# bbc/vc2-reference

Hardware: AMD Instinct MI355X
Metric: Mpixels/s encode+decode, UHD-1 10-bit HQ_ConstQ (higher is better)
Workload: dtype int32; 1 GPU; BASELINE cfg2: UHD-1 3840x2160 4:2:2 10-bit HQ_ConstQ DD97 depth 4, -u 1 -a 2 -q 16 -S 2; streams=1, parallelism=frame-parallel x1, no collective

## Files before the change

include/vc2hip.h:

```cpp
#ifndef VC2HIP_H
#define VC2HIP_H

#include <stddef.h>
#include <stdint.h>

#ifdef __cplusplus
extern "C" {
#endif
#if defined(__GNUC__)
#pragma GCC visibility push(default)
#endif

typedef struct vc2hip_ctx vc2hip_ctx;

enum { VC2HIP_DD97 = 0, VC2HIP_LEGALL = 1, VC2HIP_DD137 = 2, VC2HIP_HAAR0 = 3,
       VC2HIP_HAAR1 = 4, VC2HIP_FIDELITY = 5, VC2HIP_DAUB97 = 6 };
enum { VC2HIP_CF444 = 0, VC2HIP_CF422 = 1, VC2HIP_CF420 = 2 };
enum { VC2HIP_HQ_CONSTQ = 0, VC2HIP_HQ_CBR = 1, VC2HIP_LD = 2 };

enum {
  VC2HIP_OK = 0,
  VC2HIP_EINVAL = -1,
  VC2HIP_EQINDEX = -2,
  VC2HIP_ESCALAR = -3,
  VC2HIP_ECBR_TOOBIG = -4,
  VC2HIP_ECBR_LEN = -5,
  VC2HIP_ECBR_WRONG = -6,
  VC2HIP_EBOUNDED = -7,
  VC2HIP_ELD_TOOBIG = -8,
  VC2HIP_ECAP = -9,
  VC2HIP_ESTREAM = -10,
  VC2HIP_ECODE32 = -11,
  VC2HIP_ESYNTAX = -12,
  VC2HIP_EHIP = -100
};

int vc2hip_create(int device, vc2hip_ctx **out);
#define VC2HIP_FLAG_STORE32         0x001u
#define VC2HIP_FLAG_NO_STREAM       0x002u
#define VC2HIP_FLAG_NO_PAIR         0x004u
#define VC2HIP_FLAG_NO_BANDPLANES   0x008u
#define VC2HIP_FLAG_NO_HEADS        0x010u
#define VC2HIP_FLAG_NO_CBR_INDEX    0x020u
#define VC2HIP_FLAG_GENERIC_DWT     0x040u
#define VC2HIP_FLAG_SINGLE_PASS_VBR 0x080u
#define VC2HIP_FLAG_CBR_GENERAL     0x100u
#define VC2HIP_FLAG_LD_DIAGONALS    0x200u
#define VC2HIP_FLAG_PLANES8_ALWAYS  0x400u
#define VC2HIP_FLAG_PLANES8_NEVER   0x800u
#define VC2HIP_FLAG_TWO_PASS_VBR    0x1000u
int vc2hip_create_with_flags(int device, unsigned flags, vc2hip_ctx **out);
int vc2hip_create_on_stream(int device, void *hip_stream, vc2hip_ctx **out);
void vc2hip_destroy(vc2hip_ctx *ctx);
const char *vc2hip_last_error(const vc2hip_ctx *ctx);
const char *vc2hip_error_string(int code);
int vc2hip_sync(vc2hip_ctx *ctx);

int vc2hip_padded_size(int size, int depth);
int vc2hip_slice_size_is_valid(int depth, int len_luma, int len_chroma, int n_size);
int vc2hip_quant_matrix(int kernel, int depth, int32_t *out);
int vc2hip_slice_bytes(int y_slices, int x_slices, int total_bytes, int scalar, int32_t *out);

int vc2hip_dwt_forward(vc2hip_ctx *ctx, const int32_t *in, int h, int w, int kernel, int depth,
                       int32_t *out);
int vc2hip_dwt_inverse(vc2hip_ctx *ctx, const int32_t *in, int ph, int pw, int kernel, int depth,
                       int32_t *out, int h, int w);
int vc2hip_quantise_np(vc2hip_ctx *ctx, const int32_t *coef, int ph, int pw, int depth,
                       const int32_t *qidx, int ys, int xs, const int32_t *qmatrix, int32_t *out);
int vc2hip_dequantise_np(vc2hip_ctx *ctx, const int32_t *q, int ph, int pw, int depth,
                         const int32_t *qidx, int ys, int xs, const int32_t *qmatrix, int32_t *out);
int vc2hip_dequantise_ld(vc2hip_ctx *ctx, const int32_t *q, int ph, int pw, int depth,
                         const int32_t *qidx, int ys, int xs, const int32_t *qmatrix, int32_t *out);

int vc2hip_quantise_ld(vc2hip_ctx *ctx, const int32_t *coef, int ph, int pw, int depth,
                       const int32_t *qidx, int ys, int xs, const int32_t *qmatrix, int32_t *out);

typedef struct {
  int luma_h, luma_w;
  int chroma_h, chroma_w;
  int depth;
  int y_slices, x_slices;
} vc2hip_geom;

int vc2hip_hq_pack(vc2hip_ctx *ctx, const int32_t *y, const int32_t *u, const int32_t *v,
                   const vc2hip_geom *g, const int32_t *qidx, int prefix, int scalar,
                   const int32_t *cbr_slice_bytes, uint8_t *out, size_t cap, size_t *out_len);
int vc2hip_hq_unpack(vc2hip_ctx *ctx, const uint8_t *in, size_t len, const vc2hip_geom *g,
                     int prefix, int scalar, int32_t *y, int32_t *u, int32_t *v, int32_t *qidx,
                     size_t *consumed);
int vc2hip_ld_unpack(vc2hip_ctx *ctx, const uint8_t *in, size_t len, const vc2hip_geom *g,
                     const int32_t *slice_bytes, int32_t *y, int32_t *u, int32_t *v,
                     int32_t *qidx, size_t *consumed);
int vc2hip_ld_pack(vc2hip_ctx *ctx, const int32_t *y, const int32_t *u, const int32_t *v,
                   const vc2hip_geom *g, const int32_t *qidx, const int32_t *slice_bytes,
                   uint8_t *out, size_t cap, size_t *out_len);
int vc2hip_ld_qindices(vc2hip_ctx *ctx, const int32_t *y, const int32_t *u, const int32_t *v,
                       const vc2hip_geom *g, const int32_t *qmatrix, const int32_t *slice_bytes,
                       int32_t *qidx);
int vc2hip_cbr_qindices(vc2hip_ctx *ctx, const int32_t *y, const int32_t *u, const int32_t *v,
                        const vc2hip_geom *g, const int32_t *qmatrix, const int32_t *slice_bytes,
                        int scalar, int32_t *qidx);

typedef struct {
  int width, height;
  int chroma_format;
  int bit_depth;
  int word_bytes;
  int chroma_bit_depth;
} vc2hip_picture_format;

typedef struct {
  int kernel, depth;
  int y_slices, x_slices;
  int mode;
  int q_index;
  int compressed_bytes;
  int prefix, scalar;
} vc2hip_coding_params;

size_t vc2hip_raw_picture_bytes(const vc2hip_picture_format *fmt);
size_t vc2hip_max_payload_bytes(const vc2hip_picture_format *fmt, const vc2hip_coding_params *cp);

int vc2hip_encode_picture_hq(vc2hip_ctx *ctx, const void *raw, const vc2hip_picture_format *fmt,
                             const vc2hip_coding_params *cp, uint8_t *payload, size_t cap,
                             size_t *len, int32_t *qidx_out);
int vc2hip_encode_picture_ld(vc2hip_ctx *ctx, const void *raw, const vc2hip_picture_format *fmt,
                             const vc2hip_coding_params *cp, uint8_t *payload, size_t cap,
                             size_t *len, int32_t *qidx_out);
int vc2hip_decode_picture_hq(vc2hip_ctx *ctx, const uint8_t *payload, size_t len,
                             const vc2hip_picture_format *fmt, const vc2hip_coding_params *cp,
                             void *raw_out);
int vc2hip_decode_picture_ld(vc2hip_ctx *ctx, const uint8_t *payload, size_t len,
                             const vc2hip_picture_format *fmt, const vc2hip_coding_params *cp,
                             void *raw_out);

#define VC2HIP_MAX_INFLIGHT 2
void *vc2hip_host_alloc(size_t bytes);
void vc2hip_host_free(void *p);
int vc2hip_encode_picture_begin(vc2hip_ctx *ctx, const void *raw, const vc2hip_picture_format *fmt,
                                const vc2hip_coding_params *cp, uint8_t *payload, size_t cap, int32_t *qidx_out, int *ticket);
int vc2hip_encode_picture_end(vc2hip_ctx *ctx, int ticket, size_t *len);
int vc2hip_decode_picture_begin(vc2hip_ctx *ctx, const uint8_t *payload, size_t len, const vc2hip_picture_format *fmt,
                                const vc2hip_coding_params *cp, void *raw_out, int *ticket);
int vc2hip_decode_picture_end(vc2hip_ctx *ctx, int ticket);

int vc2hip_set_streams(vc2hip_ctx *ctx, int k);
int vc2hip_encode_batch_dev(vc2hip_ctx *ctx, const void *d_raw, int n,
                            const vc2hip_picture_format *fmt, const vc2hip_coding_params *cp,
                            void *d_payload, size_t payload_stride, uint64_t *d_lens);
int vc2hip_decode_batch_dev(vc2hip_ctx *ctx, const void *d_payload, size_t payload_stride,
                            const uint64_t *d_lens, int n, const vc2hip_picture_format *fmt,
                            const vc2hip_coding_params *cp, void *d_raw_out);

typedef struct {
  int major_version;
  uint32_t first_picture_number;
  uint32_t prev_parse_offset;
  int end_of_sequence;
} vc2hip_stream_params;

int vc2hip_picture_header(const vc2hip_coding_params *cp, int major_version, uint32_t picture_number,
                          uint8_t *out, size_t cap, size_t *len);
int vc2hip_stream_write_dev(vc2hip_ctx *ctx, const void *d_payload, size_t payload_stride, const uint64_t *d_lens, int n,
                            const vc2hip_coding_params *cp, const vc2hip_stream_params *sp,
                            uint8_t *d_stream, size_t cap, uint64_t *d_stream_len);
int vc2hip_stream_read_dev(vc2hip_ctx *ctx, const uint8_t *d_stream, size_t len, int n,
                           const vc2hip_coding_params *cp, const vc2hip_stream_params *sp,
                           void *d_payload, size_t payload_stride, uint64_t *d_lens,
                           uint32_t *d_picture_numbers, uint64_t *d_consumed);

int vc2hip_band_plane_bits(const vc2hip_ctx *ctx);

#define VC2HIP_DWT_TILE   0
#define VC2HIP_DWT_FAST   1
#define VC2HIP_DWT_STREAM 2
#define VC2HIP_DWT_PAIR   3
#define VC2HIP_DWT_PLANE  4
typedef struct {
  int inverse;
  int level;
  int levels;
  int family;
  int edge;
  int store_bits;
  int segments;
  int tail;
  int small_gather;
  int pictures;
  int band_planes;
} vc2hip_dwt_launch;
int vc2hip_dwt_launches(const vc2hip_ctx *ctx, vc2hip_dwt_launch *out, int cap);

int vc2hip_profile_enable(vc2hip_ctx *ctx, int on);
int vc2hip_profile_only(vc2hip_ctx *ctx, const char *name);
int vc2hip_profile_count(vc2hip_ctx *ctx);
int vc2hip_profile_get(vc2hip_ctx *ctx, int i, const char **name, int *launches, double *total_ms);
int vc2hip_profile_reset(vc2hip_ctx *ctx);

#if defined(__GNUC__)
#pragma GCC visibility pop
#endif
#ifdef __cplusplus
}
#endif
#endif
```

vc2-reference_amd/csrc/vc2hip_api.hip:

```cpp
#include <math.h>
#include <stdio.h>
#include <stdlib.h>
#include <string.h>

#include <algorithm>
#include <string>
#include <map>
#include <mutex>
#include <utility>
#include <vector>

#include "vc2hip_internal.h"

void vc2_upload_tables_slices(const QuantTables &t, hipStream_t s);
int vc2_halo_x(int kernel);
int vc2_halo_y(int kernel);
void vc2_upload_vlc_lut(hipStream_t s);
void vc2_upload_unpack_lut(hipStream_t s);
bool vc2_slice_index_supported(int prefix, int scalar);
size_t vc2_pack_lds_bytes(int prefix, int scalar);
int vc2_pack_image_mode(int prefix, int scalar);
void vc2_upload_tables_fast(const QuantTables &t, hipStream_t s);
bool vc2_fast_level_applicable(LevelParams &p);
int vc2_launch_forward_fast(Launcher &L, int kernel, bool first, const LevelParams &p, int n, bool store16, hipStream_t s);
int vc2_launch_inverse_fast(Launcher &L, int kernel, bool final_level, const LevelParams &p, int n, bool store16, hipStream_t s);
bool vc2_fast_small_gather(const LevelParams &p);
void vc2_upload_tables_stream(const QuantTables &t, hipStream_t s);
size_t vc2_stream_level_applicable(LevelParams &p, int kernel, bool edge, bool inverse, bool store16, int n_pictures);
int vc2_launch_forward_stream(Launcher &L, int kernel, bool first, const LevelParams &p, int n, bool store16, size_t lds, hipStream_t s);
int vc2_launch_inverse_stream(Launcher &L, int kernel, bool final_level, const LevelParams &p, int n, bool store16, size_t lds, hipStream_t s);
size_t vc2_pair_applicable(PairParams &pp, int kernel, bool edge, bool inverse, bool store16, int n_pictures);
int vc2_launch_forward_pair(Launcher &L, int kernel, bool first, const PairParams &pp, int n, bool store16, size_t lds, hipStream_t s);
int vc2_launch_inverse_pair(Launcher &L, int kernel, bool final_level, const PairParams &pp, int n, bool store16, size_t lds, hipStream_t s);
void vc2_upload_tables_pair(const QuantTables &t, hipStream_t s);
int vc2_launch_plane_transform(Launcher &L, int kernel, int32_t *plane, long long plane_stride, int ph, int pw, int depth, bool inverse,
                               int n, hipStream_t s);
void vc2_launch_plane_ingest(Launcher &L, const void *raw, long long raw_stride, int pic_h, int pic_w, int word_bytes, int bit_depth,
                             int32_t *plane, long long plane_stride, int ph, int pw, int n, hipStream_t s);
void vc2_launch_plane_emit(Launcher &L, const int32_t *plane, long long plane_stride, int pw, void *raw, long long raw_stride, int pic_h,
                           int pic_w, int word_bytes, int bit_depth, int n, hipStream_t s);
void vc2_launch_ll_into_plane(Launcher &L, const int32_t *ll, long long ll_stride, int llh, int llw, int32_t *plane, long long plane_stride,
                              int pw, int depth, int n, hipStream_t s);
void vc2_launch_fill_i32(Launcher &L, int32_t *p, int32_t v, size_t n, hipStream_t s);
void vc2_launch_fill_u64(Launcher &L, unsigned long long *p, unsigned long long v, size_t n, hipStream_t s);

struct ProfEntry {
  std::string name;
  int launches = 0;
  double ms = 0;
};
struct Launcher {
  bool on = false;
  std::string only;
  const char *last_name = nullptr;
  std::string launch_error;
  std::vector<ProfEntry> entries;
  struct Pending { int entry; hipEvent_t a, b; };
  std::vector<Pending> pending;
  std::vector<hipEvent_t> pool;
  int cur_entry = -1;
  hipEvent_t get() {
    hipEvent_t e;
    if (!pool.empty()) { e = pool.back(); pool.pop_back(); }
    else (void)hipEventCreate(&e);
    return e;
  }
  void collect() {
    for (auto &p : pending) {
      float ms = 0;
      if (hipEventElapsedTime(&ms, p.a, p.b) == hipSuccess) { entries[p.entry].ms += ms; entries[p.entry].launches++; }
      pool.push_back(p.a);
      pool.push_back(p.b);
    }
    pending.clear();
  }
};
void vc2_prof_begin(Launcher &L, const char *name, hipStream_t s) {
  (void)s;
  L.last_name = name;
  if (!L.on) return;
  if (!L.only.empty() && ("," + L.only + ",").find(std::string(",") + name + ",") == std::string::npos) return;
  int idx = -1;
  for (size_t i = 0; i < L.entries.size(); ++i) if (L.entries[i].name == name) { idx = (int)i; break; }
  if (idx < 0) { L.entries.push_back(ProfEntry{name, 0, 0}); idx = (int)L.entries.size() - 1; }
  L.cur_entry = idx;
}
void vc2_prof_pair(Launcher &L, hipEvent_t *a, hipEvent_t *b) {
  *a = *b = nullptr;
  if (!L.on || L.cur_entry < 0) return;
  *a = L.get();
  *b = L.get();
  L.pending.push_back(Launcher::Pending{L.cur_entry, *a, *b});
}
void vc2_prof_end(Launcher &L, hipStream_t s) {
  (void)s;
  const hipError_t le = hipGetLastError();
  if (le != hipSuccess && L.launch_error.empty())
    L.launch_error = std::string("kernel launch failed (") + (L.last_name ? L.last_name : "?") + "): " + hipGetErrorString(le);
  L.cur_entry = -1;
#ifdef VC2HIP_ABLATE
  {
    static const bool dbg_sync = getenv("VC2HIP_DEBUG_SYNC") != nullptr;
    if (dbg_sync) {
      fprintf(stderr, "vc2hip stage %s ...", L.last_name ? L.last_name : "?");
      fflush(stderr);
      const hipError_t e = hipStreamSynchronize(s);
      fprintf(stderr, " %s\n", e == hipSuccess ? "done" : hipGetErrorString(e));
      fflush(stderr);
    }
  }
#endif
}
void vc2_prof_break(Launcher &L) { (void)L; }

struct Buf {
  void *p = nullptr;
  size_t cap = 0;
};
enum { B_RAW, B_STORE, B_STOREW, B_LL0, B_LLW, B_QIDX, B_SLOTS, B_SIZES, B_OFFS, B_LENS, B_PAYLOAD,
       B_INDEX, B_PLANE, B_PLANE2, B_CBRB, B_CBRO, B_QM, B_UNITS, B_SEGS, B_COUNT };

struct vc2hip_ctx {
  int device = 0;
  hipStream_t stream = nullptr;
  bool own_stream = false;
  unsigned *d_err = nullptr;
  unsigned *h_err = nullptr;
  Buf buf[B_COUNT];
  Launcher L;
  std::string err;
  int cbr_key[5] = {-1, -1, -1, -1, -1};
  uint64_t cbr_total = 0;
  int debug_skip = 0;
  bool two_pass_vbr = true;
  bool force_two_pass_vbr = false;
#ifndef VC2_ONE_PASS_MIN_PICTURES
#define VC2_ONE_PASS_MIN_PICTURES 112
#endif
  bool force_generic = false;
  bool allow_store16 = true;
  bool allow_planes = true;
  int planes8_mode = 0;
  bool planes8_on = false;
  unsigned long long *d_stat = nullptr;
  unsigned long long *h_stat = nullptr;
  hipEvent_t stat_ev = nullptr;
  bool stat_pending = false, stat_was8 = false, stat_seen = false;
  int stat_n = 0;
  int stat_n_total = 0;
  int last_plane_bits = 0;
  std::vector<vc2hip_dwt_launch> dwt_rec;
  bool dwt_rec_stale = true;
  double stat_samples = 0;
  int ld_batch = 1;
  bool allow_heads = true;
  bool allow_cbr_index = true;
  bool allow_stream = true;
  bool allow_pair = true;
  bool cbr_general = false;
  bool ld_diagonals = false;
  unsigned flags = 0;
  std::vector<vc2hip_ctx *> lanes;
  bool in_split = false;
  hipEvent_t fork_ev = nullptr;
  std::vector<hipEvent_t> join_ev;
  bool lanes_pending = false;
  struct Range { const uint8_t *lo, *hi; };
  struct LaneUse { Range r[2], w[2]; bool valid = false; };
  std::vector<LaneUse> lane_use;
  std::vector<ProfEntry> merged;
  struct Flight {
    vc2hip_ctx *lane = nullptr;
    bool open = false, encode = false;
    uint8_t *payload = nullptr;
    size_t cap = 0;
    unsigned long long *h_len = nullptr;
  };
  Flight flight[VC2HIP_MAX_INFLIGHT];
  int flight_next = 0;
};

static const char *code_text(int code) {
  switch (code) {
    case VC2HIP_OK: return "ok";
    case VC2HIP_EINVAL: return "invalid argument";
    case VC2HIP_EQINDEX: return "quantization index exceeds maximum implemented value.";
    case VC2HIP_ESCALAR: return "Slice scalar is too small, consider using a larger slice scalar.";
    case VC2HIP_ECBR_TOOBIG: return "SliceIO, HQ CBR mode: Too many bytes for the slice";
    case VC2HIP_ECBR_LEN: return "Slice component length exceeds 1 byte when divided by slice size scalar. See above for suggestions to prevent this.";
    case VC2HIP_ECBR_WRONG: return "SliceIO, HQ CBR mode: Wrong number of bytes for a slice";
    case VC2HIP_EBOUNDED: return "Attempt to write beyond end of bounded write";
    case VC2HIP_ELD_TOOBIG: return "SliceIO, LD mode: Too many bytes for the U and V slices";
    case VC2HIP_ECAP: return "output buffer too small";
    case VC2HIP_ESTREAM: return "truncated or malformed slice data";
    case VC2HIP_ECODE32: return "quantised coefficient magnitude exceeds 65534 (outside the 32-bit exp-Golomb code domain)";
    case VC2HIP_ESYNTAX: return "VC-2 stream syntax error";
    case VC2HIP_EHIP: return "HIP runtime error";
  }
  return "unknown error";
}
extern "C" const char *vc2hip_error_string(int code) { return code_text(code); }

static int set_err(vc2hip_ctx *c, int code, const char *msg = nullptr) {
  if (c) c->err = msg ? msg : code_text(code);
  return code;
}
static int hip_fail(vc2hip_ctx *c, hipError_t e, const char *what) {
  char b[256];
  snprintf(b, sizeof b, "HIP error in %s: %s", what, hipGetErrorString(e));
  return set_err(c, VC2HIP_EHIP, b);
}
#define HIPCHK(ctx, call)                                       \
  do {                                                          \
    hipError_t e_ = (call);                                     \
    if (e_ != hipSuccess) return hip_fail(ctx, e_, #call);      \
  } while (0)

extern "C" const char *vc2hip_last_error(const vc2hip_ctx *ctx) { return ctx ? ctx->err.c_str() : "null context"; }

extern "C" int vc2hip_padded_size(int size, int depth) {
  const int cell = 1 << depth;
  return cell * ((size + cell - 1) / cell);
}
extern "C" int vc2hip_slice_size_is_valid(int depth, int len_luma, int len_chroma, int n_size) {
  if (depth <= 0 || depth > 31) return 0;
  const int unit = 1 << depth;
  const int max_slices = (len_luma < len_chroma ? len_luma : len_chroma) / unit;
  if (n_size <= 0 || n_size > max_slices) return 0;
  const int ts = n_size * unit;
  const int pl = vc2hip_padded_size(len_luma, depth), pc = vc2hip_padded_size(len_chroma, depth);
  const int n = (pl + ts - 1) / ts;
  if (pl % n == 0 && (pl / n) % unit == 0 && pc % n == 0 && (pc / n) % unit == 0) return n;
  return 0;
}
extern "C" int vc2hip_quant_matrix(int kernel, int depth, int32_t *out) {
  static const float A[7] = {1.280868846f, 1.224744871f, 1.280868846f, 1.414213562f, 1.414213562f, 0.682408629f, 1.139917028f};
  static const float B[7] = {0.820572875f, 0.847791248f, 0.809253958f, 0.707106871f, 0.707106871f, 1.367856979f, 0.887168005f};
  static const int S[7] = {1, 1, 1, 0, 1, 0, 1};
  if (kernel < 0 || kernel > 6 || depth < 0 || depth > 30) return VC2HIP_EINVAL;
  if (depth == 0) { out[0] = 0; return 0; }
  const float a2 = A[kernel] * A[kernel], ab = A[kernel] * B[kernel], b2 = B[kernel] * B[kernel];
  std::vector<float> gl(depth + 1), gh(depth + 1), gd(depth + 1);
  float mn = 3.402823466e+38f;
  for (int lv = depth; lv > 0; --lv) {
    const float sc = (float)(pow((double)a2, depth - lv) / pow(2.0, S[kernel] * (depth - lv + 1)));
    gl[lv] = sc * a2; gh[lv] = sc * ab; gd[lv] = sc * b2;
    mn = fminf(fminf(fminf(gl[lv], gh[lv]), gd[lv]), mn);
  }
  auto qv = [&](float g) { return (int)floorf(4.0f * logf(g / mn) / logf(2.0f) + 0.5f); };
  int i = 0;
  out[i++] = qv(gl[1]);
  for (int lv = 1; lv <= depth; ++lv) { out[i++] = qv(gh[lv]); out[i++] = qv(gh[lv]); out[i++] = qv(gd[lv]); }
  return 0;
}
void vc2_allow_lds(const void *kernel, size_t bytes) {
  static std::mutex mu;
  static std::map<std::pair<const void *, int>, size_t> done;
  int dev = 0;
  (void)hipGetDevice(&dev);
  std::lock_guard<std::mutex> lock(mu);
  size_t &have = done[std::make_pair(kernel, dev)];
  if (bytes > have) {
    (void)hipFuncSetAttribute(kernel, hipFuncAttributeMaxDynamicSharedMemorySize, (int)bytes);
    have = bytes;
  }
}

static int gcd_i(int a, int b) { a = abs(a); b = abs(b); while (b) { int t = a % b; a = b; b = t; } return a; }
extern "C" int vc2hip_slice_bytes(int ys, int xs, int total_bytes, int scalar, int32_t *out) {
  if (ys < 1 || xs < 1 || scalar < 1) return VC2HIP_EINVAL;
  const int n = ys * xs;
  int num = total_bytes / scalar - 4 * n, den = n;
  const int g = gcd_i(num, den);
  if (g) { num /= g; den /= g; }
  const int ratio = num / den, rem = num - ratio * den;
  int residue = 0;
  for (int i = 0; i < n; ++i) {
    residue += rem;
    if (residue < den) out[i] = ratio * scalar + 4;
    else { out[i] = (ratio + 1) * scalar + 4; residue -= den; }
  }
  return 0;
}
static void make_tables(QuantTables &t) {
  for (int q = 0; q < 120; ++q) {
    const uint64_t base = 1ull << (q / 4);
    uint64_t f;
    switch (q % 4) {
      case 0: f = 4 * base; break;
      case 1: f = (503829 * base + 52958) / 105917; break;
      case 2: f = (665857 * base + 58854) / 117708; break;
      default: f = (440253 * base + 32722) / 65444; break;
    }
    t.qf[q] = (int32_t)(uint32_t)f;
    t.off[q] = q == 0 ? 1 : (q == 1 ? 2 : (int32_t)(((uint32_t)t.qf[q] + 1u)) / 2);
    t.magic[q] = 0;
    t.shift[q] = 0;
    if (t.qf[q] > 1) {
      const uint64_t d = (uint64_t)t.qf[q];
      int l = 0;
      while ((1ull << l) < d) ++l;
      t.magic[q] = (uint32_t)((((1ull << l) - d) << 32) / d + 1);
      t.shift[q] = l - 1;
    }
    const double r = 4.0 / (double)(uint32_t)t.qf[q];
    float up = (float)r;
    if ((double)up < r) up = nextafterf(up, INFINITY);
    t.inv4[q] = up;
  }
}

static int create_common(int device, hipStream_t stream, bool own, vc2hip_ctx **out, unsigned flags = 0) {
  if (!out) return VC2HIP_EINVAL;
  *out = nullptr;
  int n = 0;
  if (hipGetDeviceCount(&n) != hipSuccess || device < 0 || device >= n) return VC2HIP_EHIP;
  vc2hip_ctx *c = new vc2hip_ctx;
  c->device = device;
#ifdef VC2HIP_ABLATE
  {
    static const struct { const char *name; unsigned flag; } env[] = {
      {"VC2HIP_STORE32", VC2HIP_FLAG_STORE32}, {"VC2HIP_NO_STREAM", VC2HIP_FLAG_NO_STREAM}, {"VC2HIP_NO_PAIR", VC2HIP_FLAG_NO_PAIR},
      {"VC2HIP_NO_BANDPLANES", VC2HIP_FLAG_NO_BANDPLANES}, {"VC2HIP_NO_HEADS", VC2HIP_FLAG_NO_HEADS},
      {"VC2HIP_NO_CBR_INDEX", VC2HIP_FLAG_NO_CBR_INDEX}, {"VC2HIP_GENERIC_DWT", VC2HIP_FLAG_GENERIC_DWT},
      {"VC2HIP_SINGLE_PASS_VBR", VC2HIP_FLAG_SINGLE_PASS_VBR}, {"VC2HIP_TWO_PASS_VBR", VC2HIP_FLAG_TWO_PASS_VBR}, {"VC2HIP_CBR_GENERAL", VC2HIP_FLAG_CBR_GENERAL},
      {"VC2HIP_PLANES8_ALWAYS", VC2HIP_FLAG_PLANES8_ALWAYS}, {"VC2HIP_PLANES8_NEVER", VC2HIP_FLAG_PLANES8_NEVER}};
    for (const auto &e : env) { const char *v = getenv(e.name); if (v && v[0] == '1') flags |= e.flag; }
    { const char *v = getenv("VC2HIP_LD_ROWS"); if (v && v[0] == '0') flags |= VC2HIP_FLAG_LD_DIAGONALS; }
    { const char *e = getenv("VC2HIP_DEBUG_SKIP"); c->debug_skip = e ? atoi(e) : 0; }
  }
#endif
  c->force_generic = (flags & VC2HIP_FLAG_GENERIC_DWT) != 0;
  c->allow_store16 = !(flags & VC2HIP_FLAG_STORE32);
  c->allow_stream = !(flags & VC2HIP_FLAG_NO_STREAM);
  c->allow_pair = !(flags & VC2HIP_FLAG_NO_PAIR);
  c->allow_planes = !(flags & VC2HIP_FLAG_NO_BANDPLANES);
  c->planes8_mode = (flags & VC2HIP_FLAG_PLANES8_NEVER) ? 2 : (flags & VC2HIP_FLAG_PLANES8_ALWAYS) ? 1 : 0;
  c->allow_heads = !(flags & VC2HIP_FLAG_NO_HEADS);
  c->allow_cbr_index = !(flags & VC2HIP_FLAG_NO_CBR_INDEX);
  c->two_pass_vbr = !(flags & VC2HIP_FLAG_SINGLE_PASS_VBR);
  c->force_two_pass_vbr = (flags & VC2HIP_FLAG_TWO_PASS_VBR) != 0;
  c->cbr_general = (flags & VC2HIP_FLAG_CBR_GENERAL) != 0;
  c->ld_diagonals = (flags & VC2HIP_FLAG_LD_DIAGONALS) != 0;
  c->flags = flags;
  if (hipSetDevice(device) != hipSuccess) { delete c; return VC2HIP_EHIP; }
  if (own) { if (hipStreamCreateWithFlags(&stream, hipStreamNonBlocking) != hipSuccess) { delete c; return VC2HIP_EHIP; } }
  c->stream = stream;
  c->own_stream = own;
  if (hipMalloc((void **)&c->d_err, 256 + 4096) != hipSuccess ||
     
      hipHostMalloc((void **)&c->h_err, VC2_ERRBLK_COPY) != hipSuccess ||
      hipMalloc((void **)&c->d_stat, 64) != hipSuccess || hipHostMalloc((void **)&c->h_stat, 64 * 8) != hipSuccess ||
      hipEventCreateWithFlags(&c->stat_ev, hipEventDisableTiming) != hipSuccess) { delete c; return VC2HIP_EHIP; }
  (void)hipMemsetAsync(c->d_stat, 0, 64, c->stream);
  (void)hipMemsetAsync(c->d_err, 0, sizeof(unsigned), c->stream);
  QuantTables t;
  make_tables(t);
  vc2_upload_tables(t, c->stream);
  vc2_upload_tables_slices(t, c->stream);
  vc2_upload_tables_fast(t, c->stream);
  vc2_upload_tables_pair(t, c->stream);
  vc2_upload_tables_stream(t, c->stream);
  vc2_upload_vlc_lut(c->stream);
  vc2_upload_unpack_lut(c->stream);
  if (hipStreamSynchronize(c->stream) != hipSuccess) { delete c; return VC2HIP_EHIP; }
  *out = c;
  return VC2HIP_OK;
}
extern "C" int vc2hip_create(int device, vc2hip_ctx **out) { return create_common(device, nullptr, true, out); }
extern "C" int vc2hip_create_with_flags(int device, unsigned flags, vc2hip_ctx **out) { return create_common(device, nullptr, true, out, flags); }
extern "C" int vc2hip_create_on_stream(int device, void *s, vc2hip_ctx **out) { return create_common(device, (hipStream_t)s, false, out); }
extern "C" void vc2hip_destroy(vc2hip_ctx *c) {
  if (!c) return;
  (void)hipSetDevice(c->device);
  (void)hipStreamSynchronize(c->stream);
  for (vc2hip_ctx *l : c->lanes) if (l != c) vc2hip_destroy(l);
  for (auto &f : c->flight) { if (f.lane) vc2hip_destroy(f.lane); if (f.h_len) (void)hipHostFree(f.h_len); }
  for (hipEvent_t e : c->join_ev) (void)hipEventDestroy(e);
  if (c->fork_ev) (void)hipEventDestroy(c->fork_ev);
  c->L.collect();
  for (auto e : c->L.pool) (void)hipEventDestroy(e);
  for (auto &b : c->buf) if (b.p) (void)hipFree(b.p);
  if (c->d_err) (void)hipFree(c->d_err);
  if (c->h_err) (void)hipHostFree(c->h_err);
  if (c->h_stat) (void)hipHostFree(c->h_stat);
  if (c->d_stat) (void)hipFree(c->d_stat);
  if (c->stat_ev) (void)hipEventDestroy(c->stat_ev);
  if (c->own_stream) (void)hipStreamDestroy(c->stream);
  delete c;
}

void vc2_ld_disable_rows();
static int err_from_flags(vc2hip_ctx *c, unsigned f) {
  if (!f) return VC2HIP_OK;
  if (f & VC2_DEVERR_HANDOFF) {
    vc2_ld_disable_rows();
    return set_err(c, VC2HIP_EHIP, "LD index search: a hand-over between workgroups timed out; nothing was written for the batch. "
                                   "The library now searches with one launch per slice diagonal: submit the batch again.");
  }
  if (f & VC2_DEVERR_SYNTAX) {
    static const char *why[VC2_SYN_COUNT] = {"?", "parse info prefix is not BBCD", "unknown parse code",
                                             "data unit runs past the end of the stream", "next_parse_offset is 0",
                                             "end of sequence before the pictures asked for",
                                             "picture parameters differ from the coding parameters",
                                             "custom quantisation matrix flag set", "asymmetric transform",
                                             "picture before any sequence header and no major version given",
                                             "fragment out of order"};
    const unsigned w = *(const unsigned *)((const char *)c->h_err + VC2_ERRBLK_SYNTAX_WHY);
    char b[256];
    snprintf(b, sizeof b, "VC-2 stream syntax error at byte %llu: %s",
             *(const unsigned long long *)((const char *)c->h_err + VC2_ERRBLK_SYNTAX_AT), why[w < VC2_SYN_COUNT ? w : 0]);
    return set_err(c, VC2HIP_ESYNTAX, b);
  }
  if (f & VC2_DEVERR_QINDEX) return set_err(c, VC2HIP_EQINDEX);
  if (f & VC2_DEVERR_SCALAR) return set_err(c, VC2HIP_ESCALAR);
  if (f & VC2_DEVERR_CBR_TOOBIG) return set_err(c, VC2HIP_ECBR_TOOBIG);
  if (f & VC2_DEVERR_CBR_LEN) return set_err(c, VC2HIP_ECBR_LEN);
  if (f & VC2_DEVERR_CODE32) return set_err(c, VC2HIP_ECODE32);
  if (f & VC2_DEVERR_LD_TOOBIG) return set_err(c, VC2HIP_ELD_TOOBIG);
  if (f & VC2_DEVERR_CAP) return set_err(c, VC2HIP_ECAP);
  return set_err(c, VC2HIP_ESTREAM);
}
static int join_lanes(vc2hip_ctx *c) {
  if (!c->lanes_pending || c->in_split) return VC2HIP_OK;
  for (size_t i = 1; i < c->lanes.size(); ++i)
    if (c->lane_use[i].valid) HIPCHK(c, hipStreamWaitEvent(c->stream, c->join_ev[i], 0));
  c->lanes_pending = false;
  return VC2HIP_OK;
}
static int enter(vc2hip_ctx *c) {
  HIPCHK(c, hipSetDevice(c->device));
  if (!c->in_split) vc2_prof_break(c->L);
  c->dwt_rec_stale = true;
  return join_lanes(c);
}
#define ENTER(ctx) do { int rc_ = enter(ctx); if (rc_) return rc_; } while (0)

extern "C" int vc2hip_set_streams(vc2hip_ctx *c, int k) {
  if (!c || k < 1 || k > 16) return set_err(c, VC2HIP_EINVAL);
  ENTER(c);
  HIPCHK(c, hipStreamSynchronize(c->stream));
  for (vc2hip_ctx *l : c->lanes) if (l != c) vc2hip_destroy(l);
  c->lanes.clear();
  c->lane_use.clear();
  for (hipEvent_t e : c->join_ev) (void)hipEventDestroy(e);
  c->join_ev.clear();
  if (k == 1) return VC2HIP_OK;
  if (!c->fork_ev) HIPCHK(c, hipEventCreateWithFlags(&c->fork_ev, hipEventDisableTiming));
  for (int i = 0; i < k; ++i) {
    vc2hip_ctx *l = c;
    if (i > 0) {
      const int rc = vc2hip_create_with_flags(c->device, c->flags, &l);
      if (rc) return set_err(c, rc);
      l->L.on = c->L.on;
    }
    c->lanes.push_back(l);
    hipEvent_t e;
    HIPCHK(c, hipEventCreateWithFlags(&e, hipEventDisableTiming));
    c->join_ev.push_back(e);
  }
  c->lane_use.assign((size_t)k, vc2hip_ctx::LaneUse());
  return VC2HIP_OK;
}

template <class U, class F> static int split_batch(vc2hip_ctx *c, int n, U use, F fn) {
  const int k = std::min<int>((int)c->lanes.size(), n);
  HIPCHK(c, hipSetDevice(c->device));
  HIPCHK(c, hipEventRecord(c->fork_ev, c->stream));
  std::vector<vc2hip_ctx::LaneUse> cur((size_t)c->lanes.size());
  std::vector<int> first((size_t)k), count((size_t)k);
  auto overlap = [](const vc2hip_ctx::Range &a, const vc2hip_ctx::Range &b) { return a.lo && b.lo && a.lo < b.hi && b.lo < a.hi; };
  for (int i = 0, f0 = 0; i < k; ++i) {
    count[i] = n / k + (i < n % k ? 1 : 0);
    first[i] = f0;
    f0 += count[i];
    use(first[i], count[i], cur[i]);
    cur[i].valid = true;
  }
  for (int i = 0; i < k; ++i) {
    vc2hip_ctx *l = c->lanes[i];
    if (i > 0) HIPCHK(c, hipStreamWaitEvent(l->stream, c->fork_ev, 0));
    for (size_t j = 0; j < c->lanes.size(); ++j) {
      const vc2hip_ctx::LaneUse &p = c->lane_use[j];
      if ((int)j == i || !p.valid) continue;
      bool dep = false;
      for (int a = 0; a < 2; ++a)
        for (int b = 0; b < 2; ++b)
          dep |= overlap(cur[i].r[a], p.w[b]) || overlap(cur[i].w[a], p.w[b]) || overlap(cur[i].w[a], p.r[b]);
// ... 34 lines not shown
    return set_err(c, VC2HIP_EHIP, m.c_str());
  }
  const int rc = err_from_flags(c, *c->h_err);
  return rc ? rc : lane_rc;
}

static int need(vc2hip_ctx *c, int which, size_t bytes, void **out) {
  Buf &b = c->buf[which];
  if (b.cap < bytes) {
    HIPCHK(c, hipStreamSynchronize(c->stream));
    if (b.p) HIPCHK(c, hipFree(b.p));
    b.p = nullptr;
    b.cap = 0;
    size_t cap = bytes >= (1u << 21) ? (bytes + (1u << 21) - 1) & ~(size_t)((1u << 21) - 1) : (bytes + 4095) & ~(size_t)4095;
    { static const size_t unit = (size_t)vc2_tune_int("VC2HIP_ALLOC_ROUND_MB", 0) << 20;
      if (unit && bytes >= (1u << 21)) cap = (bytes + unit - 1) / unit * unit; }
    HIPCHK(c, hipMalloc(&b.p, cap));
    b.cap = cap;
#ifdef VC2HIP_ABLATE
    if (getenv("VC2HIP_DEBUG_ALLOC")) fprintf(stderr, "vc2hip alloc: buffer %d at %p, %zu bytes\n", which, b.p, cap);
#endif
  }
  *out = b.p;
  return VC2HIP_OK;
}
#define NEED(ctx, which, bytes, ptr)                                   \
  do {                                                                 \
    void *p_;                                                          \
    int rc_ = need(ctx, which, bytes, &p_);                            \
    if (rc_) return rc_;                                               \
    ptr = (decltype(ptr))p_;                                           \
  } while (0)

extern "C" int vc2hip_profile_enable(vc2hip_ctx *c, int on) {
  if (!c) return VC2HIP_EINVAL;
  c->L.on = on != 0;
  for (vc2hip_ctx *l : c->lanes) l->L.on = on != 0;
  return 0;
}
extern "C" int vc2hip_profile_only(vc2hip_ctx *c, const char *name) {
  if (!c) return VC2HIP_EINVAL;
  c->L.only = name ? name : "";
  for (vc2hip_ctx *l : c->lanes) l->L.only = c->L.only;
  return 0;
}
extern "C" int vc2hip_profile_count(vc2hip_ctx *c) {
  if (!c) return 0;
  c->merged = c->L.entries;
  for (vc2hip_ctx *l : c->lanes)
    if (l != c) for (const ProfEntry &e : l->L.entries) {
      bool found = false;
      for (ProfEntry &m : c->merged) if (m.name == e.name) { m.launches += e.launches; m.ms += e.ms; found = true; break; }
      if (!found) c->merged.push_back(e);
    }
  return (int)c->merged.size();
}
extern "C" int vc2hip_profile_get(vc2hip_ctx *c, int i, const char **name, int *launches, double *total_ms) {
  if (!c || i < 0 || i >= (int)c->merged.size()) return VC2HIP_EINVAL;
  if (name) *name = c->merged[i].name.c_str();
  if (launches) *launches = c->merged[i].launches;
  if (total_ms) *total_ms = c->merged[i].ms;
  return 0;
}
extern "C" int vc2hip_profile_reset(vc2hip_ctx *c) {
  if (!c) return VC2HIP_EINVAL;
  c->L.collect(); c->L.entries.clear(); c->merged.clear();
  for (vc2hip_ctx *l : c->lanes) if (l != c) { l->L.collect(); l->L.entries.clear(); }
  return 0;
}

static int make_geom(Geom &g, const int ph[3], const int pw[3], const int h[3], const int w[3], int depth,
                     int ys, int xs) {
  if (depth < 1 || depth > VC2_MAX_DEPTH || ys < 1 || xs < 1) return VC2HIP_EINVAL;
  g.depth = depth; g.ys = ys; g.xs = xs;
  int off = 0;
  for (int c = 0; c < 3; ++c) {
    CompGeom &cg = g.c[c];
    cg.h = h[c]; cg.w = w[c]; cg.ph = ph[c]; cg.pw = pw[c];
    if (ph[c] == 0 || pw[c] == 0) { cg.sh = cg.sw = cg.n0 = 0; cg.coef_off = off; continue; }
    if (ph[c] % ys || pw[c] % xs) return VC2HIP_EINVAL;
    cg.sh = ph[c] / ys; cg.sw = pw[c] / xs;
    if (cg.sh % (1 << depth) || cg.sw % (1 << depth)) return VC2HIP_EINVAL;
    cg.n0 = (cg.sh >> depth) * (cg.sw >> depth);
    cg.coef_off = off;
    off += cg.sh * cg.sw;
  }
  g.slice_coefs = off;
  return VC2HIP_OK;
}

static void chroma_dims(int h, int w, int cf, int *ch, int *cw) {
  *ch = cf == VC2HIP_CF420 ? h / 2 : h;
  *cw = cf == VC2HIP_CF444 ? w : w / 2;
}

static int picture_geom(Geom &g, const vc2hip_picture_format *f, const vc2hip_coding_params *cp, bool decoder) {
  if (!f || !cp || f->width < 1 || f->height < 1 || f->word_bytes < 1 || f->word_bytes > 4 ||
      f->bit_depth < 1 || f->bit_depth > 8 * f->word_bytes || f->chroma_format < 0 || f->chroma_format > 2 ||
      f->chroma_bit_depth < 0 || f->chroma_bit_depth > 8 * f->word_bytes)
    return VC2HIP_EINVAL;
  int ch, cw;
  chroma_dims(f->height, f->width, f->chroma_format, &ch, &cw);
  int h[3] = {f->height, ch, ch}, w[3] = {f->width, cw, cw}, ph[3], pw[3];
  ph[0] = vc2hip_padded_size(f->height, cp->depth);
  pw[0] = vc2hip_padded_size(f->width, cp->depth);
  if (decoder) chroma_dims(ph[0], pw[0], f->chroma_format, &ph[1], &pw[1]);
  else { ph[1] = vc2hip_padded_size(ch, cp->depth); pw[1] = vc2hip_padded_size(cw, cp->depth); }
  ph[2] = ph[1]; pw[2] = pw[1];
  return make_geom(g, ph, pw, h, w, cp->depth, cp->y_slices, cp->x_slices);
}

extern "C" size_t vc2hip_raw_picture_bytes(const vc2hip_picture_format *f) {
  int ch, cw;
  chroma_dims(f->height, f->width, f->chroma_format, &ch, &cw);
  return ((size_t)f->height * f->width + 2 * (size_t)ch * cw) * f->word_bytes;
}
static size_t max_slice_bytes(int prefix, int scalar) { return (size_t)prefix + 4 + 3 * 255 * (size_t)scalar; }
extern "C" size_t vc2hip_max_payload_bytes(const vc2hip_picture_format *f, const vc2hip_coding_params *cp) {
  (void)f;
  const size_t n = (size_t)cp->y_slices * cp->x_slices;
  if (cp->mode == VC2HIP_HQ_CONSTQ) return n * max_slice_bytes(cp->prefix, cp->scalar);
  if (cp->mode == VC2HIP_HQ_CBR) return (size_t)cp->compressed_bytes + n * (cp->prefix + (size_t)cp->scalar + 4);
  return (size_t)cp->compressed_bytes + n;
}

struct LLPlanes {
  void *p[VC2_MAX_DEPTH + 1][3];
  int32_t *w[VC2_MAX_DEPTH + 1][3];
  long long stride[VC2_MAX_DEPTH + 1][3];
};

static size_t ll_elems(const Geom &g, int n) {
  size_t e = 0;
  for (int l = 1; l <= g.depth; ++l)
    for (int c = 0; c < 3; ++c) e += (((size_t)(g.c[c].ph >> l) * (g.c[c].pw >> l) * n + 7) & ~(size_t)7);
  return e;
}
static size_t ll_bytes(const Geom &g, int n) { return ll_elems(g, n) * sizeof(int32_t); }
static void ll_layout(const Geom &g, int n, void *base, int elem_bytes, int32_t *wide, LLPlanes &ll) {
  size_t off = 0;
  memset(&ll, 0, sizeof ll);
  for (int l = 1; l <= g.depth; ++l)
    for (int c = 0; c < 3; ++c) {
      const size_t e = (size_t)(g.c[c].ph >> l) * (g.c[c].pw >> l);
      ll.p[l][c] = (char *)base + off * elem_bytes;
      ll.w[l][c] = wide ? wide + off : nullptr;
      ll.stride[l][c] = (long long)e;
      off += (e * n + 7) & ~(size_t)7;
    }
}
static void ll_layout(const Geom &g, int n, int32_t *base, LLPlanes &ll) { ll_layout(g, n, base, 4, nullptr, ll); }

static void record_dwt(vc2hip_ctx *c, bool inverse, int level, int levels, int family, bool edge, bool s16, int segments, int tail,
                       bool small_gather, int n, int band_planes = 0) {
  if (c->dwt_rec_stale) { c->dwt_rec.clear(); c->dwt_rec_stale = false; }
  vc2hip_dwt_launch r;
  r.inverse = inverse; r.level = level; r.levels = levels; r.family = family; r.edge = edge; r.store_bits = s16 ? 16 : 32;
  r.segments = segments; r.tail = tail; r.small_gather = small_gather; r.pictures = n; r.band_planes = band_planes;
  c->dwt_rec.push_back(r);
}

static int band_plane_bits(const LevelParams &p) {
  for (int k = 0; k < 3; ++k) if (p.bp_base[k] >= 0) return p.bp8 ? 8 : 16;
  return 0;
}

static void fill_level(LevelParams &p, const Geom &g, int level, int kernel, const int32_t *qm) {
  const int D = g.depth, Lv = D - level;
  p.band = 3 * (Lv - 1) + 1;
  p.ys = g.ys; p.xs = g.xs; p.slice_coefs = g.slice_coefs;
  const int hx = vc2_halo_x(kernel), hy = vc2_halo_y(kernel);
  for (int c = 0; c < 3; ++c) {
    const CompGeom &cg = g.c[c];
    p.in_h[c] = cg.ph >> level; p.in_w[c] = cg.pw >> level;
    p.pic_h[c] = cg.h; p.pic_w[c] = cg.w;
    p.coef_off[c] = cg.coef_off;
    p.rec_stride[c] = g.slice_coefs;
    if (cg.ph == 0) { p.tiles_x[c] = p.tiles_y[c] = 0; p.fh[c] = p.fw[c] = 2; p.tsy[c] = p.tsx[c] = 1; continue; }
    p.fh[c] = cg.sh >> level; p.fw[c] = cg.sw >> level;
    int tsy = 1, tsx = 1;
    while (tsy * 2 * p.fh[c] <= 64 && tsy * 2 <= g.ys) tsy *= 2;
    while (tsx * 2 * p.fw[c] <= 128 && tsx * 2 <= g.xs) tsx *= 2;
    while ((size_t)(tsy * p.fh[c] + 2 * hy) * (tsx * p.fw[c] + 2 * hx) * 4 > 150 * 1024) {
      if (tsx > 1) tsx /= 2; else if (tsy > 1) tsy /= 2; else break;
    }
    p.tsy[c] = tsy; p.tsx[c] = tsx;
    p.tiles_y[c] = (g.ys + tsy - 1) / tsy;
    p.tiles_x[c] = (g.xs + tsx - 1) / tsx;
    p.band_n[c] = (p.fh[c] / 2) * (p.fw[c] / 2);
    p.band_off[c] = p.band_n[c];
  }
  for (int b = 0; b < 3 * D + 1; ++b) p.qmatrix[b] = qm ? qm[b] : 0;
}

static int run_forward(vc2hip_ctx *c, const Geom &g, int kernel, int n, const void *const src[3],
                       const long long src_stride[3], bool src_raw, const vc2hip_picture_format *f,
                       void *store, const LLPlanes &ll, bool s16 = false, int32_t *store_wide = nullptr) {
  auto level_params = [&](LevelParams &p, int level) {
    memset(&p, 0, sizeof p);
    fill_level(p, g, level, kernel, nullptr);
    p.store = store; p.store_stride = (long long)g.ys * g.xs * g.slice_coefs;
    p.store_wide = store_wide;
    p.err = c->d_err;
    p.ll_to_store = (level == g.depth - 1);
    const bool first = (level == 0) && src_raw;
    for (int k = 0; k < 3; ++k) {
      if (level == 0) { p.plane[k] = (void *)src[k]; p.plane_stride[k] = src_stride[k]; }
      else { p.plane[k] = ll.p[level][k]; p.plane_wide[k] = ll.w[level][k]; p.plane_stride[k] = ll.stride[level][k]; }
      p.ll[k] = ll.p[level + 1][k]; p.ll_wide[k] = ll.w[level + 1][k]; p.ll_stride[k] = ll.stride[level + 1][k];
    }
    if (first) {
      p.word_bytes = f->word_bytes;
      p.sample_shift = 8 * f->word_bytes - f->bit_depth;
      p.sample_offset = 1 << (f->bit_depth - 1);
      const int cd = f->chroma_bit_depth ? f->chroma_bit_depth : f->bit_depth;
      p.sample_shift_c = 8 * f->word_bytes - cd;
      p.sample_offset_c = 1 << (cd - 1);
    }
  };
  for (int level = 0; level < g.depth; ++level) {
    LevelParams p;
    level_params(p, level);
    const bool first = (level == 0) && src_raw;
    if (!c->force_generic && c->allow_stream && c->allow_pair && level + 1 < g.depth) {
      PairParams pp;
      memset(&pp, 0, sizeof pp);
      pp.a = p;
      pp.a.debug_skip = c->debug_skip;
      level_params(pp.b, level + 1);
      const size_t lds = vc2_pair_applicable(pp, kernel, first, false, s16, n);
      if (lds) {
        int rc = vc2_launch_forward_pair(c->L, kernel, first, pp, n, s16, lds, c->stream);
        if (rc) return set_err(c, rc, "invalid wavelet kernel");
        record_dwt(c, false, level, 2, VC2HIP_DWT_PAIR, first, s16, pp.a.st_segmax, 0, false, n);
        ++level;
        continue;
      }
    }
    LevelParams pf = p;
    pf.debug_skip = c->debug_skip;
    if (!c->force_generic && c->allow_stream) {
      LevelParams ps = p;
      const size_t lds = vc2_stream_level_applicable(ps, kernel, first, false, s16, n);
      if (lds) {
        int rc = vc2_launch_forward_stream(c->L, kernel, first, ps, n, s16, lds, c->stream);
        if (rc) return set_err(c, rc, "invalid wavelet kernel");
        record_dwt(c, false, level, 1, VC2HIP_DWT_STREAM, first, s16, ps.st_segmax, ps.st_tail, false, n);
        continue;
      }
    }
    if (!c->force_generic && vc2_fast_level_applicable(pf)) {
      int rc = vc2_launch_forward_fast(c->L, kernel, first, pf, n, s16, c->stream);
      if (rc) return set_err(c, rc, "invalid wavelet kernel");
      record_dwt(c, false, level, 1, VC2HIP_DWT_FAST, first, s16, 0, 0, false, n);
      continue;
    }
    if (s16) return set_err(c, VC2HIP_EINVAL, "internal: 16-bit store without the fast level kernels");
    if (vc2_level_lds_bytes(kernel, p) > 160 * 1024) return set_err(c, VC2HIP_EINVAL, "slice too large for one LDS tile");
    int rc = vc2_launch_forward_level(c->L, kernel, first, p, n, c->stream);
    if (rc) return set_err(c, rc, "invalid wavelet kernel");
    record_dwt(c, false, level, 1, VC2HIP_DWT_TILE, first, false, 0, 0, false, n);
  }
  return VC2HIP_OK;
}

static int run_inverse(vc2hip_ctx *c, const Geom &g, int kernel, int n, void *store, const int32_t *qidx,
                       const int32_t *qm, bool dequant, bool ll_ready, const LLPlanes &ll, void *const dst[3],
                       const long long dst_stride[3], bool dst_raw, const vc2hip_picture_format *f,
                       bool s16 = false, int32_t *store_wide = nullptr, const BandPlanes *bp = nullptr,
                       long long store_stride = 0, unsigned *stream_mask = nullptr, const HeadSplit *hs = nullptr, int head_level = 1 << 30,
                       unsigned *fast_mask = nullptr, unsigned *tail_mask = nullptr) {
  if (tail_mask) *tail_mask = 0;
  if (stream_mask) *stream_mask = 0;
  if (fast_mask) *fast_mask = 0;
  auto level_params = [&](LevelParams &p, int level) {
    memset(&p, 0, sizeof p);
    fill_level(p, g, level, kernel, qm);
    if (hs && level >= head_level)
      for (int k = 0; k < 3; ++k) if (g.c[k].ph) { p.rec_stride[k] = hs->n[k]; p.coef_off[k] = (int)hs->base[k]; }
    p.store = store; p.store_stride = store_stride ? store_stride : (long long)g.ys * g.xs * g.slice_coefs;
    for (int k = 0; k < 3; ++k) p.bp_base[k] = (bp && level < bp->levels && g.c[k].ph) ? bp->base[k][level] : -1;
    p.bp8 = bp && level < bp->levels && bp->bytes8;
    p.store_wide = store_wide;
    p.qidx = qidx; p.err = c->d_err; p.dequant = dequant;
    p.ll_from_store = (level == g.depth - 1) && !ll_ready;
    const bool fin = (level == 0) && dst_raw;
    for (int k = 0; k < 3; ++k) {
      if (level == 0) { p.plane[k] = dst ? dst[k] : nullptr; p.plane_stride[k] = dst_stride ? dst_stride[k] : 0; }
      else { p.plane[k] = ll.p[level][k]; p.plane_wide[k] = ll.w[level][k]; p.plane_stride[k] = ll.stride[level][k]; }
      p.ll[k] = ll.p[level + 1][k]; p.ll_wide[k] = ll.w[level + 1][k]; p.ll_stride[k] = ll.stride[level + 1][k];
    }
    if (fin) {
      p.word_bytes = f->word_bytes;
      p.sample_shift = 8 * f->word_bytes - f->bit_depth;
      p.sample_offset = 1 << (f->bit_depth - 1);
      p.clip_lo = -(1 << (f->bit_depth - 1));
      p.clip_hi = (1 << (f->bit_depth - 1)) - 1;
    }
  };
  for (int level = g.depth - 1; level >= 0; --level) {
    LevelParams p;
    level_params(p, level);
    const bool fin = (level == 0) && dst_raw;
    if (!stream_mask && !c->force_generic && c->allow_stream && c->allow_pair && level >= 1) {
      PairParams pp;
      memset(&pp, 0, sizeof pp);
      level_params(pp.a, level - 1);
      pp.b = p;
      pp.a.debug_skip = c->debug_skip;
      const bool fin_a = (level - 1 == 0) && dst_raw;
      static const int inv_final = vc2_tune_int("VC2HIP_PAIR_INV_FINAL", 0);
      const size_t lds = (fin_a && !inv_final) ? 0 : vc2_pair_applicable(pp, kernel, fin_a, true, s16, n);
      if (lds) {
        int rc = vc2_launch_inverse_pair(c->L, kernel, fin_a, pp, n, s16, lds, c->stream);
        if (rc) return set_err(c, rc, "invalid wavelet kernel");
        record_dwt(c, true, level - 1, 2, VC2HIP_DWT_PAIR, fin_a, s16, pp.a.st_segmax, 0, false, n,
                   std::max(band_plane_bits(pp.a), band_plane_bits(pp.b)));
        --level;
        continue;
      }
    }
    LevelParams pf = p;
    pf.debug_skip = c->debug_skip;
    if (!c->force_generic && c->allow_stream) {
      LevelParams ps = p;
      const size_t lds = vc2_stream_level_applicable(ps, kernel, fin, true, s16, n);
      if (lds) {
        if (stream_mask) { *stream_mask |= 1u << level; if (tail_mask && ps.st_tail) *tail_mask |= 1u << level; continue; }
        int rc = vc2_launch_inverse_stream(c->L, kernel, fin, ps, n, s16, lds, c->stream);
        if (rc) return set_err(c, rc, "invalid wavelet kernel");
        record_dwt(c, true, level, 1, VC2HIP_DWT_STREAM, fin, s16, ps.st_segmax, ps.st_tail, false, n, band_plane_bits(ps));
        continue;
      }
    }
    if (stream_mask) { if (fast_mask && !c->force_generic && vc2_fast_level_applicable(pf)) *fast_mask |= 1u << level; continue; }
    if (bp && level < bp->levels) return set_err(c, VC2HIP_EINVAL, "internal: band planes without the streaming kernel");
    if (!c->force_generic && vc2_fast_level_applicable(pf)) {
      int rc = vc2_launch_inverse_fast(c->L, kernel, fin, pf, n, s16, c->stream);
      if (rc) return set_err(c, rc, "invalid wavelet kernel");
      record_dwt(c, true, level, 1, VC2HIP_DWT_FAST, fin, s16, 0, 0, vc2_fast_small_gather(pf), n, band_plane_bits(pf));
      continue;
    }
    if (s16) return set_err(c, VC2HIP_EINVAL, "internal: 16-bit store without the fast level kernels");
    if (vc2_level_lds_bytes(kernel, p) > 160 * 1024) return set_err(c, VC2HIP_EINVAL, "slice too large for one LDS tile");
    int rc = vc2_launch_inverse_level(c->L, kernel, fin, p, n, c->stream);
    if (rc) return set_err(c, rc, "invalid wavelet kernel");
    record_dwt(c, true, level, 1, VC2HIP_DWT_TILE, fin, false, 0, 0, false, n, band_plane_bits(p));
  }
  return VC2HIP_OK;
}

static bool use_store16(const vc2hip_ctx *c, const Geom &g, int kernel) {
  if (!c->allow_store16 || c->force_generic) return false;
  for (int k = 0; k < 3; ++k) {
    if (!g.c[k].ph) continue;
    if ((g.c[k].sh * g.c[k].sw) % 8 || g.c[k].coef_off % 8) return false;
  }
  if (g.slice_coefs % 8) return false;
  for (int level = 0; level < g.depth; ++level) {
    LevelParams p;
    memset(&p, 0, sizeof p);
    fill_level(p, g, level, kernel, nullptr);
    if (!vc2_fast_level_applicable(p)) return false;
  }
  return true;
}

static bool needs_plane_path(const vc2hip_ctx *c, const Geom &g, int kernel) {
  for (int level = 0; level < g.depth; ++level) {
    LevelParams p;
    memset(&p, 0, sizeof p);
    fill_level(p, g, level, kernel, nullptr);
    LevelParams pf = p;
    if (!c->force_generic && vc2_fast_level_applicable(pf)) continue;
    if (vc2_level_lds_bytes(kernel, p) > 160 * 1024) return true;
  }
  return false;
}
static size_t plane_elems(const Geom &g) {
  size_t e = 0;
  for (int k = 0; k < 3; ++k) e += (size_t)g.c[k].ph * g.c[k].pw;
  return e;
}
static int plane_forward(vc2hip_ctx *c, const Geom &g, int kernel, int n, const void *const src[3], const long long ss[3],
                         const vc2hip_picture_format *f, int32_t *d_store) {
  int32_t *d_plane;
  NEED(c, B_PLANE, plane_elems(g) * n * 4, d_plane);
// ... 724 lines not shown
        for (int k = 0; k < c->stat_n; ++k) bytes += (double)c->h_stat[1 + k];
        const double bits = c->stat_n ? 8.0 * bytes / (c->stat_n * c->stat_samples) : 99.0;
        const double esc = (double)c->h_stat[0] * 8.0 / (std::max(1, c->stat_n_total) * c->stat_samples);
#ifdef VC2HIP_ABLATE
        if (getenv("VC2HIP_PLANES8_DEBUG")) fprintf(stderr, "planes8: previous batch %d pictures, %.2f payload bits per sample, %s planes, escape pieces %.4f%%\n", c->stat_n, bits, c->stat_was8 ? "byte" : "16-bit", 100 * esc);
#endif
        if (c->stat_was8 && esc > 0.005) c->planes8_on = false;
        else if (!c->stat_was8 || esc < 0.002) c->planes8_on = bits < (c->planes8_on ? 6.5 : 6.0);
      }
      bool b8 = c->planes8_mode == 1 || (c->planes8_mode == 0 && c->planes8_on);
      for (int l = 0; l < bp.levels; ++l) if (tails >> l & 1) b8 = false;
      bp.bytes8 = b8;
    }
  }
  HeadSplit hs;
  memset(&hs, 0, sizeof hs);
  int head_level = 1 << 30;
  if (s16 && !plane_path && c->allow_heads) {
    unsigned smask = 0, fmask = 0;
    LLPlanes none;
    memset(&none, 0, sizeof none);
    (void)run_inverse(c, g, cp->kernel, n, nullptr, nullptr, qm, true, ld, none, dst, ds, true, f, s16, nullptr, nullptr, 0, &smask, nullptr, 1 << 30, &fmask);
    int ls = g.depth;
    while (ls > 0 && !(smask >> (ls - 1) & 1) && (fmask >> (ls - 1) & 1)) --ls;
    bool ok = ls >= 1 && ls < g.depth && ls >= bp.levels;
    for (int k = 0; k < 3 && ok; ++k) {
      if (!g.c[k].ph) continue;
      const int hn = (g.c[k].sh >> ls) * (g.c[k].sw >> ls);
      ok = hn >= 8 && hn % 8 == 0 && hn <= bp.from[k];
    }
    if (ok) {
      long long at = sstride;
      for (int k = 0; k < 3; ++k) {
        if (!g.c[k].ph) continue;
        hs.n[k] = (g.c[k].sh >> ls) * (g.c[k].sw >> ls);
        hs.base[k] = at;
        at += ((long long)ns * hs.n[k] + 7) & ~7ll;
      }
      if (at < (1ll << 31)) { sstride = at; head_level = ls; } else memset(&hs, 0, sizeof hs);
    }
  }
  int32_t *d_store, *d_ll, *d_q, *d_storew = nullptr, *d_llw = nullptr;
  {
    static const int pad = vc2_tune_int("VC2HIP_DEC_STORE_PAD", 0);
    if (s16 && pad > 0 && sstride + pad < (1ll << 31)) sstride += pad & ~7;
  }
  NEED(c, B_STORE, std::max((size_t)n * ns * g.slice_coefs * 4, (size_t)n * (size_t)sstride * 2), d_store);
  NEED(c, B_LL0, ll_bytes(g, n) + 16, d_ll);
  if (s16) {
    NEED(c, B_STOREW, (size_t)n * sstride * 4, d_storew);
    NEED(c, B_LLW, ll_bytes(g, n) + 16, d_llw);
  }
  NEED(c, B_QIDX, (size_t)n * ns * 4, d_q);
  LLPlanes ll;
  ll_layout(g, n, d_ll, s16 ? 2 : 4, d_llw, ll);
  if (!ld) {
    if (!d_lens || cp->scalar < 1 || cp->prefix < 0) return set_err(c, VC2HIP_EINVAL);
    uint32_t *d_offs;
    const int32_t *d_cb = nullptr; const uint32_t *d_co = nullptr; uint64_t cbr_total = 0;
    if (cp->mode == VC2HIP_HQ_CBR && cp->compressed_bytes > 0 && c->allow_cbr_index) {
      const int key[5] = {g.ys, g.xs, cp->compressed_bytes, cp->scalar, cp->prefix};
      if (memcmp(key, c->cbr_key, sizeof key) || !c->buf[B_CBRB].p) {
        std::vector<int32_t> sb(ns);
        int32_t *db; uint32_t *dof; uint64_t total;
        if (vc2hip_slice_bytes(g.ys, g.xs, cp->compressed_bytes, cp->scalar, sb.data()) == VC2HIP_OK &&
            cbr_offsets_upload(c, sb.data(), ns, cp->prefix, &db, &dof, &total) == VC2HIP_OK) {
          memcpy(c->cbr_key, key, sizeof key);
          c->cbr_total = total;
        }
      }
      if (!memcmp(key, c->cbr_key, sizeof key)) { d_cb = (const int32_t *)c->buf[B_CBRB].p; d_co = (const uint32_t *)c->buf[B_CBRO].p; cbr_total = c->cbr_total; }
    }
    if ((rc = build_index(c, (const uint8_t *)d_payload, (long long)payload_stride, (const unsigned long long *)d_lens, n, ns,
                          cp->prefix, cp->scalar, &d_offs, d_cb, d_co, cbr_total))) return rc;
    UnpackParams p;
    memset(&p, 0, sizeof p);
    p.payload = (const uint8_t *)d_payload; p.payload_stride = (long long)payload_stride;
    p.lens = (const unsigned long long *)d_lens; p.offsets = d_offs;
    p.store = d_store; p.store_stride = sstride; p.qidx = d_q;
    p.store16 = s16; p.store_wide = d_storew;
    p.n_slices = ns; p.slice_coefs = g.slice_coefs;
    int n0[3];
    fill_comp_arrays(g, p.comp_n, p.comp_off, n0);
    p.prefix = cp->prefix; p.scalar = cp->scalar; p.err = c->d_err;
    p.bp = bp; p.hs = hs; p.xs = g.xs;
    c->last_plane_bits = bp.levels ? (bp.bytes8 ? 8 : 16) : 0;
    p.stats = c->d_stat;
    bool capturing = false;
    if (!c->own_stream) {
      hipStreamCaptureStatus cs = hipStreamCaptureStatusNone;
      capturing = hipStreamIsCapturing(c->stream, &cs) != hipSuccess || cs != hipStreamCaptureStatusNone;
    }
    const bool track = bp.levels && c->planes8_mode == 0 && !c->stat_pending && !capturing;
    if (track) HIPCHK(c, hipMemsetAsync(c->d_stat, 0, 8, c->stream));
    vc2_launch_unpack(c->L, p, n, c->stream);
    if (track) {
      c->stat_n = std::min(n, 60);
      c->stat_n_total = n;
      c->stat_samples = 0;
      for (int k = 0; k < 3; ++k) c->stat_samples += (double)g.c[k].h * g.c[k].w;
      c->stat_was8 = bp.bytes8 != 0;
      HIPCHK(c, hipMemcpyAsync(c->h_stat, c->d_stat, 8, hipMemcpyDeviceToHost, c->stream));
      HIPCHK(c, hipMemcpyAsync(c->h_stat + 1, d_lens, (size_t)c->stat_n * 8, hipMemcpyDeviceToHost, c->stream));
      HIPCHK(c, hipEventRecord(c->stat_ev, c->stream));
      c->stat_pending = true;
    }
  } else {
    int32_t *d_sb; uint32_t *d_so; uint64_t total;
    const int key[5] = {g.ys, g.xs, cp->compressed_bytes, 1, -7};
    if (memcmp(key, c->cbr_key, sizeof key) || !c->buf[B_CBRB].p) {
      std::vector<int32_t> sb(ns);
      vc2hip_slice_bytes(g.ys, g.xs, cp->compressed_bytes, 1, sb.data());
      if ((rc = ld_offsets_upload(c, sb.data(), ns, &d_sb, &d_so, &total))) return rc;
      memcpy(c->cbr_key, key, sizeof key);
      c->cbr_total = total;
    }
    d_sb = (int32_t *)c->buf[B_CBRB].p; d_so = (uint32_t *)c->buf[B_CBRO].p; total = c->cbr_total;
    if (total > payload_stride) return set_err(c, VC2HIP_ESTREAM);
    LdUnpackParams p;
    fill_ld_unpack(p, g, (const uint8_t *)d_payload, (long long)payload_stride, d_sb, d_so, d_store, d_q, c->d_err);
    unsigned *d_shifted; uint32_t *d_starts;
    NEED(c, B_SIZES, (size_t)n * 4, d_shifted);
    NEED(c, B_OFFS, (size_t)n * ns * 4, d_starts);
    int flag_fill = 0;
#ifdef VC2HIP_ABLATE
    if (getenv("VC2HIP_DEBUG_LD_REDO")) flag_fill = 1;
#endif
    HIPCHK(c, hipMemsetAsync(d_shifted, flag_fill, (size_t)n * 4, c->stream));
    vc2_prof_break(c->L);
    p.lens = (const unsigned long long *)d_lens; p.shifted = d_shifted; p.starts = d_starts;
    vc2_launch_ld_unpack(c->L, p, n, c->stream);
    vc2_launch_ld_walk(c->L, p, n, c->stream);
    p.redo = 1;
    vc2_launch_ld_unpack(c->L, p, n, c->stream);
    LdLl3Params lp;
    lp.store = d_store; lp.store_stride = (long long)ns * g.slice_coefs; lp.slice_coefs = g.slice_coefs;
    lp.ys = g.ys; lp.xs = g.xs; lp.qidx = d_q; lp.qm0 = qm[0]; lp.err = c->d_err;
    for (int k = 0; k < 3; ++k) {
      lp.coef_off[k] = g.c[k].coef_off; lp.llh[k] = g.c[k].ph >> g.depth; lp.llw[k] = g.c[k].pw >> g.depth;
      lp.ll_plane[k] = (int32_t *)ll.p[g.depth][k]; lp.ll_stride[k] = ll.stride[g.depth][k];
    }
    if (!vc2_launch_ld_ll3(c->L, lp, n, c->stream))
    for (int k = 0; k < 3; ++k)
      vc2_launch_ld_ll(c->L, d_store, (long long)ns * g.slice_coefs, g.slice_coefs, g.c[k].coef_off, g.c[k].n0,
                       g.c[k].ph >> g.depth, g.c[k].pw >> g.depth, g.ys, g.xs, d_q, qm[0], (int32_t *)ll.p[g.depth][k],
                       ll.stride[g.depth][k], n, c->d_err, c->stream);
  }
  if (plane_path) return plane_inverse(c, g, cp->kernel, n, d_store, d_q, qm, dst, ds, f, ld ? &ll : nullptr);
  return run_inverse(c, g, cp->kernel, n, d_store, d_q, qm, true, ld, ll, dst, ds, true, f, s16, d_storew, &bp, sstride, nullptr,
                     hs.n[0] ? &hs : nullptr, head_level);
}

extern "C" int vc2hip_band_plane_bits(const vc2hip_ctx *c) { return c ? c->last_plane_bits : 0; }

namespace {
struct HeaderBits {
  uint8_t *out;
  size_t cap, pos = 0;
  unsigned cache = 0;
  int cached = 0;
  void bit(unsigned b) {
    cache = (cache << 1) | (b & 1);
    if (++cached == 8) { if (pos < cap) out[pos] = (uint8_t)cache; ++pos; cache = 0; cached = 0; }
  }
  void uvlc(uint32_t v) {
    const unsigned long long x = (unsigned long long)v + 1;
    int top = 63;
    while (!(x >> top & 1)) --top;
    for (int i = top - 1; i >= 0; --i) { bit(0); bit((unsigned)(x >> i) & 1); }
    bit(1);
  }
  void align() { while (cached) bit(0); }
};
bool stream_cp_ok(const vc2hip_coding_params *cp) {
  if (!cp || cp->kernel < 0 || cp->kernel > 6 || cp->depth < 0 || cp->y_slices < 1 || cp->x_slices < 1) return false;
  if (cp->mode == VC2HIP_LD) return cp->compressed_bytes > 0;
  return (cp->mode == VC2HIP_HQ_CONSTQ || cp->mode == VC2HIP_HQ_CBR) && cp->prefix >= 0 && cp->scalar >= 1;
}
void stream_ab(const vc2hip_coding_params *cp, uint32_t *a, uint32_t *b) {
  if (cp->mode != VC2HIP_LD) { *a = (uint32_t)cp->prefix; *b = (uint32_t)cp->scalar; return; }
  const int ns = cp->y_slices * cp->x_slices, g = gcd_i(cp->compressed_bytes, ns);
  *a = (uint32_t)(cp->compressed_bytes / g);
  *b = (uint32_t)(ns / g);
}
}

extern "C" int vc2hip_picture_header(const vc2hip_coding_params *cp, int major_version, uint32_t picture_number, uint8_t *out,
                                     size_t cap, size_t *len) {
  if (!stream_cp_ok(cp) || major_version < 1 || !len || (cap && !out)) return VC2HIP_EINVAL;
  uint32_t a, b;
  stream_ab(cp, &a, &b);
  HeaderBits w{out, cap};
  for (int i = 24; i >= 0; i -= 8) for (int k = 7; k >= 0; --k) w.bit(picture_number >> (i + k));
  w.uvlc((uint32_t)cp->kernel);
  w.uvlc((uint32_t)cp->depth);
  if (major_version >= 3) { w.bit(0); w.bit(0); }
  w.uvlc((uint32_t)cp->x_slices);
  w.uvlc((uint32_t)cp->y_slices);
  w.uvlc(a);
  w.uvlc(b);
  w.bit(0);
  w.align();
  *len = w.pos;
  return w.pos > cap ? VC2HIP_ECAP : VC2HIP_OK;
}

extern "C" int vc2hip_stream_write_dev(vc2hip_ctx *c, const void *d_payload, size_t payload_stride, const uint64_t *d_lens, int n,
                                       const vc2hip_coding_params *cp, const vc2hip_stream_params *sp, uint8_t *d_stream,
                                       size_t cap, uint64_t *d_stream_len) {
  if (!c || !d_payload || !d_lens || n < 1 || !cp || !sp || !d_stream || !d_stream_len) return set_err(c, VC2HIP_EINVAL);
  if (((size_t)d_payload | payload_stride | (size_t)d_stream) & 15 || ((size_t)d_lens | (size_t)d_stream_len) & 7)
    return set_err(c, VC2HIP_EINVAL, "device buffers and the payload stride must be 16-byte aligned");
  if (sp->major_version < 1) return set_err(c, VC2HIP_EINVAL, "major_version must be at least 1");
  StreamWriteParams p;
  memset(&p, 0, sizeof p);
  size_t hl = 0;
  if (vc2hip_picture_header(cp, sp->major_version, sp->first_picture_number, p.hdr, sizeof p.hdr, &hl))
    return set_err(c, VC2HIP_EINVAL);
  ENTER(c);
  NEED(c, B_UNITS, (size_t)n * 8, p.unit_off);
  p.payload = (const uint8_t *)d_payload; p.payload_stride = (long long)payload_stride;
  p.lens = (const unsigned long long *)d_lens;
  p.stream = d_stream; p.cap = cap; p.stream_len = (unsigned long long *)d_stream_len;
  p.err = c->d_err;
  p.n = n; p.hdr_len = (int)hl; p.code = cp->mode == VC2HIP_LD ? 0xC8 : 0xE8; p.eos = sp->end_of_sequence != 0;
  p.first_picture_number = sp->first_picture_number; p.prev_parse_offset = sp->prev_parse_offset;
  vc2_launch_stream_layout(c->L, p, c->stream);
  vc2_launch_stream_copy(c->L, p, c->stream);
  return VC2HIP_OK;
}

extern "C" int vc2hip_stream_read_dev(vc2hip_ctx *c, const uint8_t *d_stream, size_t len, int n, const vc2hip_coding_params *cp,
                                      const vc2hip_stream_params *sp, void *d_payload, size_t payload_stride, uint64_t *d_lens,
                                      uint32_t *d_picture_numbers, uint64_t *d_consumed) {
  if (!c || !d_stream || n < 1 || !cp || !sp || !d_payload || !d_lens) return set_err(c, VC2HIP_EINVAL);
  if (((size_t)d_payload | payload_stride) & 15 || ((size_t)d_lens | (size_t)d_consumed) & 7 || (size_t)d_picture_numbers & 3)
    return set_err(c, VC2HIP_EINVAL, "device buffers and the payload stride must be 16-byte aligned");
  if (!stream_cp_ok(cp) || sp->major_version < 0 || payload_stride >= (1ull << 32)) return set_err(c, VC2HIP_EINVAL);
  ENTER(c);
  StreamReadParams p;
  memset(&p, 0, sizeof p);
  p.seg_cap = cp->y_slices * cp->x_slices + 1;
  NEED(c, B_SEGS, (size_t)n * p.seg_cap * sizeof(StreamSeg), p.segs);
  NEED(c, B_UNITS, (size_t)n * sizeof(uint2), p.meta);
  p.stream = d_stream; p.len = len; p.n = n; p.major_version = sp->major_version;
  p.kernel = cp->kernel; p.depth = cp->depth; p.ys = cp->y_slices; p.xs = cp->x_slices; p.ld = cp->mode == VC2HIP_LD;
  stream_ab(cp, &p.a, &p.b);
  p.payload = (uint8_t *)d_payload; p.payload_stride = (long long)payload_stride;
  p.lens = (unsigned long long *)d_lens; p.picture_numbers = d_picture_numbers; p.consumed = (unsigned long long *)d_consumed;
  p.err = c->d_err;
  vc2_launch_stream_walk(c->L, p, c->stream);
  vc2_launch_stream_gather(c->L, p, c->stream);
  return VC2HIP_OK;
}

extern "C" int vc2hip_dwt_launches(const vc2hip_ctx *c, vc2hip_dwt_launch *out, int cap) {
  if (!c || cap < 0 || (cap && !out)) return VC2HIP_EINVAL;
  const int n = (int)c->dwt_rec.size();
  for (int i = 0; i < n && i < cap; ++i) out[i] = c->dwt_rec[i];
  return n;
}

extern "C" int vc2hip_decode_batch_dev(vc2hip_ctx *c, const void *d_payload, size_t payload_stride, const uint64_t *d_lens,
                                       int n, const vc2hip_picture_format *f, const vc2hip_coding_params *cp, void *d_raw_out) {
  if (c && c->lanes.size() > 1 && n > 1 && !c->in_split && d_payload && f && cp && d_raw_out) {
    const size_t rb = vc2hip_raw_picture_bytes(f);
    const uint8_t *out8 = (const uint8_t *)d_raw_out, *pay8 = (const uint8_t *)d_payload, *len8 = (const uint8_t *)d_lens;
    return split_batch(c, n,
      [&](int first, int count, vc2hip_ctx::LaneUse &u) {
        u.r[0] = {pay8 + (size_t)first * payload_stride, pay8 + (size_t)(first + count) * payload_stride};
        u.r[1] = {len8 ? len8 + (size_t)first * 8 : nullptr, len8 ? len8 + (size_t)(first + count) * 8 : nullptr};
        u.w[0] = {out8 + (size_t)first * rb, out8 + (size_t)(first + count) * rb}; u.w[1] = {nullptr, nullptr};
      },
      [&](vc2hip_ctx *l, int first, int count) {
        return vc2hip_decode_batch_dev(l, pay8 + (size_t)first * payload_stride, payload_stride,
                                       d_lens ? d_lens + first : nullptr, count, f, cp, (uint8_t *)d_raw_out + (size_t)first * rb);
      });
  }
  return decode_batch_common(c, d_payload, payload_stride, d_lens, n, f, cp, d_raw_out, cp && cp->mode == VC2HIP_LD);
}

extern "C" int vc2hip_encode_picture_hq(vc2hip_ctx *c, const void *raw, const vc2hip_picture_format *f,
                                        const vc2hip_coding_params *cp, uint8_t *payload, size_t cap, size_t *len,
                                        int32_t *qidx_out) {
  if (!c || !raw || !f || !cp || !payload || !len) return set_err(c, VC2HIP_EINVAL);
  ENTER(c);
  const size_t rb = vc2hip_raw_picture_bytes(f), pcap = (vc2hip_max_payload_bytes(f, cp) + 15) & ~(size_t)15;
  uint8_t *d_raw, *d_pay; unsigned long long *d_len;
  NEED(c, B_RAW, rb + 64, d_raw);
  NEED(c, B_PAYLOAD, pcap + 64, d_pay);
  NEED(c, B_LENS, 64, d_len);
  HIPCHK(c, hipMemcpyAsync(d_raw, raw, rb, hipMemcpyHostToDevice, c->stream));
  int rc = vc2hip_encode_batch_dev(c, d_raw, 1, f, cp, d_pay, pcap, (uint64_t *)d_len);
  if (rc) return rc;
  unsigned long long l = 0;
  HIPCHK(c, hipMemcpyAsync(&l, d_len, 8, hipMemcpyDeviceToHost, c->stream));
  if (qidx_out)
    HIPCHK(c, hipMemcpyAsync(qidx_out, c->buf[B_QIDX].p, (size_t)cp->y_slices * cp->x_slices * 4, hipMemcpyDeviceToHost, c->stream));
  if ((rc = vc2hip_sync(c))) return rc;
  if (l > cap) return set_err(c, VC2HIP_ECAP);
  HIPCHK(c, hipMemcpy(payload, d_pay, l, hipMemcpyDeviceToHost));
  *len = (size_t)l;
  return VC2HIP_OK;
}

extern "C" int vc2hip_encode_picture_ld(vc2hip_ctx *c, const void *raw, const vc2hip_picture_format *f,
// ... 126 lines not shown
```

vc2-reference_amd/csrc/vc2hip_dwt_pair.hip:

```cpp
#include <stdio.h>
#include <stdlib.h>

#include <algorithm>
#include <map>
#include <mutex>
#include <tuple>
#include <type_traits>
#include <vector>

#include "vc2hip_internal.h"
#include "vc2hip_store.h"
#include "vc2hip_wavelets.h"

void vc2_prof_begin(Launcher &L, const char *name, hipStream_t s);
void vc2_prof_end(Launcher &L, hipStream_t s);

__constant__ QuantTables c_qsp;
void vc2_upload_tables_pair(const QuantTables &t, hipStream_t s) {
  (void)hipMemcpyToSymbolAsync(HIP_SYMBOL(c_qsp), &t, sizeof t, 0, hipMemcpyHostToDevice, s);
}

namespace {

#ifndef VC2_PAIR_NT
#define VC2_PAIR_NT 1
#endif
#include "vc2hip_stream_eng.h"

__device__ __forceinline__ void pair_prio(int mode, int prio0, int block) {
  if (mode == 1) { prio_turn(prio0 + block); return; }
  const int t = mode == 2 ? block : block >> (mode - 2);
  if ((prio0 + t) & 1) __builtin_amdgcn_s_setprio(3);
  else __builtin_amdgcn_s_setprio(0);
}

template <int V> using IC = std::integral_constant<int, V>;
template <bool V> using BC = std::integral_constant<bool, V>;

template <int K> constexpr bool pair_kernel() {
  if constexpr (K == VC2HIP_FIDELITY || K == VC2HIP_DAUB97) return false;
  else return reach_fits<K, 2>() && reach_fits<K, 4>() && WT<K>::nsteps == 2;
}
template <int K> constexpr int pair_halo() { return halo_lanes<K, 4>() + halo_lanes<K, 2>(); }
constexpr int fdiv2(int v) { return v >= 0 ? v / 2 : -((-v + 1) / 2); }

#ifndef VC2_PAIR_WPE
#define VC2_PAIR_WPE 2
#endif
template <int K> constexpr int pair_wpe() { return K == VC2HIP_DD137 ? 2 : VC2_PAIR_WPE; }
#ifndef VC2_PAIR_PF
#define VC2_PAIR_PF 2
#endif
constexpr int PFP = VC2_PAIR_PF;
template <int K, bool FIRST, class ST>
__global__ __launch_bounds__(64, (pair_wpe<K>())) void k_fwd_pair(const PairParams pp) {
  using S_ = St<ST>;
  using EA = VEng<K, false, 4>;
  using EB = VEng<K, false, 2>;
  using T = VT<K, false>;
  constexpr int OFFL = T::OFFL, SD = T::sum_dmin();
  constexpr int ACC = WT<K>::accuracy;
  extern __shared__ __attribute__((aligned(16))) unsigned char smem[];
#define p pp.a
#define pb pp.b
  const int lane = threadIdx.x & 63;
  int comp, pic;
  Strip sp;
  if (!strip_of_block_h<pair_halo<K>()>(p, comp, pic, sp)) return;
  const int spl = pp.spl[comp];
  sp.nsl *= spl;
  sp.sx0 *= spl;
  ST *imgA = (ST *)smem, *imgB = (ST *)(smem + pp.img_b);
  unsigned *ring_ll = (unsigned *)(smem + pp.ring_ll);
  const int szA = pp.sz_a, szB = pp.sz_b, grpA = pp.grp_a, nll = pp.n_ll;
  const int xs = p.xs, slice_coefs = p.slice_coefs, st_prio = p.st_prio;
#ifdef VC2HIP_ABLATE
  const int dskip = p.debug_skip;
#else
  constexpr int dskip = 0;
#endif
  const int pieceA = pp.piece_a[comp], pieceB = pp.piece_b[comp];
  const int sshift = FIRST ? (comp ? p.sample_shift_c : p.sample_shift) : 0;
  const int bias = FIRST ? -((comp ? p.sample_offset_c : p.sample_offset) << ACC) : 0;
  const int in_h = p.in_h[comp], in_w = p.in_w[comp], npA = in_h >> 1, npB = npA >> 1;
  const int chunk = min(sp.c0 + lane, (in_w >> 3) - 1);
  const bool own = lane >= sp.lo && lane < sp.hi;
  const bool redge = sp.c0 + lane == (in_w >> 3) - 1 && lane != 63;

  const uint8_t *raw = nullptr;
  const ST *lvl = nullptr;
  const int32_t *lvl_w = nullptr;
  if constexpr (FIRST) raw = (const uint8_t *)p.plane[comp] + (size_t)pic * p.plane_stride[comp] + (size_t)chunk * 16;
  else {
    lvl = (const ST *)p.plane[comp] + (size_t)pic * p.plane_stride[comp] + (size_t)chunk * 8;
    if constexpr (S_::narrow) lvl_w = p.plane_wide[comp] + (size_t)pic * p.plane_stride[comp] + (size_t)chunk * 8;
  }
  const int pic_h = FIRST ? p.pic_h[comp] : in_h;
  constexpr int NQ = (FIRST || S_::narrow) ? 1 : 2;
  uint4 pf[PFP][2][NQ];
  auto fetch = [&](int m, int slot) __attribute__((always_inline)) {
#pragma unroll
    for (int h = 0; h < 2; ++h) {
      const int y = min(2 * m + h, pic_h - 1);
      if constexpr (FIRST) pf[slot][h][0] = *(const uint4 *)(raw + mul24z(y, in_w) * 2);
      else {
        const ST *q = lvl + mul24z(y, in_w);
        pf[slot][h][0] = *(const uint4 *)q;
        if constexpr (NQ == 2) pf[slot][h][1] = *(const uint4 *)(q + 4);
      }
    }
  };
  auto convert = [&](int m, int slot, int h, RowT<4> &r) __attribute__((always_inline)) {
    if constexpr (FIRST) {
      const unsigned w[4] = {pf[slot][h][0].x, pf[slot][h][0].y, pf[slot][h][0].z, pf[slot][h][0].w};
#pragma unroll
      for (int k = 0; k < 4; ++k) {
        const unsigned b = __builtin_amdgcn_perm(w[k], w[k], 0x02030001u);
        r[k] = (int)(((b & 0xFFFFu) >> sshift) << ACC) + bias;
        r[4 + k] = (int)((b >> (16 + sshift)) << ACC) + bias;
      }
    } else {
      int s[8];
      if constexpr (S_::narrow) S_::unpack8(pf[slot][h][0], lvl_w + mul24z(2 * m + h, in_w), s);
      else {
        s[0] = (int)pf[slot][h][0].x; s[1] = (int)pf[slot][h][0].y; s[2] = (int)pf[slot][h][0].z; s[3] = (int)pf[slot][h][0].w;
        s[4] = (int)pf[slot][h][NQ - 1].x; s[5] = (int)pf[slot][h][NQ - 1].y; s[6] = (int)pf[slot][h][NQ - 1].z; s[7] = (int)pf[slot][h][NQ - 1].w;
      }
#pragma unroll
      for (int k = 0; k < 4; ++k) { r[k] = (int)((unsigned)s[2 * k] << ACC); r[4 + k] = (int)((unsigned)s[2 * k + 1] << ACC); }
    }
  };

  const int bshA = p.fh[comp] >> 1, bswA = p.fw[comp] >> 1, lbshA = ilog2d(bshA), bnA = bshA * bswA;
  const int bshB = bshA >> 1, bswB = bswA >> 1, lbshB = lbshA - 1, bnB = bshB * bswB;
  const int b_last = pb.ll_to_store;
  const int run0A = p.coef_off[comp] + bnA, run0B = pb.coef_off[comp] + (b_last ? 0 : bnB);
  const int ssA = pp.ss_a[comp], ssB = pp.ss_b[comp];
  const int llps = p.st_llps[comp];
  const int si = spl == 1 ? (lane - sp.lo) >> llps : (lane - sp.lo) * spl;
  const int cl = spl == 1 ? (lane - sp.lo) & ((1 << llps) - 1) : 0;
  ST *store = (ST *)p.store + (size_t)pic * p.store_stride;
  int32_t *wide = S_::narrow ? p.store_wide + (size_t)pic * p.store_stride : nullptr;
  ST *llp = nullptr;
  int32_t *llp_w = nullptr;
  const int owB = in_w >> 2;
  if (!b_last) {
    llp = (ST *)pb.ll[comp] + (size_t)pic * pb.ll_stride[comp] + (size_t)chunk * 2;
    if constexpr (S_::narrow) llp_w = pb.ll_wide[comp] + (size_t)pic * pb.ll_stride[comp] + (size_t)chunk * 2;
  }
  const int baseA = si * ssA + cl * 4, baseB = si * ssB + cl * 2;
  auto escapes = [&](int *v, auto NBc, auto NVc, int sv, int run0, int bn, int off_r, int clv) __attribute__((always_inline)) {
    constexpr int NB = decltype(NBc)::value, NV = decltype(NVc)::value, H = NV / 2;
    if constexpr (S_::narrow) {
      int32_t *w0 = wide + mul24z(sv * xs + sp.sx0 + si, slice_coefs) + run0 + off_r + (spl == 1 ? clv : 0);
      int32_t *w1 = spl == 1 ? w0 + H : w0 + slice_coefs;
#pragma unroll
      for (int b = 0; b < NB; ++b, w0 += bn, w1 += bn)
#pragma unroll
        for (int j = 0; j < NV; ++j)
          if (!S_::fits(v[b * NV + j])) { (j < H ? w0 : w1)[j % H] = v[b * NV + j]; v[b * NV + j] = VC2_ST_SENTINEL; }
    }
  };
  auto stageA = [&](ST *img, int r, int sv, const RowT<4> &oe, const RowT<4> &oo) __attribute__((always_inline)) {
    int v[12] = {oe[4], oe[5], oe[6], oe[7], oo[0], oo[1], oo[2], oo[3], oo[4], oo[5], oo[6], oo[7]};
    if constexpr (S_::narrow) {
      int mx = v[0], mn = v[0];
#pragma unroll
      for (int j = 1; j < 12; ++j) { mx = max(mx, v[j]); mn = min(mn, v[j]); }
      if (__builtin_expect(mx > 32767 || mn < -32767, 0)) escapes(v, IC<3>(), IC<4>(), sv, run0A, bnA, r * bswA, cl * 4);
    }
    ST *d = img + baseA + r * bswA;
#pragma unroll
    for (int b = 0; b < 3; ++b, d += bnA) {
      if constexpr (S_::narrow) {
        const unsigned w0 = vc2_pack16(v[4 * b], v[4 * b + 1]), w1 = vc2_pack16(v[4 * b + 2], v[4 * b + 3]);
        if (spl == 1) *(uint2 *)d = make_uint2(w0, w1);
        else { *(unsigned *)d = w0; *(unsigned *)(d + ssA) = w1; }
      } else {
        if (spl == 1) *(int4 *)d = make_int4(v[4 * b], v[4 * b + 1], v[4 * b + 2], v[4 * b + 3]);
        else { *(int2 *)d = make_int2(v[4 * b], v[4 * b + 1]); *(int2 *)(d + ssA) = make_int2(v[4 * b + 2], v[4 * b + 3]); }
      }
    }
  };
  auto stageB = [&](ST *img, int r, int sv, const RowT<2> &oe, const RowT<2> &oo) __attribute__((always_inline)) {
    int v[8] = {oe[0], oe[1], oe[2], oe[3], oo[0], oo[1], oo[2], oo[3]};
    if constexpr (S_::narrow) {
      int mx = v[2], mn = v[2];
#pragma unroll
      for (int j = 3; j < 8; ++j) { mx = max(mx, v[j]); mn = min(mn, v[j]); }
      if (b_last) { mx = max(mx, max(v[0], v[1])); mn = min(mn, min(v[0], v[1])); }
      if (__builtin_expect(mx > 32767 || mn < -32767, 0)) {
        if (b_last) escapes(v, IC<4>(), IC<2>(), sv, run0B, bnB, r * bswB, cl * 2);
        else escapes(v + 2, IC<3>(), IC<2>(), sv, run0B, bnB, r * bswB, cl * 2);
      }
    }
    ST *d = img + baseB + r * bswB;
#pragma unroll
    for (int b = 0; b < 4; ++b) {
      if (b == 0 && !b_last) continue;
      if constexpr (S_::narrow) {
        if (spl == 1) *(unsigned *)d = vc2_pack16(v[2 * b], v[2 * b + 1]);
        else { *d = (ST)v[2 * b]; *(d + ssB) = (ST)v[2 * b + 1]; }
      } else {
        if (spl == 1) *(int2 *)d = make_int2(v[2 * b], v[2 * b + 1]);
        else { *d = (ST)v[2 * b]; *(d + ssB) = (ST)v[2 * b + 1]; }
      }
      d += bnB;
    }
  };
  auto flush = [&](const ST *img, int ss, int run0, int run_n, int piece, int sv) __attribute__((always_inline)) {
    const int epp = piece / (int)sizeof(ST), ppr = run_n / epp;
    ST *rec0 = store + mul24z(sv * xs + sp.sx0, slice_coefs) + run0;
    const bool nt = FIRST && VC2_PAIR_NT && piece == 16 && (((run0 | run_n | slice_coefs) * (int)sizeof(ST)) & 127) == 0;
    if (ppr <= 64) {
      const int spt = 64 / ppr;
      int ls = (int)((float)lane * (1.0f / (float)ppr));
      ls -= ls * ppr > lane ? 1 : 0;
      ls += (ls + 1) * ppr <= lane ? 1 : 0;
      const int e = (lane - ls * ppr) * epp;
      const ST *src = img + ls * ss + e;
      ST *dst = rec0 + mul24z(ls, slice_coefs) + e;
      const int dsrc = spt * ss;
      const size_t ddst = mul24z(spt, slice_coefs);
#pragma unroll 1
      for (int s2 = ls; s2 < sp.nsl; s2 += spt, src += dsrc, dst += ddst) {
        if (ls < spt) {
          if (piece == 16) { if (nt) st_nt(dst, *(const uint4 *)src); else *(uint4 *)dst = *(const uint4 *)src; }
          else if (piece == 8) *(uint2 *)dst = *(const uint2 *)src;
          else *(unsigned *)dst = *(const unsigned *)src;
        }
      }
    } else {
#pragma unroll 1
      for (int s2 = 0; s2 < sp.nsl; ++s2) {
        const ST *src = img + s2 * ss;
        ST *dst = rec0 + mul24z(s2, slice_coefs);
#pragma unroll 1
        for (int q = lane; q < ppr; q += 64) {
          if (piece == 16) { if (nt) st_nt(dst + q * epp, *(const uint4 *)(src + q * epp)); else *(uint4 *)(dst + q * epp) = *(const uint4 *)(src + q * epp); }
          else if (piece == 8) *(uint2 *)(dst + q * epp) = *(const uint2 *)(src + q * epp);
          else *(unsigned *)(dst + q * epp) = *(const unsigned *)(src + q * epp);
        }
      }
    }
  };

  EA engA;
  EB engB;
  engA.clear();
  engB.clear();
  const int kA = sp.kA, kB = sp.kB, kA1 = kA >> 1, kB1 = kB >> 1;
  const int want = (kA + 3 * SD) & ~1;
  const bool top = want <= 0;
  const bool bottom = kB >= npA;
  const int m0 = top ? 0 : bottom ? npA - ((npA - want + 7) & ~7) : want;
  const int mend = bottom ? npA : kB + 3 * OFFL;
  const int mload = npA - 1;
#pragma unroll
  for (int u = 0; u < PFP; ++u) fetch(min(m0 + u, mload), u);
  static_assert(8 % PFP == 0, "the prefetch ring shares the unrolled walk");
  const int sv0 = kA >> lbshA, sv1 = kB >> lbshA;
  int stA = sv0, dnA = sv0, stB = sv0, dnB = sv0, stL = kA1, dnL = kA1;
  int slotBs = 0, slotBf = 0;
  bool due = false;
  int llE[4] = {0, 0, 0, 0};
  int mb = m0;

  auto burst = [&]() __attribute__((always_inline)) {
    wave_sync();
#pragma unroll 1
    for (; stA < dnA; ++stA) if (!(dskip & 256)) flush(imgA + ((stA - sv0) & (grpA - 1)) * szA, ssA, run0A, 3 * bnA, pieceA, stA);
#pragma unroll 1
    for (; stB < dnB; ++stB) {
      if (!(dskip & 64)) flush(imgB + slotBf * szB, ssB, run0B, (b_last ? 4 : 3) * bnB, pieceB, stB);
      slotBf = slotBf == grpA ? 0 : slotBf + 1;
    }
    if (!b_last) {
#pragma unroll 1
      for (; stL < dnL; ++stL) {
        if (own && !(dskip & 128)) {
          ST *d = llp + mul24z(stL, owB);
          if constexpr (S_::narrow) *(unsigned *)d = ring_ll[(stL & (nll - 1)) * 64 + lane];
          else *(uint2 *)d = *(const uint2 *)(ring_ll + ((stL & (nll - 1)) * 64 + lane) * 2);
        }
      }
    }
    wave_sync();
    due = false;
  };
  auto deferred = [&]() __attribute__((always_inline)) { if (__builtin_expect(due, 0)) burst(); };
  auto emitB = [&](auto UBc, int k1) __attribute__((always_inline)) {
    constexpr int UB = decltype(UBc)::value;
    if (k1 >= kA1 && k1 < kB1) {
      const RowT<2> &oe = engB.template out<UB>(false), &oo = engB.template out<UB>(true);
      const int r = k1 & (bshB - 1), sv = k1 >> lbshB;
      if (!(dskip & 16)) {
        if (!b_last) {
          int a0 = oe[0], a1 = oe[1];
          if constexpr (S_::narrow) {
            if (__builtin_expect(own && (!S_::fits(a0) || !S_::fits(a1)), 0)) {
              int32_t *w = llp_w + mul24z(k1, owB);
              if (!S_::fits(a0)) { w[0] = a0; a0 = VC2_ST_SENTINEL; }
              if (!S_::fits(a1)) { w[1] = a1; a1 = VC2_ST_SENTINEL; }
            }
#if !(defined(VC2_PAIR_X) && (VC2_PAIR_X & 2))
            ring_ll[(k1 & (nll - 1)) * 64 + lane] = vc2_pack16(a0, a1);
#endif
          } else *(uint2 *)(ring_ll + ((k1 & (nll - 1)) * 64 + lane) * 2) = make_uint2((unsigned)a0, (unsigned)a1);
          dnL = k1 + 1;
        }
#if !(defined(VC2_PAIR_X) && (VC2_PAIR_X & 1))
        if (own) stageB(imgB + slotBs * szB, r, sv, oe, oo);
#endif
#if !(defined(VC2_PAIR_X) && (VC2_PAIR_X & 4))
        if (r == bshB - 1) {
          dnB = sv + 1;
          slotBs = slotBs == grpA ? 0 : slotBs + 1;
          if (sv + 1 == sv1) due = true;
        }
#endif
      }
    }
  };
  auto iter = [&](auto U0c, auto BMc, auto DRc) __attribute__((always_inline)) {
    constexpr int U0 = decltype(U0c)::value, BM = decltype(BMc)::value;
    constexpr bool DRAIN = decltype(DRc)::value;
    if constexpr (!DRAIN || U0 < OFFL) {
      constexpr int UA = U0 & 3;
      constexpr int MODEA = DRAIN ? 2 : (BM == 1 && U0 < 4) ? 1 : 0;
      const int m = DRAIN ? npA + U0 : mb + U0;
      RowT<4> re, ro;
      if constexpr (!DRAIN) {
        convert(min(m, mload), U0 % PFP, 0, re);
        convert(min(m, mload), U0 % PFP, 1, ro);
      }
      deferred();
      if constexpr (!DRAIN) {
        fetch(min(m + PFP, mload), U0 % PFP);
        h_lift<K, false, 4>(re, redge);
        h_lift<K, false, 4>(ro, redge);
      }
      engA.template step<UA, MODEA, (DRAIN ? U0 : UA)>(m, npA, re, ro);
      const int k = m - OFFL;
      const RowT<4> &oe = engA.template out<UA>(false), &oo = engA.template out<UA>(true);
      if (k >= kA && k < kB) {
        const int r = k & (bshA - 1), sv = k >> lbshA;
        if (!(dskip & 32)) {
          if (own) stageA(imgA + ((sv - sv0) & (grpA - 1)) * szA, r, sv, oe, oo);
          if (r == bshA - 1) {
            dnA = sv + 1;
            if (((sv + 1 - sv0) & (grpA - 1)) == 0 || sv + 1 == sv1) due = true;
          }
        }
      }
      constexpr bool KODD = ((U0 - OFFL) & 1) != 0;
      if constexpr (!KODD) {
#pragma unroll
        for (int j = 0; j < 4; ++j) llE[j] = oe[j];
      } else {
        constexpr int J = fdiv2(U0 - OFFL - 1);
        constexpr int UB = ((J % 4) + 4) % 4;
        constexpr bool SKIP = BM == 1 && J < 0;
        constexpr int MODEB = (BM == 1 && J >= 0 && J < 4) || (BM == 2 && J < 0) ? 1 : 0;
        if (!SKIP && !(dskip & 8)) {
          const int m1 = ((DRAIN ? npA : mb) >> 1) + J;
          RowT<2> re1, ro1;
          re1[0] = (int)((unsigned)llE[0] << ACC); re1[1] = (int)((unsigned)llE[2] << ACC);
          re1[2] = (int)((unsigned)llE[1] << ACC); re1[3] = (int)((unsigned)llE[3] << ACC);
          ro1[0] = (int)((unsigned)oe[0] << ACC); ro1[1] = (int)((unsigned)oe[2] << ACC);
          ro1[2] = (int)((unsigned)oe[1] << ACC); ro1[3] = (int)((unsigned)oe[3] << ACC);
          h_lift<K, false, 2>(re1, redge);
          h_lift<K, false, 2>(ro1, redge);
          engB.template step<UB, MODEB>(m1, npB, re1, ro1);
          emitB(IC<UB>(), m1 - OFFL);
        }
      }
    }
  };
  auto block = [&](auto BMc, auto DRc) __attribute__((always_inline)) {
    iter(IC<0>(), BMc, DRc); iter(IC<1>(), BMc, DRc); iter(IC<2>(), BMc, DRc); iter(IC<3>(), BMc, DRc);
    iter(IC<4>(), BMc, DRc); iter(IC<5>(), BMc, DRc); iter(IC<6>(), BMc, DRc); iter(IC<7>(), BMc, DRc);
  };
  if (top) {
    block(IC<1>(), BC<false>());
    mb += 8;
    block(IC<2>(), BC<false>());
    mb += 8;
  }
  const int prio0 = (int)(blockIdx.x >> 10);
  for (; mb < mend; mb += 8) {
    if (st_prio) pair_prio(st_prio, prio0, mb >> 3);
    block(IC<0>(), BC<false>());
  }
  if (bottom) {
    block(IC<0>(), BC<true>());
    auto drainB = [&](auto Dc) __attribute__((always_inline)) {
      constexpr int D = decltype(Dc)::value;
      if constexpr (D < OFFL) {
        deferred();
        RowT<2> none;
#pragma unroll
        for (int j = 0; j < 4; ++j) none[j] = 0;
        engB.template step<D, 2, D>(npB + D, npB, none, none);
        emitB(IC<D>(), npB + D - OFFL);
      }
    };
    drainB(IC<0>()); drainB(IC<1>()); drainB(IC<2>()); drainB(IC<3>());
  }
  burst();
#undef p
#undef pb
}

__device__ __forceinline__ int dequant_fullp(int v, int qf, int off) {
  if (v == 0) return 0;
  const unsigned mag = v < 0 ? 0u - (unsigned)v : (unsigned)v;
  int a = (int)(mag * (unsigned)qf);
  if (a > 0) a = (int)((unsigned)a + (unsigned)off);
  a = (int)((unsigned)a + 2u);
  a /= 4;
  return v < 0 ? (int)(0u - (unsigned)a) : a;
}

#ifndef VC2_PAIR_WPE_INV
#define VC2_PAIR_WPE_INV 2
#endif
#ifndef VC2_PAIR_PFI
#define VC2_PAIR_PFI 2
#endif
constexpr int PFQ = VC2_PAIR_PFI;
template <int K, bool FINAL, class ST, bool SPL2>
__global__ __launch_bounds__(64, (K == VC2HIP_DD137 || SPL2 ? 2 : VC2_PAIR_WPE_INV)) void k_inv_pair(const PairParams pp) {
  using S_ = St<ST>;
  using EA = VEng<K, true, 4>;
  using EB = VEng<K, true, 2>;
  using T = VT<K, true>;
  constexpr int OFFL = T::OFFL, SD = T::sum_dmin();
  constexpr int ACC = WT<K>::accuracy;
  __shared__ int qtab[360];
  __shared__ int rare[12 * 64];
  constexpr bool PARK = !SPL2 && VC2_PAIR_WPE_INV >= 3;
  __shared__ __attribute__((aligned(16))) int parked[PARK ? VEng<K, true, 2>::park_rows() * 64 * 4 : 4];
#define p pp.a
#define pb pp.b
  const int lane = threadIdx.x & 63;
  int comp, pic;
  Strip sp;
  if (!strip_of_block_h<pair_halo<K>()>(p, comp, pic, sp)) return;
  for (int i = lane; i < 120; i += 64) {
    const int qf = c_qsp.qf[i], off = c_qsp.off[i];
    qtab[i] = qf; qtab[120 + i] = off;
    qtab[240 + i] = (qf > 0 && qf < (1 << 24)) ? (int)min(((1u << 25) - (unsigned)off - 8u) / (unsigned)qf, 0x7FFFFFu) : -1;
  }
  wave_sync();
  const int spl = SPL2 ? pp.spl[comp] : 1;
  const int xs = p.xs, st_prio = p.st_prio, dequant = p.dequant;
#ifdef VC2HIP_ABLATE
  const int dskip = p.debug_skip;
#else
  constexpr int dskip = 0;
#endif
  const int out_h = p.in_h[comp], out_w = p.in_w[comp], npA = out_h >> 1, npB = npA >> 1, owA = out_w >> 1, owB = out_w >> 2;
  const int chunk = min(sp.c0 + lane, (out_w >> 3) - 1);
  const bool own = lane >= sp.lo && lane < sp.hi;
  const bool redge = sp.c0 + lane == (out_w >> 3) - 1 && lane != 63;
  const int bshA = p.fh[comp] >> 1, bswA = p.fw[comp] >> 1, lbshA = ilog2d(bshA), bnA = bshA * bswA;
  const int bshB = bshA >> 1, bswB = bswA >> 1, lbshB = lbshA - 1, bnB = bshB * bswB;
  const int llps = p.st_llps[comp];
  const int sx = spl == 1 ? chunk >> llps : chunk * 2;
  const int cl = spl == 1 ? chunk & ((1 << llps) - 1) : 0;
  const int b_last = pb.ll_from_store;
  const int rsA = p.rec_stride[comp], rsB = pb.rec_stride[comp];
  const int run0A = p.coef_off[comp] + bnA + cl * 4, run0B = pb.coef_off[comp] + (b_last ? 0 : bnB) + cl * 2;
  const long long bpA = p.bp_base[comp], bpB = pb.bp_base[comp];
  const ST *store = (const ST *)p.store + (size_t)pic * p.store_stride;
  const int32_t *wide = S_::narrow ? p.store_wide + (size_t)pic * p.store_stride : nullptr;
  const int32_t *qidx = p.qidx ? p.qidx + (size_t)pic * p.ys * xs : nullptr;
  const ST *llp = nullptr;
  const int32_t *llp_w = nullptr;
  if (!b_last) {
    llp = (const ST *)pb.ll[comp] + (size_t)pic * pb.ll_stride[comp];
    if constexpr (S_::narrow) llp_w = pb.ll_wide[comp] + (size_t)pic * pb.ll_stride[comp];
  }
  auto ldq = [&](const void *base, unsigned elem, auto tag) __attribute__((always_inline)) {
    using Q = decltype(tag);
    return *(const Q *)((const char *)base + (size_t)(elem * (unsigned)sizeof(ST)));
  };
  const int qmA = p.band, qmB = pb.band;
  const int qm0 = p.qmatrix[0];
  int qmxA[3], qmxB[3];
#pragma unroll
  for (int b = 0; b < 3; ++b) { qmxA[b] = p.qmatrix[qmA + b]; qmxB[b] = p.qmatrix[qmB + b]; }

  const unsigned bpA32 = (unsigned)bpA + (unsigned)chunk * 4, bpB32 = (unsigned)bpB + (unsigned)chunk * 2;
  auto atA = [&](int m, int b) __attribute__((always_inline)) -> unsigned {
    if (bpA >= 0) return bpA32 + __umul24((unsigned)((b - 1) * npA + m), (unsigned)owA);
    const int sv = m >> lbshA, r = m & (bshA - 1);
    return __umul24((unsigned)(sv * xs + sx), (unsigned)rsA) + (unsigned)(run0A + (b - 1) * bnA + r * bswA);
  };
  auto atB = [&](int m1, int b) __attribute__((always_inline)) -> unsigned {
    if (bpB >= 0 && b > 0) return bpB32 + __umul24((unsigned)((b - 1) * npB + m1), (unsigned)owB);
    const int sv = m1 >> lbshB, r = m1 & (bshB - 1);
    return __umul24((unsigned)(sv * xs + sx), (unsigned)rsB) + (unsigned)(run0B + (b - (b_last ? 0 : 1)) * bnB + r * bswB);
  };
  typedef typename std::conditional<S_::narrow, uint2, uint4>::type Q4;
  typedef typename std::conditional<S_::narrow, unsigned, uint2>::type Q2;
  typedef typename std::conditional<S_::narrow, unsigned short, unsigned>::type Q1;
  Q4 bqA[PFQ][3];
  Q2 bqB[4];
  const bool splitA = spl == 2 && bpA < 0, splitB = spl == 2 && bpB < 0;
  auto fetchA = [&](int m, int slot) __attribute__((always_inline)) {
#pragma unroll
    for (int b = 1; b < 4; ++b) {
      const unsigned q = atA(m, b);
      if (!splitA) bqA[slot][b - 1] = ldq(store, q, Q4());
      else {
        const Q2 lo = ldq(store, q, Q2()), hi = ldq(store, q + (unsigned)rsA, Q2());
        if constexpr (S_::narrow) bqA[slot][b - 1] = make_uint2(lo, hi);
        else bqA[slot][b - 1] = make_uint4(lo.x, lo.y, hi.x, hi.y);
      }
    }
  };
  auto fetchB = [&](int m1) __attribute__((always_inline)) {
// ... 229 lines not shown
#pragma unroll
    for (int r = 0; r < EB::park_rows(); ++r) *(int4 *)(parked + (r * 64 + lane) * 4) = make_int4(0, 0, 0, 0);
  }
  const int kA = sp.kA, kB = sp.kB;
  const int wantA = kA + SD;
  const int wantB = (wantA >> 1) + SD;
  const bool top = wantB <= 0;
  const bool bottom = kB >= npA;
  const int m0e = wantA & ~1;
  const int m0 = top ? 0 : bottom ? npA - ((npA - m0e + 7) & ~7) : m0e;
  const int mend = bottom ? npA : kB + OFFL;
  const int mloadA = npA - 1, mloadB = npB - 1;
  int pend_k = -1;
  Pend pe, po;
#pragma unroll
  for (int k = 0; k < OW; ++k) { pe.w[k] = 0; po.w[k] = 0; }
  int llO[4] = {0, 0, 0, 0};
  int mb = m0;

  auto stepB = [&](auto UBc, auto MODEc, auto Dc, int m1, bool prefetch, int (&llE)[4]) __attribute__((always_inline)) {
    constexpr int UB = decltype(UBc)::value, MODE = decltype(MODEc)::value, D = decltype(Dc)::value;
    RowT<2> re1, ro1;
    if constexpr (MODE != 2) {
      const int ml = min(max(m1, 0), mloadB), sv = ml >> lbshB;
      if (__builtin_expect(sv != svB_have, 0)) { load_qB(sv); svB_have = sv; }
      int v[8] = {0, 0, 0, 0, 0, 0, 0, 0};
      if (!(dskip & 16)) unpackB(ml, v);
      re1[0] = v[0]; re1[1] = v[1]; re1[2] = v[2]; re1[3] = v[3];
      ro1[0] = v[4]; ro1[1] = v[5]; ro1[2] = v[6]; ro1[3] = v[7];
      if (prefetch && !(dskip & 64)) fetchB(min(max(m1 + 1, 0), mloadB));
    } else {
#pragma unroll
      for (int j = 0; j < 4; ++j) { re1[j] = 0; ro1[j] = 0; }
    }
    if constexpr (PARK) engB.template unpark<((UB + 3) & 3)>(parked, lane);
    if (!(dskip & 128)) engB.template step<UB, MODE, D>(m1, npB, re1, ro1);
    RowT<2> oe = engB.template out<UB>(false), oo = engB.template out<UB>(true);
    if constexpr (PARK) engB.template park<UB>(parked, lane);
    if (!(dskip & 256)) {
      h_lift<K, true, 2>(oe, redge);
      h_lift<K, true, 2>(oo, redge);
    }
#pragma unroll
    for (int j = 0; j < 2; ++j) {
      int a = oe[j], b = oe[2 + j], c = oo[j], d = oo[2 + j];
      if (ACC) { a = (a + (1 << (ACC > 0 ? ACC - 1 : 0))) >> ACC; b = (b + (1 << (ACC > 0 ? ACC - 1 : 0))) >> ACC; c = (c + (1 << (ACC > 0 ? ACC - 1 : 0))) >> ACC; d = (d + (1 << (ACC > 0 ? ACC - 1 : 0))) >> ACC; }
      llE[2 * j] = a; llE[2 * j + 1] = b; llO[2 * j] = c; llO[2 * j + 1] = d;
    }
  };
  auto iter = [&](auto U0c, auto BMc, auto DRc) __attribute__((always_inline)) {
    constexpr int U0 = decltype(U0c)::value, BM = decltype(BMc)::value;
    constexpr bool DRAIN = decltype(DRc)::value;
    if constexpr (!DRAIN || U0 < OFFL) {
      constexpr int UA = U0 & 3;
      constexpr int MODEA = DRAIN ? 2 : (BM == 1 && U0 < 4) ? 1 : 0;
      const int m = DRAIN ? npA + U0 : mb + U0;
      int ll[4];
      if constexpr (!DRAIN && (U0 & 1) == 0) {
        constexpr int J = U0 / 2, UB = (J + OFFL) & 3;
        constexpr int DB = J + OFFL - 4;
        constexpr int MODEB = (BM == 1 && J + OFFL < 4) ? 1 : (BM == 3 && DB >= 0) ? 2 : 0;
#ifdef VC2_PAIR_NO_B
        ll[0] = ll[1] = ll[2] = ll[3] = 0;
#else
        if (!(dskip & 8)) stepB(IC<UB>(), IC<MODEB>(), IC<(MODEB == 2 ? DB : UB)>(), (mb >> 1) + J + OFFL, true, ll);
        else { ll[0] = ll[1] = ll[2] = ll[3] = 0; }
#endif
      } else {
#pragma unroll
        for (int j = 0; j < 4; ++j) ll[j] = llO[j];
      }
      RowT<4> re, ro;
      if constexpr (!DRAIN) {
        const int ml = min(m, mloadA), sv = ml >> lbshA;
        if (__builtin_expect(sv != svA_have, 0)) { load_qA(sv); svA_have = sv; }
        int v[12];
        unpackA(ml, U0 % PFQ, v);
#pragma unroll
        for (int j = 0; j < 4; ++j) { re[j] = ll[j]; re[4 + j] = v[j]; ro[j] = v[4 + j]; ro[4 + j] = v[8 + j]; }
      }
      if (pend_k >= 0) { put_out(2 * pend_k, pe); put_out(2 * pend_k + 1, po); }
      if constexpr (!DRAIN) fetchA(min(m + PFQ, mloadA), U0 % PFQ);
      engA.template step<UA, MODEA, (DRAIN ? U0 : UA)>(m, npA, re, ro);
      const int k = m - OFFL;
      if (k >= kA && k < kB) {
        RowT<4> oe = engA.template out<UA>(false), oo = engA.template out<UA>(true);
        make_out(2 * k, oe, pe);
        make_out(2 * k + 1, oo, po);
        pend_k = k;
      } else pend_k = -1;
    }
  };
  auto block = [&](auto BMc, auto DRc) __attribute__((always_inline)) {
    iter(IC<0>(), BMc, DRc); iter(IC<1>(), BMc, DRc); iter(IC<2>(), BMc, DRc); iter(IC<3>(), BMc, DRc);
    iter(IC<4>(), BMc, DRc); iter(IC<5>(), BMc, DRc); iter(IC<6>(), BMc, DRc); iter(IC<7>(), BMc, DRc);
  };
  {
    int none[4];
    auto pro = [&](auto Ic, auto TOPc) __attribute__((always_inline)) {
      constexpr int I = decltype(Ic)::value;
      constexpr bool TOP = decltype(TOPc)::value;
      constexpr int NPRO = TOP ? OFFL : OFFL - SD;
      if constexpr (I < NPRO) {
        constexpr int REL = OFFL - NPRO + I;
        constexpr int UB = ((REL % 4) + 4) % 4;
        const int m1 = (m0 >> 1) + REL;
        fetchB(min(max(m1, 0), mloadB));
        stepB(IC<UB>(), IC<(TOP ? 1 : 0)>(), IC<UB>(), m1, false, none);
      }
    };
    if (top) { pro(IC<0>(), BC<true>()); pro(IC<1>(), BC<true>()); pro(IC<2>(), BC<true>()); pro(IC<3>(), BC<true>()); }
    else {
      pro(IC<0>(), BC<false>()); pro(IC<1>(), BC<false>()); pro(IC<2>(), BC<false>()); pro(IC<3>(), BC<false>());
      pro(IC<4>(), BC<false>()); pro(IC<5>(), BC<false>()); pro(IC<6>(), BC<false>()); pro(IC<7>(), BC<false>());
    }
    fetchB(min((m0 >> 1) + OFFL, mloadB));
  }
#pragma unroll
  for (int u = 0; u < PFQ; ++u) fetchA(min(m0 + u, mloadA), u);
  static_assert(8 % PFQ == 0, "the prefetch ring shares the unrolled walk");
  if (top) {
    block(IC<1>(), BC<false>());
    mb += 8;
  }
  const int prio0 = (int)(blockIdx.x >> 10);
  const int mlast = bottom ? npA - 8 : mend;
  for (; mb < mlast; mb += 8) {
    if (st_prio) pair_prio(st_prio, prio0, mb >> 3);
    block(IC<0>(), BC<false>());
  }
  if (bottom) {
    if constexpr (OFFL > 0) block(IC<3>(), BC<false>());
    else block(IC<0>(), BC<false>());
    mb += 8;
    block(IC<0>(), BC<true>());
  }
  if (pend_k >= 0) { put_out(2 * pend_k, pe); put_out(2 * pend_k + 1, po); }
#undef p
#undef pb
}

#ifdef VC2HIP_ABLATE
#define VC2_PAIR_INV_EDGE true
#else
#define VC2_PAIR_INV_EDGE false
#endif
#ifdef VC2_PAIR_ONLY_INV
#define VC2_PAIR_HAS(INV, EDGE) ((INV) && (!(EDGE) || VC2_PAIR_INV_EDGE))
#elif defined(VC2_PAIR_ONLY_FWD)
#define VC2_PAIR_HAS(INV, EDGE) (!(INV))
#else
#define VC2_PAIR_HAS(INV, EDGE) (!(INV) || !(EDGE) || VC2_PAIR_INV_EDGE)
#endif
template <int K, bool EDGE, bool INV, class ST> const void *pair_fn(bool SPL2) {
  if constexpr (!pair_kernel<K>() || !VC2_PAIR_HAS(INV, EDGE)) return nullptr;
  else if constexpr (INV) return SPL2 ? (const void *)k_inv_pair<K, EDGE, ST, true> : (const void *)k_inv_pair<K, EDGE, ST, false>;
  else return (const void *)k_fwd_pair<K, EDGE, ST>;
}
template <int K, bool EDGE, bool INV, class ST>
int launch_pair(Launcher &L, const PairParams &pp, int n_pictures, size_t lds, hipStream_t s) {
  if constexpr (!pair_kernel<K>() || !VC2_PAIR_HAS(INV, EDGE)) return VC2HIP_EINVAL;
  else {
    const LevelParams &p = pp.a;
    const int cols = (p.st_strips[0] + p.st_strips[1] + p.st_strips[2]) * n_pictures;
    const int gx = ((cols + 7) / 8) * p.st_segmax * 8;
    dim3 grid(gx), block(64);
    if constexpr (INV) {
      vc2_prof_begin(L, EDGE ? "idwt_pair_final" : "idwt_pair", s);
      if (pp.spl[0] == 2 || pp.spl[1] == 2 || pp.spl[2] == 2) VC2_LAUNCH(L, (k_inv_pair<K, EDGE, ST, true>), grid, block, 0, s, pp);
      else VC2_LAUNCH(L, (k_inv_pair<K, EDGE, ST, false>), grid, block, 0, s, pp);
    } else {
      vc2_prof_begin(L, EDGE ? "dwt_pair_first" : "dwt_pair", s);
      vc2_allow_lds((const void *)k_fwd_pair<K, EDGE, ST>, std::max<size_t>(64 * 1024, lds));
      VC2_LAUNCH(L, (k_fwd_pair<K, EDGE, ST>), grid, block, lds, s, pp);
    }
    vc2_prof_end(L, s);
    return 0;
  }
}
template <int K, bool EDGE, bool INV, class ST> int pair_slots_of(size_t lds) {
  int nb = 0, dev = 0;
  hipDeviceProp_t prop;
  const void *fn = pair_fn<K, EDGE, INV, ST>(false);
  if (!fn) return 0;
  if (!INV) vc2_allow_lds(fn, std::max<size_t>(64 * 1024, lds));
  if (hipGetDevice(&dev) != hipSuccess || hipGetDeviceProperties(&prop, dev) != hipSuccess ||
      hipOccupancyMaxActiveBlocksPerMultiprocessor(&nb, fn, 64, INV ? 0 : lds) != hipSuccess || nb < 1)
    return 256 * 8;
  static const int whole = vc2_tune_int("VC2HIP_PAIR_WHOLE_SIMDS", 0);
  if (nb >= 4 && whole) nb &= ~3;
  return nb * prop.multiProcessorCount;
}
#ifdef VC2_PAIR_ONE
#define VC2_PAIR_CASES(X) X(VC2HIP_DD97)
#else
#define VC2_PAIR_CASES(X) X(VC2HIP_DD97) X(VC2HIP_LEGALL) X(VC2HIP_DD137) X(VC2HIP_HAAR0) X(VC2HIP_HAAR1)
#endif
template <bool INV, class ST> int pair_dispatch(Launcher &L, int kernel, bool edge, const PairParams &pp, int n, size_t lds, hipStream_t s) {
#define VC2_CASE(KK) case KK: return edge ? launch_pair<KK, true, INV, ST>(L, pp, n, lds, s) : launch_pair<KK, false, INV, ST>(L, pp, n, lds, s);
  switch (kernel) { VC2_PAIR_CASES(VC2_CASE) }
#undef VC2_CASE
  return VC2HIP_EINVAL;
}
template <bool INV, class ST> int pair_slots_dispatch(int kernel, bool edge, size_t lds) {
#define VC2_CASE(KK) case KK: return edge ? pair_slots_of<KK, true, INV, ST>(lds) : pair_slots_of<KK, false, INV, ST>(lds);
  switch (kernel) { VC2_PAIR_CASES(VC2_CASE) }
#undef VC2_CASE
  return 0;
}
int pair_slots(int kernel, bool edge, bool inverse, bool store16, size_t lds) {
  static std::mutex mu;
  static std::map<std::tuple<int, int, int, int, size_t, int>, int> cache;
  int dev = 0;
  (void)hipGetDevice(&dev);
  const auto key = std::make_tuple(kernel, (int)edge, (int)inverse, (int)store16, lds, dev);
  std::lock_guard<std::mutex> lock(mu);
  auto it = cache.find(key);
  if (it != cache.end()) return it->second;
  int v;
  if (!store16) v = 0;
  else if (inverse) v = pair_slots_dispatch<true, int16_t>(kernel, edge, lds);
  else v = pair_slots_dispatch<false, int16_t>(kernel, edge, lds);
  cache[key] = v;
  return v;
}
struct PairTaps { int halo, offl, sd; };
template <int K> constexpr PairTaps taps_of(bool inv) {
  return inv ? PairTaps{pair_halo<K>(), VT<K, true>::OFFL, VT<K, true>::sum_dmin()} : PairTaps{pair_halo<K>(), VT<K, false>::OFFL, VT<K, false>::sum_dmin()};
}
bool pair_taps(int kernel, bool inv, PairTaps &t) {
  switch (kernel) {
#define VC2_CASE(KK) case KK: t = taps_of<KK>(inv); return true;
    VC2_PAIR_CASES(VC2_CASE)
#undef VC2_CASE
  }
  return false;
}
bool pow2p(int v) { return v > 0 && (v & (v - 1)) == 0; }
int spl_of(int fw) { return fw >= 8 ? 1 : 2; }
int ilog2h(int v) { return 31 - __builtin_clz((unsigned)v); }

int image_stride(int run_elems, int elem, int lps, int spl, int vals) {
  const int base = (run_elems * elem + 15) & ~15;
  int best = base, best_cost = 1 << 30;
  for (int pad = 0; pad <= 256; pad += 16) {
    const int ss = base + pad;
    int bank[64] = {0};
    for (int l = 0; l < 64; ++l)
      for (int q = 0; q < spl; ++q) {
        const int slice = spl == 1 ? l / lps : l * spl + q;
        const int off = spl == 1 ? (l % lps) * vals * elem : 0;
        const int bytes = std::max(4, vals / spl * elem);
        for (int b = 0; b < bytes; b += 4) ++bank[((slice * ss + off + b) >> 2) & 63];
      }
    int cost = 0;
    for (int b = 0; b < 64; ++b) cost = std::max(cost, bank[b]);
    if (cost < best_cost) { best_cost = cost; best = ss; }
  }
  return best / elem;
}

}

size_t vc2_pair_applicable(PairParams &pp, int kernel, bool edge, bool inverse, bool store16, int n_pictures) {
  PairTaps t;
  if (!pair_taps(kernel, inverse, t)) return 0;
  LevelParams &p = pp.a;
  const LevelParams &pb = pp.b;
  const int elem = store16 ? 2 : 4;
  const bool b_last = inverse ? pb.ll_from_store != 0 : pb.ll_to_store != 0;
  if (inverse && (p.bp8 || pb.bp8)) return 0;
  if (!store16) return 0;
  size_t imgA = 16, imgB = 16;
  p.st_tail = 0;
  p.st_segmax = 0;
  for (int c = 0; c < 3; ++c) {
    p.st_strips[c] = p.st_segs[c] = 0;
    pp.spl[c] = 1;
    if (p.tiles_x[c] == 0 || p.tiles_y[c] == 0) continue;
    const int w = p.in_w[c], h = p.in_h[c], fw = p.fw[c], fh = p.fh[c];
    if (w < VC2_STREAM_MIN_W || (w & 7) || (h & 3) || h < 48) return 0;
    if (edge && (p.word_bytes != 2 || p.pic_w[c] != w)) return 0;
    if (!pow2p(fw) || !pow2p(fh) || fw < 4 || fh < 4 || fw > 64 * 8) return 0;
    if (pb.fw[c] * 2 != fw || pb.fh[c] * 2 != fh || pb.in_w[c] * 2 != w || pb.in_h[c] * 2 != h) return 0;
    const int spl = fw >= 8 ? 1 : 2, lps = fw >= 8 ? fw / 8 : 1;
    const int bnA = (fh / 2) * (fw / 2), bnB = (fh / 4) * (fw / 4);
    const int runA = 3 * bnA, runB = (b_last ? 4 : 3) * bnB;
    const int pieceA = std::min(16, bnA * elem), pieceB = std::min(16, (b_last ? 4 * bnB : bnB) * elem);
    if (!inverse) {
      if (pieceA < 4 || pieceB < 4) return 0;
      if ((p.coef_off[c] * elem) % 16 || (pb.coef_off[c] * elem) % 16 || (p.slice_coefs * elem) % 16) return 0;
    } else {
      if ((p.coef_off[c] | pb.coef_off[c] | p.rec_stride[c] | pb.rec_stride[c] | bnA) & 3) return 0;
      if ((bnB & 1) && !(bnB == 1 && b_last && spl_of(fw) == 2)) return 0;
    }
    pp.piece_a[c] = pieceA;
    pp.piece_b[c] = pieceB;
    pp.spl[c] = spl;
    static const int out_cap = vc2_tune_int("VC2HIP_PAIR_OUT", 64);
    const int out = (std::min(64 - 2 * t.halo, out_cap) / lps) * lps;
    if (out < lps) return 0;
    const int nch = w / 8;
    p.st_out[c] = out;
    p.st_llps[c] = ilog2h(lps);
    p.st_strips[c] = (nch + out - 1) / out;
    const int nsl = out / lps * spl;
    pp.ss_a[c] = image_stride(runA, elem, lps, spl, 4);
    pp.ss_b[c] = (runB * elem + 15) / 16 * 16 / elem;
    imgA = std::max(imgA, (size_t)nsl * pp.ss_a[c] * elem);
    imgB = std::max(imgB, (size_t)nsl * pp.ss_b[c] * elem);
  }
  if (inverse) imgA = imgB = 0;
  imgA = (imgA + 15) & ~(size_t)15;
  imgB = (imgB + 15) & ~(size_t)15;
  int bsh_min = 1 << 20, bshb_max = 1;
  for (int c = 0; c < 3; ++c) if (p.st_strips[c]) { bsh_min = std::min(bsh_min, p.fh[c] / 2); bshb_max = std::max(bshb_max, p.fh[c] / 4); }
  int grp = 1;
  auto lds_of = [&](int g) {
    int nll = 4;
    while (nll < g * bshb_max) nll *= 2;
    return (size_t)g * imgA + (size_t)(g + 1) * imgB + (b_last ? 0 : (size_t)nll * 64 * (store16 ? 4 : 8));
  };
  while (grp * 2 * bsh_min <= 8 && lds_of(grp * 2) <= 20 * 1024) grp *= 2;
  static const int force_grp = vc2_tune_int("VC2HIP_PAIR_GROUP", 0);
  if (force_grp > 0) grp = force_grp;
  int nll = 4;
  while (nll < grp * bshb_max) nll *= 2;
  pp.grp_a = grp;
  pp.sz_a = (int)(imgA / elem);
  pp.sz_b = (int)(imgB / elem);
  pp.img_b = (int)(grp * imgA);
  pp.ring_ll = (int)(grp * imgA + (grp + 1) * imgB);
  pp.n_ll = nll;
  const size_t lds = inverse ? 16 : lds_of(grp);
  if (lds > 48 * 1024) return 0;
  int cols = 0;
  for (int c = 0; c < 3; ++c) if (p.st_strips[c]) cols += p.st_strips[c] * n_pictures;
  const int slots = pair_slots(kernel, edge, inverse, store16, lds);
  if (slots <= 0) return 0;
  const int runin = -3 * t.sd + 3 * t.offl + 8;
  int nseg = 0;
  long long best = -1;
  for (int g = 1; g <= p.ys; ++g) {
    bool ok = true;
    int tallest = 0;
    for (int c = 0; c < 3 && ok; ++c) {
      if (!p.st_strips[c]) continue;
      const int bsh = p.fh[c] / 2, np = p.in_h[c] / 2;
      tallest = std::max(tallest, ((p.ys + g - 1) / g) * bsh);
      if (g == 1) { ok = np % 8 == 0; continue; }
      const int ka_bottom = (int)((long long)(g - 1) * p.ys / g) * bsh;
      if (np - ka_bottom < 3 * t.offl) ok = false;
      if (ka_bottom + 3 * t.sd - 8 < 0) ok = false;
    }
    if (!ok) continue;
    const long long rounds = ((long long)cols * g + slots - 1) / slots;
    const long long cost = rounds * ((long long)tallest + runin);
    if (best < 0 || cost <= best) { best = cost; nseg = g; }
  }
  if (!nseg) return 0;
  {
    static const int f = vc2_tune_int("VC2HIP_PAIR_NSEG", 0), fe = vc2_tune_int("VC2HIP_PAIR_NSEG_EDGE", 0);
    if (f > 0) nseg = std::min(f, p.ys);
    if (fe > 0 && edge) nseg = std::min(fe, p.ys);
  }
  for (int c = 0; c < 3; ++c) if (p.st_strips[c]) p.st_segs[c] = nseg;
  p.st_segmax = nseg;
  p.st_npic = n_pictures;
  static const int prio = vc2_tune_int("VC2HIP_PAIR_PRIO", 1);
  p.st_prio = prio;
  p.st_lds = (int)lds;
#ifdef VC2HIP_ABLATE
  if (getenv("VC2HIP_PAIR_DEBUG")) fprintf(stderr, "pair: kernel %d edge %d lds %zu (img a %zu) slots %d cols %d nseg %d runin %d\n", kernel, (int)edge, lds, imgA, slots, cols, nseg, runin);
#endif
  return lds;
}
int vc2_launch_forward_pair(Launcher &L, int kernel, bool first, const PairParams &pp, int n, bool store16, size_t lds, hipStream_t s) {
  return store16 ? pair_dispatch<false, int16_t>(L, kernel, first, pp, n, lds, s) : VC2HIP_EINVAL;
}
int vc2_launch_inverse_pair(Launcher &L, int kernel, bool final_level, const PairParams &pp, int n, bool store16, size_t lds, hipStream_t s) {
  return store16 ? pair_dispatch<true, int16_t>(L, kernel, final_level, pp, n, lds, s) : VC2HIP_EINVAL;
}
```

vc2-reference_amd/csrc/vc2hip_internal.h:

```cpp
#pragma once

#include <hip/hip_runtime.h>
#include <hip/hip_ext.h>
#include <stddef.h>
#include <stdint.h>

#include "../../include/vc2hip.h"

#define VC2_MAX_DEPTH 7
#define VC2_MAX_BANDS (3 * VC2_MAX_DEPTH + 1)

enum : unsigned {
  VC2_DEVERR_QINDEX = 1u << 0,
  VC2_DEVERR_SCALAR = 1u << 1,
  VC2_DEVERR_CBR_TOOBIG = 1u << 2,
  VC2_DEVERR_CBR_LEN = 1u << 3,
  VC2_DEVERR_CODE32 = 1u << 4,
  VC2_DEVERR_STREAM = 1u << 5,
  VC2_DEVERR_LD_TOOBIG = 1u << 6,
  VC2_DEVERR_HANDOFF = 1u << 7,
  VC2_DEVERR_CAP = 1u << 8,
  VC2_DEVERR_SYNTAX = 1u << 9,
};
#define VC2_ERRBLK_SYNTAX_AT 8
#define VC2_ERRBLK_SYNTAX_WHY 16
#define VC2_ERRBLK_COPY 32
enum {
  VC2_SYN_PREFIX = 1, VC2_SYN_CODE, VC2_SYN_PAST_END, VC2_SYN_NEXT_ZERO, VC2_SYN_FEWER, VC2_SYN_PARAMS, VC2_SYN_QUANT_MATRIX,
  VC2_SYN_ASYMMETRIC, VC2_SYN_NO_VERSION, VC2_SYN_FRAGMENT, VC2_SYN_COUNT
};

struct CompGeom {
  int h, w;
  int ph, pw;
  int sh, sw;
  int coef_off;
  int n0;
};

struct Geom {
  CompGeom c[3];
  int depth, ys, xs;
  int slice_coefs;
};

__host__ __device__ inline int band_offset(int n0, int band) {
  if (band == 0) return 0;
  const int L = (band - 1) / 3 + 1, kind = (band - 1) % 3;
  return n0 * ((1 << (2 * (L - 1))) * (1 + kind));
}
__host__ __device__ inline int band_of_index(int j, int n0) {
  const int m = j / n0;
  if (m == 0) return 0;
#if defined(__HIP_DEVICE_COMPILE__)
  const int lg = 31 - __clz(m);
#else
  const int lg = 31 - __builtin_clz((unsigned)m);
#endif
  const int L = lg / 2 + 1;
  return 3 * (L - 1) + (m >> (2 * (L - 1)));
}

struct QuantTables {
  int32_t qf[120];
  int32_t off[120];
  uint32_t magic[120];
  int32_t shift[120];
  float inv4[120];
};

struct LevelParams {
  void *plane[3];
  long long plane_stride[3];
  void *ll[3];
  long long ll_stride[3];
  void *store;
  long long store_stride;
  int32_t *store_wide;
  int32_t *plane_wide[3];
  int32_t *ll_wide[3];
  const int32_t *qidx;
  int in_h[3], in_w[3];
  int pic_h[3], pic_w[3];
  int fh[3], fw[3];
  int tsy[3], tsx[3];
  int tiles_y[3], tiles_x[3];
  int coef_off[3];
  int band_off[3];
  int band_n[3];
  int band;
  int ys, xs, slice_coefs;
  int rec_stride[3];
  int word_bytes, sample_shift, sample_offset;
  int sample_shift_c, sample_offset_c;
  int clip_lo, clip_hi;
  int ll_from_store;
  int ll_to_store;
  int dequant;
  unsigned *err;
  int debug_skip;
  int qmatrix[VC2_MAX_BANDS];
  int st_strips[3], st_segs[3];
  int st_out[3];
  int st_llps[3];
  int st_tail;
  int st_prio;
  int st_segmax, st_npic;
  int st_lds;
  long long bp_base[3];
  int bp8;
};

struct PairParams {
  LevelParams a, b;
  int spl[3];
  int img_b;
  int grp_a;
  int sz_a, sz_b;
  int ring_ll, n_ll;
  int ss_a[3], ss_b[3];
  int piece_a[3], piece_b[3];
};

#include <stdlib.h>
#ifdef VC2HIP_ABLATE
static inline int vc2_tune_int(const char *name, int def) { const char *e = getenv(name); return e ? atoi(e) : def; }
#else
static inline int vc2_tune_int(const char *, int def) { return def; }
#endif

#ifdef VC2HIP_ABLATE
#define VC2_SKIP(p, bit) (((p).debug_skip & (bit)) != 0)
#else
#define VC2_SKIP(p, bit) false
#endif

struct PackParams {
  const void *store;
  const int32_t *store_wide;
  int store16;
  long long store_stride;
  const int32_t *qidx;
  int n_slices, slice_coefs;
  int comp_n[3], comp_off[3], comp_n0[3];
  int depth;
  int prefix, scalar;
  int qmatrix[VC2_MAX_BANDS];
  uint8_t *slots;
  int slot_bytes;
  uint32_t *sizes;
  int tile_slices;
  const int32_t *cbr_bytes;
  const uint32_t *cbr_offsets;
  uint8_t *payload;
  long long payload_stride;
  unsigned *err;
  int quantise;
  int big_lut;
  float inv_scalar;
  union {
    unsigned char band_lut[768];
    unsigned lane16[200];
  };
  int debug_skip;
  unsigned long long *lookback;
  long long lookback_stride;
  unsigned long long *lens;
};

constexpr int VC2_BP_MAX = 3;
struct BandPlanes {
  int levels;
  int bytes8;
  int from[3];
  long long base[3][VC2_BP_MAX];
  int ow[3][VC2_BP_MAX], np[3][VC2_BP_MAX];
  int lbsh[3][VC2_BP_MAX], lbsw[3][VC2_BP_MAX];
};

struct HeadSplit {
  int n[3];
  long long base[3];
};

struct UnpackParams {
  const uint8_t *payload;
  long long payload_stride;
  const unsigned long long *lens;
  const uint32_t *offsets;
  void *store;
  int32_t *store_wide;
  int store16;
  long long store_stride;
  int32_t *qidx;
  int n_slices, slice_coefs;
  int comp_n[3], comp_off[3];
  int prefix, scalar;
  unsigned *err;
  BandPlanes bp;
  HeadSplit hs;
  int xs;
  unsigned long long *stats;
  int debug_skip;
};

struct CbrParams {
  const void *store;
  const int32_t *store_wide;
  int store16;
  long long store_stride;
  int32_t *qidx;
  const int32_t *slice_bytes;
  int n_slices, slice_coefs;
  int comp_n[3], comp_off[3], comp_n0[3];
  int scalar;
  int n_bands;
  int qmatrix[VC2_MAX_BANDS];
  unsigned *err;
  int only_marked;
  int general_only;
  float inv_scalar;
  int qm_min;
  union {
    unsigned char band_lut[768];
    unsigned lane8[72];
  };
};
#define VC2_CBR_MARK 0x7FFFFFFF

struct Launcher;
void vc2_prof_pair(Launcher &L, hipEvent_t *a, hipEvent_t *b);
#define VC2_LAUNCH(L, kernel, grid, block, lds, s, ...)                                        \
  do {                                                                                         \
    hipEvent_t vc2_ev_a_, vc2_ev_b_;                                                           \
    vc2_prof_pair(L, &vc2_ev_a_, &vc2_ev_b_);                                                  \
    hipExtLaunchKernelGGL(kernel, grid, block, lds, s, vc2_ev_a_, vc2_ev_b_, 0, __VA_ARGS__);  \
  } while (0)

void vc2_allow_lds(const void *kernel, size_t bytes);

void vc2_upload_tables(const QuantTables &t, hipStream_t s);
int vc2_launch_forward_level(Launcher &L, int kernel, bool first, const LevelParams &p, int n_pictures,
                             hipStream_t s);
int vc2_launch_inverse_level(Launcher &L, int kernel, bool final_level, const LevelParams &p,
                             int n_pictures, hipStream_t s);
size_t vc2_level_lds_bytes(int kernel, const LevelParams &p);

void vc2_launch_pack(Launcher &L, const PackParams &p, int n_pictures, hipStream_t s);
int vc2_pack_slices_per_tile(const PackParams &p);
bool vc2_pack_one_pass_default(const PackParams &p);
void vc2_launch_scan_sizes(Launcher &L, const uint32_t *sizes, uint32_t *offsets,
                           unsigned long long *totals, int n_slices, int n_pictures, hipStream_t s);
void vc2_launch_compact(Launcher &L, const uint8_t *slots, int slot_bytes, const uint32_t *sizes,
                        const uint32_t *offsets, uint8_t *payload, long long payload_stride,
                        int n_slices, int n_pictures, hipStream_t s);
void vc2_launch_cbr(Launcher &L, const CbrParams &p, int n_pictures, hipStream_t s);
void vc2_launch_unpack(Launcher &L, const UnpackParams &p, int n_pictures, hipStream_t s);
void vc2_launch_cbr_index(Launcher &L, const uint8_t *payload, long long stride, const unsigned long long *lens, const int32_t *budget,
                          const uint32_t *cbr_offs, unsigned long long total, uint32_t *offsets, int n_slices, int prefix, int scalar,
                          int n_pictures, unsigned *bad, hipStream_t s);
void vc2_launch_slice_index(Launcher &L, const uint8_t *payload, long long payload_stride,
                            const unsigned long long *lens, uint32_t *offsets, int n_slices,
                            int prefix, int scalar, int n_pictures, unsigned *err, hipStream_t s,
                            void *workspace, size_t workspace_bytes, const unsigned *skip = nullptr);
size_t vc2_slice_index_workspace(int n_pictures, size_t max_payload, int prefix, int scalar);

void vc2_launch_plane_to_store(Launcher &L, const int32_t *plane, int ph, int pw, int depth, int ys,
                               int xs, int32_t *store, int slice_coefs, int coef_off, hipStream_t s);
void vc2_launch_store_to_plane(Launcher &L, const int32_t *store, int slice_coefs, int coef_off,
                               int32_t *plane, int ph, int pw, int depth, int ys, int xs,
                               const int32_t *qidx, const int *qmatrix, int mode ,
                               unsigned *err, hipStream_t s);
void vc2_launch_quantise_store(Launcher &L, int32_t *store, int n_slices, int slice_coefs, int comp_n,
                               int comp_off, int n0, const int32_t *qidx, const int *qmatrix,
// ... 99 lines not shown
```

vc2-reference_amd/csrc/vc2hip_stream_eng.h:

```cpp
#pragma once

#ifndef VC2_STREAM_MIN_W
#define VC2_STREAM_MIN_W 192
#endif
#ifndef VC2_STREAM_PF
#define VC2_STREAM_PF 2
#endif
constexpr int PF = VC2_STREAM_PF;
#ifndef VC2_STREAM_PFI
#define VC2_STREAM_PFI 1
#endif
constexpr int PFI = VC2_STREAM_PFI;

template <int NP> struct RowT {
  int v[2 * NP];
  __device__ __forceinline__ int &operator[](int i) { return v[i]; }
  __device__ __forceinline__ const int &operator[](int i) const { return v[i]; }
};
using Row = RowT<4>;
template <int NP> __device__ __forceinline__ RowT<NP> operator+(const RowT<NP> &a, const RowT<NP> &b) { RowT<NP> r; _Pragma("unroll") for (int i = 0; i < 2 * NP; ++i) r.v[i] = a.v[i] + b.v[i]; return r; }
template <int NP> __device__ __forceinline__ RowT<NP> operator-(const RowT<NP> &a, const RowT<NP> &b) { RowT<NP> r; _Pragma("unroll") for (int i = 0; i < 2 * NP; ++i) r.v[i] = a.v[i] - b.v[i]; return r; }
template <int NP> __device__ __forceinline__ RowT<NP> operator-(const RowT<NP> &a) { RowT<NP> r; _Pragma("unroll") for (int i = 0; i < 2 * NP; ++i) r.v[i] = -a.v[i]; return r; }
template <int NP> __device__ __forceinline__ RowT<NP> operator+(const RowT<NP> &a, int b) { RowT<NP> r; _Pragma("unroll") for (int i = 0; i < 2 * NP; ++i) r.v[i] = a.v[i] + b; return r; }
template <int NP> __device__ __forceinline__ RowT<NP> operator*(int b, const RowT<NP> &a) { RowT<NP> r; _Pragma("unroll") for (int i = 0; i < 2 * NP; ++i) r.v[i] = b * a.v[i]; return r; }
template <int NP> __device__ __forceinline__ RowT<NP> operator>>(const RowT<NP> &a, int b) { RowT<NP> r; _Pragma("unroll") for (int i = 0; i < 2 * NP; ++i) r.v[i] = a.v[i] >> b; return r; }
template <int NP> __device__ __forceinline__ RowT<NP> vc2_times9(const RowT<NP> &a) { RowT<NP> r; _Pragma("unroll") for (int i = 0; i < 2 * NP; ++i) r.v[i] = ::vc2_times9(a.v[i]); return r; }

template <int CTRL> __device__ __forceinline__ int dppm(int old, int v) {
  return __builtin_amdgcn_update_dpp(old, v, CTRL, 0xf, 0xf, false);
}
typedef int vc2_nt4_t __attribute__((ext_vector_type(4)));
typedef int vc2_nt2_t __attribute__((ext_vector_type(2)));
__device__ __forceinline__ void st_nt(void *p, uint4 v) {
  const vc2_nt4_t x = {(int)v.x, (int)v.y, (int)v.z, (int)v.w};
  __builtin_nontemporal_store(x, (__attribute__((address_space(1))) vc2_nt4_t *)(size_t)p);
}
__device__ __forceinline__ void st_nt(void *p, uint2 v) {
  const vc2_nt2_t x = {(int)v.x, (int)v.y};
  __builtin_nontemporal_store(x, (__attribute__((address_space(1))) vc2_nt2_t *)(size_t)p);
}
__device__ __forceinline__ void st_nt(void *p, unsigned v) { __builtin_nontemporal_store((int)v, (__attribute__((address_space(1))) int *)(size_t)p); }

__device__ __forceinline__ void wave_sync() {
  __builtin_amdgcn_fence(__ATOMIC_RELEASE, "wavefront");
  __builtin_amdgcn_wave_barrier();
  __builtin_amdgcn_fence(__ATOMIC_ACQUIRE, "wavefront");
}

template <int K> constexpr int kdmin(int s) {
  return s == 0 ? step_dmin<K, 0>() : s == 1 ? step_dmin<K, 1>() : s == 2 ? step_dmin<K, 2>() : step_dmin<K, 3>();
}
template <int K> constexpr int kdmax(int s) {
  return s == 0 ? step_dmax<K, 0>() : s == 1 ? step_dmax<K, 1>() : s == 2 ? step_dmax<K, 2>() : step_dmax<K, 3>();
}
template <int K> constexpr bool kodd(int s) {
  return s == 0 ? step_targets_odd<K, 0>() : s == 1 ? step_targets_odd<K, 1>() : s == 2 ? step_targets_odd<K, 2>() : step_targets_odd<K, 3>();
}
template <int K, int NP = 4> constexpr int halo_lanes() {
  int l = 0, r = 0;
  for (int s = 0; s < WT<K>::nsteps; ++s) { l -= kdmin<K>(s); r += kdmax<K>(s); }
  return ((l > r ? l : r) + NP - 1) / NP;
}
template <int K, int NP> constexpr bool reach_fits() {
  for (int s = 0; s < WT<K>::nsteps; ++s) if (-kdmin<K>(s) > NP || kdmax<K>(s) > NP) return false;
  return true;
}

template <int K, int S, bool INV, int NP> __device__ __forceinline__ void h_step(RowT<NP> &r, bool redge) {
  constexpr bool odd = step_targets_odd<K, S>();
  constexpr int dmin = step_dmin<K, S>(), dmax = step_dmax<K, S>();
  static_assert(-dmin <= NP && dmax <= NP, "taps beyond the adjacent lane");
  constexpr int TO = odd ? NP : 0, UO = odd ? 0 : NP;
  int W[NP + dmax - dmin];
#pragma unroll
  for (int j = dmin; j <= NP - 1 + dmax; ++j) {
    if (j < 0) W[j - dmin] = dppm<0x138>(r[UO], r[UO + NP + j]);
    else if (j > NP - 1) {
      const int nb = dppm<0x130>(r[UO + NP - 1], r[UO + j - NP]);
      W[j - dmin] = redge ? r[UO + NP - 1] : nb;
    } else W[j - dmin] = r[UO + j];
  }
#pragma unroll
  for (int i = 0; i < NP; ++i) {
    const int d = lift_delta<K, S>([&](int t) -> int { return W[i + t - dmin]; });
    r[TO + i] = INV ? r[TO + i] - d : r[TO + i] + d;
  }
}
template <int K, bool INV, int NP> __device__ __forceinline__ void h_lift(RowT<NP> &r, bool redge) {
  constexpr int N = WT<K>::nsteps;
  if constexpr (!INV) {
    h_step<K, 0, false, NP>(r, redge);
    h_step<K, 1, false, NP>(r, redge);
    if constexpr (N == 4) { h_step<K, 2, false, NP>(r, redge); h_step<K, 3, false, NP>(r, redge); }
  } else {
    if constexpr (N == 4) { h_step<K, 3, true, NP>(r, redge); h_step<K, 2, true, NP>(r, redge); }
    h_step<K, 1, true, NP>(r, redge);
    h_step<K, 0, true, NP>(r, redge);
  }
}

template <int K, bool INV> struct VT {
  static constexpr int N = WT<K>::nsteps;
  static constexpr int sid(int p) { return INV ? N - 1 - p : p; }
  static constexpr int dmin(int p) { return kdmin<K>(sid(p)); }
  static constexpr int dmax(int p) { return kdmax<K>(sid(p)); }
  static constexpr bool odd(int p) { return kodd<K>(sid(p)); }
  static constexpr int off(int p) { int s = 0; for (int t = 0; t <= p; ++t) s += dmax(t); return s; }
  static constexpr int sum_dmin() { int s = 0; for (int t = 0; t < N; ++t) s += dmin(t); return s; }
  static constexpr int OFFL = off(N - 1);
  static constexpr int mx(int a, int b) { return a > b ? a : b; }
  static constexpr int len_raw(bool parity_odd) {
    if (parity_odd == odd(0)) return off(0) + 1;
    return mx(dmax(0) - dmin(0), N >= 2 ? off(1) : 0) + 1;
  }
  static constexpr int len_x(int p) {
    int d = 0;
    if (p + 1 < N) d = mx(d, dmax(p + 1) - dmin(p + 1));
    if (p + 2 < N) d = mx(d, dmax(p + 1) + dmax(p + 2));
    if (p >= N - 2) d = mx(d, off(N - 1) - off(p));
    return d + 1;
  }
};

template <int K> constexpr int RLK = K == VC2HIP_FIDELITY ? 8 : 4;
template <int K, bool INV, int NP = 4> struct VEng {
  using T = VT<K, INV>;
  using Row = RowT<NP>;
  static constexpr int RL = RLK<K>;
  static_assert(T::len_raw(false) <= RL && T::len_raw(true) <= RL && T::len_x(0) <= RL && T::len_x(1) <= RL &&
                (T::N < 3 || (T::len_x(2) <= RL && T::len_x(3) <= RL)), "row ring too short for this wavelet");
  Row rw[2][RL];
  Row x[4][RL];
  static constexpr int sl(int rel) { return ((rel % RL) + RL) % RL; }

  __device__ __forceinline__ void clear() {
#pragma unroll
    for (int j = 0; j < RL; ++j)
#pragma unroll
      for (int k = 0; k < 2 * NP; ++k) { rw[0][j].v[k] = 0; rw[1][j].v[k] = 0; x[0][j].v[k] = 0; x[1][j].v[k] = 0; x[2][j].v[k] = 0; x[3][j].v[k] = 0; }
  }
  template <int SLOT> static __device__ __forceinline__ void put(Row (&w)[RL], const Row &r, bool first) {
#pragma unroll
    for (int k = 0; k < 2 * NP; ++k) w[SLOT].v[k] = r.v[k];
    if (first) {
#pragma unroll
      for (int j = 0; j < RL; ++j)
        if (j != SLOT) {
#pragma unroll
          for (int k = 0; k < 2 * NP; ++k) w[j].v[k] = r.v[k];
        }
    }
  }
  template <int SRC, int DST> static __device__ __forceinline__ void copy(Row (&w)[RL]) {
#pragma unroll
    for (int k = 0; k < 2 * NP; ++k) w[DST].v[k] = w[SRC].v[k];
  }
  template <int U, int P, int MODE, int D> __device__ __forceinline__ void pos(int m, int np) {
    if constexpr (P < T::N) {
      constexpr int dst = sl(U - T::off(P));
      constexpr int dmin = T::dmin(P), dmax = T::dmax(P);
      if constexpr (MODE == 2 && (D + 1 > T::off(P))) copy<sl(U - T::off(P) - 1), dst>(x[P]);
      else {
        Row W[dmax - dmin + 1];
#pragma unroll
        for (int t = dmin; t <= dmax; ++t) {
          if constexpr (P == 0) W[t - dmin] = rw[T::odd(0) ? 0 : 1][sl(U - T::off(P) + t)];
          else W[t - dmin] = x[P - 1][sl(U - T::off(P) + t)];
        }
        const Row d = lift_delta<K, T::sid(P)>([&](int t) -> Row { return W[t - dmin]; });
        Row o;
        if constexpr (P < 2) o = rw[T::odd(P) ? 1 : 0][dst];
        else o = x[P - 2][dst];
        put<dst>(x[P], INV ? o - d : o + d, MODE == 1 && U == T::off(P));
      }
      pos<U, P + 1, MODE, D>(m, np);
    }
  }
  template <int U, int MODE, int D = U> __device__ __forceinline__ void step(int m, int np, const Row &re, const Row &ro) {
    if constexpr (MODE == 2) { copy<sl(U - 1), U>(rw[0]); copy<sl(U - 1), U>(rw[1]); }
    else { put<U>(rw[0], re, MODE == 1 && U == 0); put<U>(rw[1], ro, MODE == 1 && U == 0); }
    pos<U, 0, MODE, D>(m, np);
  }
  static constexpr int park_rows() { int n = T::len_raw(false) + T::len_raw(true); for (int p = 0; p < T::N; ++p) n += T::len_x(p); return n; }
  template <int U, bool STORE> __device__ __forceinline__ void park_io(int *area, int lane) {
    int r = 0;
    auto io = [&](Row &row) __attribute__((always_inline)) {
      int *q = area + (r * 64 + lane) * 2 * NP;
      ++r;
      static_assert(NP == 2 || NP == 4, "16- or 32-byte rows");
      if constexpr (STORE) {
        *(int4 *)q = make_int4(row.v[0], row.v[1], row.v[2], row.v[3]);
        if constexpr (NP == 4) *(int4 *)(q + 4) = make_int4(row.v[4], row.v[5], row.v[6], row.v[7]);
      } else {
        const int4 a = *(const int4 *)q;
        row.v[0] = a.x; row.v[1] = a.y; row.v[2] = a.z; row.v[3] = a.w;
        if constexpr (NP == 4) { const int4 b = *(const int4 *)(q + 4); row.v[4] = b.x; row.v[5] = b.y; row.v[6] = b.z; row.v[7] = b.w; }
      }
    };
#pragma unroll
    for (int par = 0; par < 2; ++par)
#pragma unroll
      for (int j = 0; j < RL; ++j) if (j < T::len_raw(par == 1)) io(rw[par][sl(U - j)]);
#pragma unroll
    for (int p = 0; p < 4; ++p)
#pragma unroll
      for (int j = 0; j < RL; ++j) if (p < T::N && j < T::len_x(p < T::N ? p : 0)) io(x[p][sl(U - T::off(p < T::N ? p : 0) - j)]);
  }
  template <int U> __device__ __forceinline__ void park(int *area, int lane) { park_io<U, true>(area, lane); }
  template <int U> __device__ __forceinline__ void unpark(int *area, int lane) { park_io<U, false>(area, lane); }
  template <int U> __device__ __forceinline__ const Row &out(bool odd_row) const {
    constexpr int N = T::N, s = sl(U - T::OFFL);
    if (T::odd(N - 1) == odd_row) return x[N - 1][s];
    return x[N - 2][s];
  }
};

struct Strip {
  int c0;
  int lo, hi;
  int nsl, sx0;
  int kA, kB;
};
#ifndef VC2_STREAM_WG_WAVES
#define VC2_STREAM_WG_WAVES 1
#endif
__device__ __forceinline__ int stream_wave() { return VC2_STREAM_WG_WAVES > 1 ? __builtin_amdgcn_readfirstlane((int)(threadIdx.x >> 6)) : 0; }
__device__ __forceinline__ int stream_item() {
  if (VC2_STREAM_WG_WAVES == 1) return (int)blockIdx.x;
  const int g = (int)blockIdx.x;
  return 8 * (VC2_STREAM_WG_WAVES * (g >> 3) + stream_wave()) + (g & 7);
}
template <int HLN> __device__ __forceinline__ bool strip_of_block_h(const LevelParams &p, int &comp, int &pic, Strip &s) {
  const int b = stream_item(), x = b & 7, t = b >> 3;
  const int seg = t % p.st_segmax, col = (t / p.st_segmax) * 8 + x;
  const int n0 = p.st_npic * p.st_strips[0], n1 = p.st_npic * p.st_strips[1], n2 = p.st_npic * p.st_strips[2];
  int within;
  if (col < n0) { comp = 0; within = col; }
  else if (col < n0 + n1) { comp = 1; within = col - n0; }
  else if (col < n0 + n1 + n2) { comp = 2; within = col - n0 - n1; }
  else return false;
  if (seg >= p.st_segs[comp]) return false;
  pic = within / p.st_strips[comp];
  const int strip = within - pic * p.st_strips[comp];
  const int nch = p.in_w[comp] >> 3, out = p.st_out[comp];
  s.c0 = max(min(max(strip * out - HLN, 0), nch - 64), 0);
  s.lo = strip * out - s.c0;
  s.hi = min((strip + 1) * out, nch) - s.c0;
  s.nsl = (s.hi - s.lo) >> p.st_llps[comp];
  s.sx0 = (strip * out) >> p.st_llps[comp];
  const int bsh = p.fh[comp] >> 1;
  s.kA = (int)(__umul24(seg, p.ys) / (unsigned)p.st_segmax) * bsh;
  s.kB = (int)(__umul24(seg + 1, p.ys) / (unsigned)p.st_segmax) * bsh;
  return true;
}

__device__ __forceinline__ void prio_turn(int v) {
  switch (v & 3) {
    case 0: __builtin_amdgcn_s_setprio(0); break;
    case 1: __builtin_amdgcn_s_setprio(1); break;
    case 2: __builtin_amdgcn_s_setprio(2); break;
    default: __builtin_amdgcn_s_setprio(3); break;
  }
}
__device__ __forceinline__ int ilog2d(int v) { return 31 - __clz(v); }
__device__ __forceinline__ size_t mul24z(int a, int b) { return (size_t)__umul24((unsigned)a, (unsigned)b); }

template <int K> __device__ __forceinline__ bool strip_of_block(const LevelParams &p, int &comp, int &pic, Strip &s) {
  return strip_of_block_h<halo_lanes<K>()>(p, comp, pic, s);
}
```

vc2-reference_amd/csrc/vc2hip_wavelets.h:

```cpp
#pragma once
#include "vc2hip_internal.h"

template <int K> struct WT;
template <> struct WT<VC2HIP_DD97>     { static constexpr int nsteps = 2, accuracy = 1, halo = 4; };
template <> struct WT<VC2HIP_LEGALL>   { static constexpr int nsteps = 2, accuracy = 1, halo = 2; };
template <> struct WT<VC2HIP_DD137>    { static constexpr int nsteps = 2, accuracy = 1, halo = 6; };
template <> struct WT<VC2HIP_HAAR0>    { static constexpr int nsteps = 2, accuracy = 0, halo = 0; };
template <> struct WT<VC2HIP_HAAR1>    { static constexpr int nsteps = 2, accuracy = 1, halo = 0; };
template <> struct WT<VC2HIP_FIDELITY> { static constexpr int nsteps = 2, accuracy = 0, halo = 14; };
template <> struct WT<VC2HIP_DAUB97>   { static constexpr int nsteps = 4, accuracy = 1, halo = 4; };

template <int K, int S> __device__ __forceinline__ constexpr bool step_targets_odd() {
  if constexpr (K == VC2HIP_FIDELITY) return S == 1;
  else return (S % 2) == 0;
}

__device__ __forceinline__ int vc2_times9(int x) { return (int)(((unsigned)x << 3) + (unsigned)x); }
template <class T> __device__ __forceinline__ T vc2_times9(const T &x) { const T d = x + x, q = d + d; return q + q + x; }

template <int K, int S, class F> __device__ __forceinline__ auto lift_delta(F at) {
  if constexpr (K == VC2HIP_DD97 || K == VC2HIP_DD137) {
    if constexpr (S == 0) return -((vc2_times9(at(0) + at(1)) - (at(-1) + at(2)) + 8) >> 4);
    else if constexpr (K == VC2HIP_DD97) return (at(-1) + at(0) + 2) >> 2;
    else return (vc2_times9(at(-1) + at(0)) - (at(-2) + at(1)) + 16) >> 5;
  } else if constexpr (K == VC2HIP_LEGALL) {
    if constexpr (S == 0) return -((at(0) + at(1) + 1) >> 1);
    else return (at(-1) + at(0) + 2) >> 2;
  } else if constexpr (K == VC2HIP_HAAR0 || K == VC2HIP_HAAR1) {
    if constexpr (S == 0) return -at(0);
    else return (at(0) + 1) >> 1;
  } else if constexpr (K == VC2HIP_FIDELITY) {
    if constexpr (S == 0)
      return (-8 * at(-4) + 21 * at(-3) - 46 * at(-2) + 161 * at(-1) + 161 * at(0) - 46 * at(1) +
              21 * at(2) - 8 * at(3) + 128) >> 8;
    else
      return -((-2 * at(-3) + 10 * at(-2) - 25 * at(-1) + 81 * at(0) + 81 * at(1) - 25 * at(2) +
                10 * at(3) - 2 * at(4) + 128) >> 8);
  } else {
    if constexpr (S == 0) return -((6497 * at(0) + 6497 * at(1) + 2048) >> 12);
    else if constexpr (S == 1) return -((217 * at(-1) + 217 * at(0) + 2048) >> 12);
    else if constexpr (S == 2) return (3616 * at(0) + 3616 * at(1) + 2048) >> 12;
    else return (1817 * at(-1) + 1817 * at(0) + 2048) >> 12;
  }
}

template <int K> __host__ __device__ constexpr int halo_y() { return WT<K>::halo; }
template <int K> __host__ __device__ constexpr int halo_x() { return (WT<K>::halo + 7) & ~7; }


template <int K, int S> __host__ __device__ constexpr int step_dmin() {
  if constexpr (K == VC2HIP_DD97) return S == 0 ? -1 : -1;
  else if constexpr (K == VC2HIP_LEGALL) return S == 0 ? 0 : -1;
  else if constexpr (K == VC2HIP_DD137) return S == 0 ? -1 : -2;
  else if constexpr (K == VC2HIP_HAAR0 || K == VC2HIP_HAAR1) return 0;
  else if constexpr (K == VC2HIP_FIDELITY) return S == 0 ? -4 : -3;
  else return (S % 2 == 0) ? 0 : -1;
}
template <int K, int S> __host__ __device__ constexpr int step_dmax() {
  if constexpr (K == VC2HIP_DD97) return S == 0 ? 2 : 0;
  else if constexpr (K == VC2HIP_LEGALL) return S == 0 ? 1 : 0;
  else if constexpr (K == VC2HIP_DD137) return S == 0 ? 2 : 1;
  else if constexpr (K == VC2HIP_HAAR0 || K == VC2HIP_HAAR1) return 0;
  else if constexpr (K == VC2HIP_FIDELITY) return S == 0 ? 3 : 4;
  else return (S % 2 == 0) ? 1 : 0;
}
```

vc2-reference_amd/vc2hip_py.py:

```python
import ctypes as C
import os

import numpy as np

HERE = os.path.dirname(os.path.abspath(__file__))
LIB_PATH = os.environ.get("VC2HIP_LIB") or os.path.join(HERE, "libvc2hip.so")

i32p = np.ctypeslib.ndpointer(dtype=np.int32, flags="C_CONTIGUOUS")
u8p = np.ctypeslib.ndpointer(dtype=np.uint8, flags="C_CONTIGUOUS")

FLAGS = {"STORE32": 0x001, "NO_STREAM": 0x002, "NO_PAIR": 0x004, "NO_BANDPLANES": 0x008, "NO_HEADS": 0x010, "NO_CBR_INDEX": 0x020,
         "GENERIC_DWT": 0x040, "SINGLE_PASS_VBR": 0x080, "CBR_GENERAL": 0x100, "LD_DIAGONALS": 0x200,
         "PLANES8_ALWAYS": 0x400, "PLANES8_NEVER": 0x800, "TWO_PASS_VBR": 0x1000}

KERNELS = {"DD97": 0, "LeGall": 1, "DD137": 2, "Haar0": 3, "Haar1": 4, "Fidelity": 5, "Daub97": 6}
CF = {"444": 0, "422": 1, "420": 2}
MODES = {"HQ_ConstQ": 0, "HQ_CBR": 1, "LD": 2}


class Geom(C.Structure):
    _fields_ = [("luma_h", C.c_int), ("luma_w", C.c_int), ("chroma_h", C.c_int),
                ("chroma_w", C.c_int), ("depth", C.c_int), ("y_slices", C.c_int),
                ("x_slices", C.c_int)]


class PictureFormat(C.Structure):
    _fields_ = [("width", C.c_int), ("height", C.c_int), ("chroma_format", C.c_int),
                ("bit_depth", C.c_int), ("word_bytes", C.c_int), ("chroma_bit_depth", C.c_int)]


class CodingParams(C.Structure):
    _fields_ = [("kernel", C.c_int), ("depth", C.c_int), ("y_slices", C.c_int),
                ("x_slices", C.c_int), ("mode", C.c_int), ("q_index", C.c_int),
                ("compressed_bytes", C.c_int), ("prefix", C.c_int), ("scalar", C.c_int)]


class DwtLaunch(C.Structure):
    _fields_ = [("inverse", C.c_int), ("level", C.c_int), ("levels", C.c_int), ("family", C.c_int), ("edge", C.c_int),
                ("store_bits", C.c_int), ("segments", C.c_int), ("tail", C.c_int), ("small_gather", C.c_int),
                ("pictures", C.c_int), ("band_planes", C.c_int)]


class StreamParams(C.Structure):
    _fields_ = [("major_version", C.c_int), ("first_picture_number", C.c_uint32), ("prev_parse_offset", C.c_uint32),
                ("end_of_sequence", C.c_int)]


DWT_FAMILIES = ("tile", "fast", "stream", "pair", "plane")


class Vc2HipError(RuntimeError):
    def __init__(self, code, msg):
        super().__init__(msg)
        self.code = code


EXPORTS = [
    "vc2hip_create", "vc2hip_create_with_flags", "vc2hip_create_on_stream", "vc2hip_destroy", "vc2hip_last_error",
    "vc2hip_error_string", "vc2hip_sync", "vc2hip_padded_size", "vc2hip_slice_size_is_valid",
    "vc2hip_quant_matrix", "vc2hip_slice_bytes", "vc2hip_dwt_forward", "vc2hip_dwt_inverse",
    "vc2hip_quantise_np", "vc2hip_dequantise_np", "vc2hip_dequantise_ld", "vc2hip_hq_pack",
    "vc2hip_hq_unpack", "vc2hip_ld_unpack", "vc2hip_cbr_qindices", "vc2hip_quantise_ld", "vc2hip_ld_pack",
    "vc2hip_ld_qindices", "vc2hip_encode_picture_ld", "vc2hip_set_streams", "vc2hip_raw_picture_bytes",
    "vc2hip_max_payload_bytes", "vc2hip_encode_picture_hq", "vc2hip_decode_picture_hq",
    "vc2hip_decode_picture_ld", "vc2hip_encode_batch_dev", "vc2hip_decode_batch_dev",
    "vc2hip_profile_enable", "vc2hip_profile_only", "vc2hip_profile_count", "vc2hip_profile_get", "vc2hip_profile_reset",
    "vc2hip_host_alloc", "vc2hip_host_free", "vc2hip_encode_picture_begin", "vc2hip_encode_picture_end",
    "vc2hip_decode_picture_begin", "vc2hip_decode_picture_end", "vc2hip_band_plane_bits", "vc2hip_dwt_launches",
    "vc2hip_picture_header", "vc2hip_stream_write_dev", "vc2hip_stream_read_dev",
]


def load_library():
    if not os.path.exists(LIB_PATH):
        raise RuntimeError(f"{LIB_PATH} is missing: run `python -c 'import __graft_entry__ as g; g.build()'` "
                           "(there is no CPU fallback)")
    if os.environ.get("VC2HIP_NO_TORCH") != "1":
        try:
            import torch
        except Exception:
            pass
    lib = C.CDLL(LIB_PATH)
    vp = C.c_void_p
    lib.vc2hip_create.argtypes = [C.c_int, C.POINTER(vp)]
    lib.vc2hip_create_with_flags.argtypes = [C.c_int, C.c_uint, C.POINTER(vp)]
    lib.vc2hip_create_on_stream.argtypes = [C.c_int, vp, C.POINTER(vp)]
    lib.vc2hip_destroy.argtypes = [vp]
    lib.vc2hip_destroy.restype = None
    lib.vc2hip_last_error.argtypes = [vp]
    lib.vc2hip_last_error.restype = C.c_char_p
    lib.vc2hip_error_string.argtypes = [C.c_int]
    lib.vc2hip_error_string.restype = C.c_char_p
    lib.vc2hip_sync.argtypes = [vp]
    lib.vc2hip_set_streams.argtypes = [vp, C.c_int]
    lib.vc2hip_quant_matrix.argtypes = [C.c_int, C.c_int, i32p]
    lib.vc2hip_slice_bytes.argtypes = [C.c_int, C.c_int, C.c_int, C.c_int, i32p]
    lib.vc2hip_dwt_forward.argtypes = [vp, i32p, C.c_int, C.c_int, C.c_int, C.c_int, i32p]
    lib.vc2hip_dwt_inverse.argtypes = [vp, i32p, C.c_int, C.c_int, C.c_int, C.c_int, i32p, C.c_int, C.c_int]
    for f in (lib.vc2hip_quantise_np, lib.vc2hip_dequantise_np, lib.vc2hip_dequantise_ld, lib.vc2hip_quantise_ld):
        f.argtypes = [vp, i32p, C.c_int, C.c_int, C.c_int, i32p, C.c_int, C.c_int, i32p, i32p]
    lib.vc2hip_hq_pack.argtypes = [vp, i32p, i32p, i32p, C.POINTER(Geom), i32p, C.c_int, C.c_int,
                                   vp, u8p, C.c_size_t, C.POINTER(C.c_size_t)]
    lib.vc2hip_hq_unpack.argtypes = [vp, u8p, C.c_size_t, C.POINTER(Geom), C.c_int, C.c_int, i32p,
                                     i32p, i32p, i32p, C.POINTER(C.c_size_t)]
    lib.vc2hip_ld_unpack.argtypes = [vp, u8p, C.c_size_t, C.POINTER(Geom), i32p, i32p, i32p, i32p,
                                     i32p, C.POINTER(C.c_size_t)]
    lib.vc2hip_cbr_qindices.argtypes = [vp, i32p, i32p, i32p, C.POINTER(Geom), i32p, i32p, C.c_int, i32p]
    lib.vc2hip_ld_qindices.argtypes = [vp, i32p, i32p, i32p, C.POINTER(Geom), i32p, i32p, i32p]
    lib.vc2hip_ld_pack.argtypes = [vp, i32p, i32p, i32p, C.POINTER(Geom), i32p, i32p, u8p, C.c_size_t,
                                   C.POINTER(C.c_size_t)]
    lib.vc2hip_raw_picture_bytes.argtypes = [C.POINTER(PictureFormat)]
    lib.vc2hip_raw_picture_bytes.restype = C.c_size_t
    lib.vc2hip_max_payload_bytes.argtypes = [C.POINTER(PictureFormat), C.POINTER(CodingParams)]
    lib.vc2hip_max_payload_bytes.restype = C.c_size_t
    for f in (lib.vc2hip_encode_picture_hq, lib.vc2hip_encode_picture_ld):
        f.argtypes = [vp, u8p, C.POINTER(PictureFormat), C.POINTER(CodingParams), u8p, C.c_size_t,
                      C.POINTER(C.c_size_t), vp]
    for f in (lib.vc2hip_decode_picture_hq, lib.vc2hip_decode_picture_ld):
        f.argtypes = [vp, u8p, C.c_size_t, C.POINTER(PictureFormat), C.POINTER(CodingParams), u8p]
    lib.vc2hip_encode_batch_dev.argtypes = [vp, vp, C.c_int, C.POINTER(PictureFormat),
                                            C.POINTER(CodingParams), vp, C.c_size_t, vp]
    lib.vc2hip_decode_batch_dev.argtypes = [vp, vp, C.c_size_t, vp, C.c_int, C.POINTER(PictureFormat),
                                            C.POINTER(CodingParams), vp]
    lib.vc2hip_picture_header.argtypes = [C.POINTER(CodingParams), C.c_int, C.c_uint32, u8p, C.c_size_t,
                                          C.POINTER(C.c_size_t)]
    lib.vc2hip_stream_write_dev.argtypes = [vp, vp, C.c_size_t, vp, C.c_int, C.POINTER(CodingParams), C.POINTER(StreamParams),
                                            vp, C.c_size_t, vp]
    lib.vc2hip_stream_read_dev.argtypes = [vp, vp, C.c_size_t, C.c_int, C.POINTER(CodingParams), C.POINTER(StreamParams),
                                           vp, C.c_size_t, vp, vp, vp]
    lib.vc2hip_profile_enable.argtypes = [vp, C.c_int]
    lib.vc2hip_profile_only.argtypes = [vp, C.c_char_p]
    lib.vc2hip_profile_count.argtypes = [vp]
    lib.vc2hip_profile_get.argtypes = [vp, C.c_int, C.POINTER(C.c_char_p), C.POINTER(C.c_int),
                                       C.POINTER(C.c_double)]
    lib.vc2hip_profile_reset.argtypes = [vp]
    lib.vc2hip_band_plane_bits.argtypes = [vp]
    lib.vc2hip_dwt_launches.argtypes = [vp, C.POINTER(DwtLaunch), C.c_int]
    lib.vc2hip_host_alloc.argtypes = [C.c_size_t]
    lib.vc2hip_host_alloc.restype = vp
    lib.vc2hip_host_free.argtypes = [vp]
    lib.vc2hip_host_free.restype = None
    lib.vc2hip_encode_picture_begin.argtypes = [vp, vp, C.POINTER(PictureFormat), C.POINTER(CodingParams), vp, C.c_size_t, vp,
                                                C.POINTER(C.c_int)]
    lib.vc2hip_encode_picture_end.argtypes = [vp, C.c_int, C.POINTER(C.c_size_t)]
    lib.vc2hip_decode_picture_begin.argtypes = [vp, vp, C.c_size_t, C.POINTER(PictureFormat), C.POINTER(CodingParams), vp,
                                                C.POINTER(C.c_int)]
    lib.vc2hip_decode_picture_end.argtypes = [vp, C.c_int]
    return lib


def picture_format(width, height, cf, bits, word_bytes=2, chroma_bits=0):
    return PictureFormat(width, height, CF[cf], bits, word_bytes, chroma_bits)


def coding_params(lib, fmt, kernel, depth, u, a, mode="HQ_ConstQ", q=0, s=0, prefix=0, scalar=1):
    ch = fmt.height // 2 if fmt.chroma_format == 2 else fmt.height
    cw = fmt.width if fmt.chroma_format == 0 else fmt.width // 2
    ys = lib.vc2hip_slice_size_is_valid(depth, fmt.height, ch, u)
    xs = lib.vc2hip_slice_size_is_valid(depth, fmt.width, cw, a)
    if not ys or not xs:
        raise ValueError("The given waveletDepth, hSlice, and vSlice parameters cannot encode this input.")
    return CodingParams(KERNELS[kernel], depth, ys, xs, MODES[mode], q, s, prefix, scalar)


def stream_params(major_version=2, first_picture_number=0, prev_parse_offset=0, end_of_sequence=False):
    return StreamParams(major_version, first_picture_number & 0xFFFFFFFF, prev_parse_offset, int(end_of_sequence))


def picture_header(lib, cp, major_version, picture_number):
    out = np.zeros(64, np.uint8)
    n = C.c_size_t()
    rc = lib.vc2hip_picture_header(C.byref(cp), major_version, picture_number & 0xFFFFFFFF, out, out.size, C.byref(n))
    if rc != 0:
        raise Vc2HipError(rc, lib.vc2hip_error_string(rc).decode())
    return out[:n.value].tobytes()


class Vc2Hip:

    def __init__(self, device=0, stream=None, flags=0):
        self.lib = load_library()
        h = C.c_void_p()
        if stream is not None and flags:
            raise ValueError("vc2hip_create_on_stream takes no flags: give either a stream or flags")
        if stream is None and flags:
            rc = self.lib.vc2hip_create_with_flags(device, C.c_uint(flags), C.byref(h))
        elif stream is None:
            rc = self.lib.vc2hip_create(device, C.byref(h))
        else:
            rc = self.lib.vc2hip_create_on_stream(device, C.c_void_p(stream), C.byref(h))
        if rc != 0:
            raise Vc2HipError(rc, "vc2hip_create failed: " + self.lib.vc2hip_error_string(rc).decode()
                              + " (a MI355X is required; there is no CPU fallback)")
        self.h = h

    def close(self):
        if getattr(self, "h", None):
            self.lib.vc2hip_destroy(self.h)
            self.h = None

    def __del__(self):
        try:
            self.close()
        except Exception:
            pass

    def _chk(self, rc):
        if rc != 0:
            raise Vc2HipError(rc, self.lib.vc2hip_last_error(self.h).decode())

    def padded_size(self, n, depth):
        return self.lib.vc2hip_padded_size(n, depth)

    def quant_matrix(self, kernel, depth):
        out = np.zeros(3 * depth + 1, np.int32)
        rc = self.lib.vc2hip_quant_matrix(kernel, depth, out)
        if rc:
            raise Vc2HipError(rc, "invalid wavelet kernel")
        return out

    def slice_bytes(self, ys, xs, total, scalar):
        out = np.empty((ys, xs), np.int32)
        self.lib.vc2hip_slice_bytes(ys, xs, total, scalar, out)
        return out

    def dwt_forward(self, plane, kernel, depth):
        plane = np.ascontiguousarray(plane, np.int32)
        h, w = plane.shape
        out = np.empty((self.padded_size(h, depth), self.padded_size(w, depth)), np.int32)
        self._chk(self.lib.vc2hip_dwt_forward(self.h, plane, h, w, kernel, depth, out))
        return out

    def dwt_inverse(self, coef, kernel, depth, shape=None):
        coef = np.ascontiguousarray(coef, np.int32)
        ph, pw = coef.shape
        h, w = shape if shape is not None else (ph, pw)
        out = np.empty((h, w), np.int32)
        self._chk(self.lib.vc2hip_dwt_inverse(self.h, coef, ph, pw, kernel, depth, out, h, w))
        return out

    def _q(self, fn, plane, depth, qidx, qm):
        plane = np.ascontiguousarray(plane, np.int32)
        qidx = np.ascontiguousarray(qidx, np.int32)
        out = np.empty_like(plane)
        self._chk(fn(self.h, plane, plane.shape[0], plane.shape[1], depth, qidx, qidx.shape[0],
                     qidx.shape[1], np.ascontiguousarray(qm, np.int32), out))
        return out

    def quantise_np(self, plane, depth, qidx, qm):
        return self._q(self.lib.vc2hip_quantise_np, plane, depth, qidx, qm)

    def dequantise_np(self, plane, depth, qidx, qm):
        return self._q(self.lib.vc2hip_dequantise_np, plane, depth, qidx, qm)

    def dequantise_ld(self, plane, depth, qidx, qm):
        return self._q(self.lib.vc2hip_dequantise_ld, plane, depth, qidx, qm)

    def quantise_ld(self, plane, depth, qidx, qm):
        return self._q(self.lib.vc2hip_quantise_ld, plane, depth, qidx, qm)

    @staticmethod
    def geom(y, u, depth, ys, xs):
        return Geom(y.shape[0], y.shape[1], u.shape[0], u.shape[1], depth, ys, xs)

    def hq_pack(self, y, u, v, depth, qidx, prefix=0, scalar=1, cbr=None):
        y, u, v = (np.ascontiguousarray(a, np.int32) for a in (y, u, v))
        qidx = np.ascontiguousarray(qidx, np.int32)
        g = self.geom(y, u, depth, qidx.shape[0], qidx.shape[1])
        cap = qidx.size * (prefix + 4 + 3 * 255 * scalar) + 64
        cbr_p = None
        if cbr is not None:
            cbr = np.ascontiguousarray(cbr, np.int32)
            cap = int(cbr.sum()) + qidx.size * prefix + 64
            cbr_p = cbr.ctypes.data_as(C.c_void_p)
        out = np.empty(cap, np.uint8)
        n = C.c_size_t()
        self._chk(self.lib.vc2hip_hq_pack(self.h, y, u, v, C.byref(g), qidx, prefix, scalar, cbr_p, out,
                                          cap, C.byref(n)))
        return out[:n.value].copy()

    def hq_unpack(self, data, lshape, cshape, depth, ys, xs, prefix=0, scalar=1):
        y = np.zeros(lshape, np.int32)
        u = np.zeros(cshape, np.int32)
        v = np.zeros(cshape, np.int32)
        q = np.zeros((ys, xs), np.int32)
        g = self.geom(y, u, depth, ys, xs)
        used = C.c_size_t()
        data = np.ascontiguousarray(data, np.uint8)
        self._chk(self.lib.vc2hip_hq_unpack(self.h, data, data.size, C.byref(g), prefix, scalar, y, u, v, q,
                                            C.byref(used)))
        return y, u, v, q, used.value

    def ld_unpack(self, data, lshape, cshape, depth, slice_bytes):
        ys, xs = slice_bytes.shape
        y = np.zeros(lshape, np.int32)
        u = np.zeros(cshape, np.int32)
        v = np.zeros(cshape, np.int32)
        q = np.zeros((ys, xs), np.int32)
        g = self.geom(y, u, depth, ys, xs)
        used = C.c_size_t()
        data = np.ascontiguousarray(data, np.uint8)
# ... 173 lines not shown
```

Measured before the change: 119,900 Mpixels/s.

## Run first-level forward pair DWT lifting in packed 16-bit lanes when bounds allow

Adds a packed int16x2 path for the first-level horizontal and vertical lifting of the forward pair kernel (DD97/LeGall, 16-bit store). An interval-arithmetic bound check decides whether intermediates fit in 16 bits for the given bit depth, and the DD97 predict step is split to avoid overflow. The aim is to halve register and ALU work per pixel on the largest level by packing two samples per dword. The cost is extra unpacking when feeding level b and more kernel variants; an env flag restores the 32-bit path.

```diff
diff --git a/include/vc2hip.h b/include/vc2hip.h
--- a/include/vc2hip.h
+++ b/include/vc2hip.h
@@ -49,6 +49,7 @@
 #define VC2HIP_FLAG_PLANES8_ALWAYS  0x400u
 #define VC2HIP_FLAG_PLANES8_NEVER   0x800u
 #define VC2HIP_FLAG_TWO_PASS_VBR    0x1000u
+#define VC2HIP_FLAG_LIFT32          0x2000u
 int vc2hip_create_with_flags(int device, unsigned flags, vc2hip_ctx **out);
 int vc2hip_create_on_stream(int device, void *hip_stream, vc2hip_ctx **out);
 void vc2hip_destroy(vc2hip_ctx *ctx);
@@ -188,8 +189,11 @@
   int small_gather;
   int pictures;
   int band_planes;
+  int lift_bits;
 } vc2hip_dwt_launch;
 int vc2hip_dwt_launches(const vc2hip_ctx *ctx, vc2hip_dwt_launch *out, int cap);
+
+int vc2hip_lift16_admits(int wavelet, int bit_depth, long long *max_intermediate);
 
 int vc2hip_profile_enable(vc2hip_ctx *ctx, int on);
 int vc2hip_profile_only(vc2hip_ctx *ctx, const char *name);
diff --git a/vc2-reference_amd/csrc/vc2hip_api.hip b/vc2-reference_amd/csrc/vc2hip_api.hip
--- a/vc2-reference_amd/csrc/vc2hip_api.hip
+++ b/vc2-reference_amd/csrc/vc2hip_api.hip
@@ -29,7 +29,8 @@
 size_t vc2_stream_level_applicable(LevelParams &p, int kernel, bool edge, bool inverse, bool store16, int n_pictures);
 int vc2_launch_forward_stream(Launcher &L, int kernel, bool first, const LevelParams &p, int n, bool store16, size_t lds, hipStream_t s);
 int vc2_launch_inverse_stream(Launcher &L, int kernel, bool final_level, const LevelParams &p, int n, bool store16, size_t lds, hipStream_t s);
-size_t vc2_pair_applicable(PairParams &pp, int kernel, bool edge, bool inverse, bool store16, int n_pictures);
+size_t vc2_pair_applicable(PairParams &pp, int kernel, bool edge, bool inverse, bool store16, int n_pictures, bool allow_l16 = false);
+int vc2_lift16_bound(int kernel, int bit_depth, long long *peak);
 int vc2_launch_forward_pair(Launcher &L, int kernel, bool first, const PairParams &pp, int n, bool store16, size_t lds, hipStream_t s);
 int vc2_launch_inverse_pair(Launcher &L, int kernel, bool final_level, const PairParams &pp, int n, bool store16, size_t lds, hipStream_t s);
 void vc2_upload_tables_pair(const QuantTables &t, hipStream_t s);
@@ -157,6 +158,7 @@
   bool allow_cbr_index = true;
   bool allow_stream = true;
   bool allow_pair = true;
+  bool allow_lift16 = true;
   bool cbr_general = false;
   bool ld_diagonals = false;
   unsigned flags = 0;
@@ -324,7 +326,8 @@
       {"VC2HIP_NO_BANDPLANES", VC2HIP_FLAG_NO_BANDPLANES}, {"VC2HIP_NO_HEADS", VC2HIP_FLAG_NO_HEADS},
       {"VC2HIP_NO_CBR_INDEX", VC2HIP_FLAG_NO_CBR_INDEX}, {"VC2HIP_GENERIC_DWT", VC2HIP_FLAG_GENERIC_DWT},
       {"VC2HIP_SINGLE_PASS_VBR", VC2HIP_FLAG_SINGLE_PASS_VBR}, {"VC2HIP_TWO_PASS_VBR", VC2HIP_FLAG_TWO_PASS_VBR}, {"VC2HIP_CBR_GENERAL", VC2HIP_FLAG_CBR_GENERAL},
-      {"VC2HIP_PLANES8_ALWAYS", VC2HIP_FLAG_PLANES8_ALWAYS}, {"VC2HIP_PLANES8_NEVER", VC2HIP_FLAG_PLANES8_NEVER}};
+      {"VC2HIP_PLANES8_ALWAYS", VC2HIP_FLAG_PLANES8_ALWAYS}, {"VC2HIP_PLANES8_NEVER", VC2HIP_FLAG_PLANES8_NEVER},
+      {"VC2HIP_LIFT32", VC2HIP_FLAG_LIFT32}};
     for (const auto &e : env) { const char *v = getenv(e.name); if (v && v[0] == '1') flags |= e.flag; }
     { const char *v = getenv("VC2HIP_LD_ROWS"); if (v && v[0] == '0') flags |= VC2HIP_FLAG_LD_DIAGONALS; }
     { const char *e = getenv("VC2HIP_DEBUG_SKIP"); c->debug_skip = e ? atoi(e) : 0; }
@@ -334,6 +337,7 @@
   c->allow_store16 = !(flags & VC2HIP_FLAG_STORE32);
   c->allow_stream = !(flags & VC2HIP_FLAG_NO_STREAM);
   c->allow_pair = !(flags & VC2HIP_FLAG_NO_PAIR);
+  c->allow_lift16 = !(flags & VC2HIP_FLAG_LIFT32);
   c->allow_planes = !(flags & VC2HIP_FLAG_NO_BANDPLANES);
   c->planes8_mode = (flags & VC2HIP_FLAG_PLANES8_NEVER) ? 2 : (flags & VC2HIP_FLAG_PLANES8_ALWAYS) ? 1 : 0;
   c->allow_heads = !(flags & VC2HIP_FLAG_NO_HEADS);
@@ -674,11 +678,12 @@
 static void ll_layout(const Geom &g, int n, int32_t *base, LLPlanes &ll) { ll_layout(g, n, base, 4, nullptr, ll); }
 
 static void record_dwt(vc2hip_ctx *c, bool inverse, int level, int levels, int family, bool edge, bool s16, int segments, int tail,
-                       bool small_gather, int n, int band_planes = 0) {
+                       bool small_gather, int n, int band_planes = 0, int lift_bits = 32) {
   if (c->dwt_rec_stale) { c->dwt_rec.clear(); c->dwt_rec_stale = false; }
   vc2hip_dwt_launch r;
   r.inverse = inverse; r.level = level; r.levels = levels; r.family = family; r.edge = edge; r.store_bits = s16 ? 16 : 32;
   r.segments = segments; r.tail = tail; r.small_gather = small_gather; r.pictures = n; r.band_planes = band_planes;
+  r.lift_bits = lift_bits;
   c->dwt_rec.push_back(r);
 }
 
@@ -750,11 +755,11 @@
       pp.a = p;
       pp.a.debug_skip = c->debug_skip;
       level_params(pp.b, level + 1);
-      const size_t lds = vc2_pair_applicable(pp, kernel, first, false, s16, n);
+      const size_t lds = vc2_pair_applicable(pp, kernel, first, false, s16, n, c->allow_lift16);
       if (lds) {
         int rc = vc2_launch_forward_pair(c->L, kernel, first, pp, n, s16, lds, c->stream);
         if (rc) return set_err(c, rc, "invalid wavelet kernel");
-        record_dwt(c, false, level, 2, VC2HIP_DWT_PAIR, first, s16, pp.a.st_segmax, 0, false, n);
+        record_dwt(c, false, level, 2, VC2HIP_DWT_PAIR, first, s16, pp.a.st_segmax, 0, false, n, 0, pp.lift16 ? 16 : 32);
         ++level;
         continue;
       }
@@ -1785,6 +1790,9 @@
 }
 
 extern "C" int vc2hip_band_plane_bits(const vc2hip_ctx *c) { return c ? c->last_plane_bits : 0; }
+extern "C" int vc2hip_lift16_admits(int wavelet, int bit_depth, long long *max_intermediate) {
+  return vc2_lift16_bound(wavelet, bit_depth, max_intermediate);
+}
 
 namespace {
 struct HeaderBits {
diff --git a/vc2-reference_amd/csrc/vc2hip_dwt_pair.hip b/vc2-reference_amd/csrc/vc2hip_dwt_pair.hip
--- a/vc2-reference_amd/csrc/vc2hip_dwt_pair.hip
+++ b/vc2-reference_amd/csrc/vc2hip_dwt_pair.hip
@@ -52,10 +52,13 @@
 #define VC2_PAIR_PF 2
 #endif
 constexpr int PFP = VC2_PAIR_PF;
-template <int K, bool FIRST, class ST>
+template <int K> constexpr bool pair_l16() { return K == VC2HIP_DD97 || K == VC2HIP_LEGALL; }
+template <int K, bool FIRST, class ST, bool L16 = false>
 __global__ __launch_bounds__(64, (pair_wpe<K>())) void k_fwd_pair(const PairParams pp) {
+  static_assert(!L16 || (FIRST && std::is_same<ST, int16_t>::value && pair_l16<K>()), "packed level a: raw words in, 16-bit store out");
   using S_ = St<ST>;
-  using EA = VEng<K, false, 4>;
+  using EA = std::conditional_t<L16, VEng<K, false, 2, vc2_h2>, VEng<K, false, 4>>;
+  using RA = typename EA::Row;
   using EB = VEng<K, false, 2>;
   using T = VT<K, false>;
   constexpr int OFFL = T::OFFL, SD = T::sum_dmin();
@@ -110,8 +113,17 @@
       }
     }
   };
-  auto convert = [&](int m, int slot, int h, RowT<4> &r) __attribute__((always_inline)) {
-    if constexpr (FIRST) {
+  auto convert = [&](int m, int slot, int h, RA &r) __attribute__((always_inline)) {
+    if constexpr (L16) {
+      const unsigned w[4] = {pf[slot][h][0].x, pf[slot][h][0].y, pf[slot][h][0].z, pf[slot][h][0].w};
+      const vc2_u2 sh = (vc2_u2)(unsigned short)sshift;
+#pragma unroll
+      for (int k = 0; k < 2; ++k) {
+        const unsigned e = __builtin_amdgcn_perm(w[2 * k + 1], w[2 * k], 0x04050001u), o = __builtin_amdgcn_perm(w[2 * k + 1], w[2 * k], 0x06070203u);
+        r[k] = __builtin_bit_cast(vc2_h2, (__builtin_bit_cast(vc2_u2, e) >> sh) << (unsigned short)ACC) + (short)bias;
+        r[2 + k] = __builtin_bit_cast(vc2_h2, (__builtin_bit_cast(vc2_u2, o) >> sh) << (unsigned short)ACC) + (short)bias;
+      }
+    } else if constexpr (FIRST) {
       const unsigned w[4] = {pf[slot][h][0].x, pf[slot][h][0].y, pf[slot][h][0].z, pf[slot][h][0].w};
 #pragma unroll
       for (int k = 0; k < 4; ++k) {
@@ -159,6 +171,15 @@
 #pragma unroll
         for (int j = 0; j < NV; ++j)
           if (!S_::fits(v[b * NV + j])) { (j < H ? w0 : w1)[j % H] = v[b * NV + j]; v[b * NV + j] = VC2_ST_SENTINEL; }
+    }
+  };
+  auto stageA16 = [&](ST *img, int r, const RA &oe, const RA &oo) __attribute__((always_inline)) {
+    const unsigned v[6] = {h2u(oe[2]), h2u(oe[3]), h2u(oo[0]), h2u(oo[1]), h2u(oo[2]), h2u(oo[3])};
+    ST *d = img + baseA + r * bswA;
+#pragma unroll
+    for (int b = 0; b < 3; ++b, d += bnA) {
+      if (spl == 1) *(uint2 *)d = make_uint2(v[2 * b], v[2 * b + 1]);
+      else { *(unsigned *)d = v[2 * b]; *(unsigned *)(d + ssA) = v[2 * b + 1]; }
     }
   };
   auto stageA = [&](ST *img, int r, int sv, const RowT<4> &oe, const RowT<4> &oo) __attribute__((always_inline)) {
@@ -264,6 +285,7 @@
   int slotBs = 0, slotBf = 0;
   bool due = false;
   int llE[4] = {0, 0, 0, 0};
+  unsigned llE16[2] = {0, 0};
   int mb = m0;
 
   auto burst = [&]() __attribute__((always_inline)) {
@@ -329,7 +351,7 @@
       constexpr int UA = U0 & 3;
       constexpr int MODEA = DRAIN ? 2 : (BM == 1 && U0 < 4) ? 1 : 0;
       const int m = DRAIN ? npA + U0 : mb + U0;
-      RowT<4> re, ro;
+      RA re, ro;
       if constexpr (!DRAIN) {
         convert(min(m, mload), U0 % PFP, 0, re);
         convert(min(m, mload), U0 % PFP, 1, ro);
@@ -337,16 +359,22 @@
       deferred();
       if constexpr (!DRAIN) {
         fetch(min(m + PFP, mload), U0 % PFP);
-        h_lift<K, false, 4>(re, redge);
-        h_lift<K, false, 4>(ro, redge);
+        if constexpr (L16) {
+          h_lift16<K>(re, redge);
+          h_lift16<K>(ro, redge);
+        } else {
+          h_lift<K, false, 4>(re, redge);
+          h_lift<K, false, 4>(ro, redge);
+        }
       }
       engA.template step<UA, MODEA, (DRAIN ? U0 : UA)>(m, npA, re, ro);
       const int k = m - OFFL;
-      const RowT<4> &oe = engA.template out<UA>(false), &oo = engA.template out<UA>(true);
+      const RA &oe = engA.template out<UA>(false), &oo = engA.template out<UA>(true);
       if (k >= kA && k < kB) {
         const int r = k & (bshA - 1), sv = k >> lbshA;
         if (!(dskip & 32)) {
-          if (own) stageA(imgA + ((sv - sv0) & (grpA - 1)) * szA, r, sv, oe, oo);
+          if constexpr (L16) { if (own) stageA16(imgA + ((sv - sv0) & (grpA - 1)) * szA, r, oe, oo); }
+          else if (own) stageA(imgA + ((sv - sv0) & (grpA - 1)) * szA, r, sv, oe, oo);
           if (r == bshA - 1) {
             dnA = sv + 1;
             if (((sv + 1 - sv0) & (grpA - 1)) == 0 || sv + 1 == sv1) due = true;
@@ -355,8 +383,11 @@
       }
       constexpr bool KODD = ((U0 - OFFL) & 1) != 0;
       if constexpr (!KODD) {
-#pragma unroll
-        for (int j = 0; j < 4; ++j) llE[j] = oe[j];
+        if constexpr (L16) { llE16[0] = h2u(oe[0]); llE16[1] = h2u(oe[1]); }
+        else {
+#pragma unroll
+          for (int j = 0; j < 4; ++j) llE[j] = oe[j];
+        }
       } else {
         constexpr int J = fdiv2(U0 - OFFL - 1);
         constexpr int UB = ((J % 4) + 4) % 4;
@@ -365,10 +396,18 @@
         if (!SKIP && !(dskip & 8)) {
           const int m1 = ((DRAIN ? npA : mb) >> 1) + J;
           RowT<2> re1, ro1;
-          re1[0] = (int)((unsigned)llE[0] << ACC); re1[1] = (int)((unsigned)llE[2] << ACC);
-          re1[2] = (int)((unsigned)llE[1] << ACC); re1[3] = (int)((unsigned)llE[3] << ACC);
-          ro1[0] = (int)((unsigned)oe[0] << ACC); ro1[1] = (int)((unsigned)oe[2] << ACC);
-          ro1[2] = (int)((unsigned)oe[1] << ACC); ro1[3] = (int)((unsigned)oe[3] << ACC);
+          if constexpr (L16) {
+            const unsigned e0 = llE16[0], e1 = llE16[1], o0 = h2u(oe[0]), o1 = h2u(oe[1]);
+            re1[0] = (int)(e0 << 16) >> (16 - ACC); re1[1] = (int)(e1 << 16) >> (16 - ACC);
+            re1[2] = ((int)e0 >> 16) << ACC;       re1[3] = ((int)e1 >> 16) << ACC;
+            ro1[0] = (int)(o0 << 16) >> (16 - ACC); ro1[1] = (int)(o1 << 16) >> (16 - ACC);
+            ro1[2] = ((int)o0 >> 16) << ACC;       ro1[3] = ((int)o1 >> 16) << ACC;
+          } else {
+            re1[0] = (int)((unsigned)llE[0] << ACC); re1[1] = (int)((unsigned)llE[2] << ACC);
+            re1[2] = (int)((unsigned)llE[1] << ACC); re1[3] = (int)((unsigned)llE[3] << ACC);
+            ro1[0] = (int)((unsigned)oe[0] << ACC); ro1[1] = (int)((unsigned)oe[2] << ACC);
+            ro1[2] = (int)((unsigned)oe[1] << ACC); ro1[3] = (int)((unsigned)oe[3] << ACC);
+          }
           h_lift<K, false, 2>(re1, redge);
           h_lift<K, false, 2>(ro1, redge);
           engB.template step<UB, MODEB>(m1, npB, re1, ro1);
@@ -904,10 +943,12 @@
 #else
 #define VC2_PAIR_HAS(INV, EDGE) (!(INV) || !(EDGE) || VC2_PAIR_INV_EDGE)
 #endif
-template <int K, bool EDGE, bool INV, class ST> const void *pair_fn(bool SPL2) {
+template <int K, bool EDGE, bool INV, class ST> constexpr bool has_l16() { return !INV && EDGE && pair_l16<K>() && std::is_same<ST, int16_t>::value; }
+template <int K, bool EDGE, bool INV, class ST> const void *pair_fn(bool SPL2, bool l16) {
   if constexpr (!pair_kernel<K>() || !VC2_PAIR_HAS(INV, EDGE)) return nullptr;
   else if constexpr (INV) return SPL2 ? (const void *)k_inv_pair<K, EDGE, ST, true> : (const void *)k_inv_pair<K, EDGE, ST, false>;
-  else return (const void *)k_fwd_pair<K, EDGE, ST>;
+  else if constexpr (has_l16<K, EDGE, INV, ST>()) return l16 ? (const void *)k_fwd_pair<K, EDGE, ST, true> : (const void *)k_fwd_pair<K, EDGE, ST>;
+  else return l16 ? nullptr : (const void *)k_fwd_pair<K, EDGE, ST>;
 }
 template <int K, bool EDGE, bool INV, class ST>
 int launch_pair(Launcher &L, const PairParams &pp, int n_pictures, size_t lds, hipStream_t s) {
@@ -923,17 +964,22 @@
       else VC2_LAUNCH(L, (k_inv_pair<K, EDGE, ST, false>), grid, block, 0, s, pp);
     } else {
       vc2_prof_begin(L, EDGE ? "dwt_pair_first" : "dwt_pair", s);
-      vc2_allow_lds((const void *)k_fwd_pair<K, EDGE, ST>, std::max<size_t>(64 * 1024, lds));
-      VC2_LAUNCH(L, (k_fwd_pair<K, EDGE, ST>), grid, block, lds, s, pp);
+      const void *fn = pair_fn<K, EDGE, INV, ST>(false, pp.lift16 != 0);
+      if (!fn) return VC2HIP_EINVAL;
+      vc2_allow_lds(fn, std::max<size_t>(64 * 1024, lds));
+      if constexpr (has_l16<K, EDGE, INV, ST>()) {
+        if (pp.lift16) VC2_LAUNCH(L, (k_fwd_pair<K, EDGE, ST, true>), grid, block, lds, s, pp);
+        else VC2_LAUNCH(L, (k_fwd_pair<K, EDGE, ST>), grid, block, lds, s, pp);
+      } else VC2_LAUNCH(L, (k_fwd_pair<K, EDGE, ST>), grid, block, lds, s, pp);
     }
     vc2_prof_end(L, s);
     return 0;
   }
 }
-template <int K, bool EDGE, bool INV, class ST> int pair_slots_of(size_t lds) {
+template <int K, bool EDGE, bool INV, class ST> int pair_slots_of(size_t lds, bool l16) {
   int nb = 0, dev = 0;
   hipDeviceProp_t prop;
-  const void *fn = pair_fn<K, EDGE, INV, ST>(false);
+  const void *fn = pair_fn<K, EDGE, INV, ST>(false, l16);
   if (!fn) return 0;
   if (!INV) vc2_allow_lds(fn, std::max<size_t>(64 * 1024, lds));
   if (hipGetDevice(&dev) != hipSuccess || hipGetDeviceProperties(&prop, dev) != hipSuccess ||
@@ -954,25 +1000,25 @@
 #undef VC2_CASE
   return VC2HIP_EINVAL;
 }
-template <bool INV, class ST> int pair_slots_dispatch(int kernel, bool edge, size_t lds) {
-#define VC2_CASE(KK) case KK: return edge ? pair_slots_of<KK, true, INV, ST>(lds) : pair_slots_of<KK, false, INV, ST>(lds);
+template <bool INV, class ST> int pair_slots_dispatch(int kernel, bool edge, size_t lds, bool l16) {
+#define VC2_CASE(KK) case KK: return edge ? pair_slots_of<KK, true, INV, ST>(lds, l16) : pair_slots_of<KK, false, INV, ST>(lds, l16);
   switch (kernel) { VC2_PAIR_CASES(VC2_CASE) }
 #undef VC2_CASE
   return 0;
 }
-int pair_slots(int kernel, bool edge, bool inverse, bool store16, size_t lds) {
+int pair_slots(int kernel, bool edge, bool inverse, bool store16, size_t lds, bool l16) {
   static std::mutex mu;
-  static std::map<std::tuple<int, int, int, int, size_t, int>, int> cache;
+  static std::map<std::tuple<int, int, int, int, size_t, int, int>, int> cache;
   int dev = 0;
   (void)hipGetDevice(&dev);
-  const auto key = std::make_tuple(kernel, (int)edge, (int)inverse, (int)store16, lds, dev);
+  const auto key = std::make_tuple(kernel, (int)edge, (int)inverse, (int)store16, lds, dev, (int)l16);
   std::lock_guard<std::mutex> lock(mu);
   auto it = cache.find(key);
   if (it != cache.end()) return it->second;
   int v;
   if (!store16) v = 0;
-  else if (inverse) v = pair_slots_dispatch<true, int16_t>(kernel, edge, lds);
-  else v = pair_slots_dispatch<false, int16_t>(kernel, edge, lds);
+  else if (inverse) v = pair_slots_dispatch<true, int16_t>(kernel, edge, lds, false);
+  else v = pair_slots_dispatch<false, int16_t>(kernel, edge, lds, l16);
   cache[key] = v;
   return v;
 }
@@ -1012,13 +1058,74 @@
   return best / elem;
 }
 
-}
-
-size_t vc2_pair_applicable(PairParams &pp, int kernel, bool edge, bool inverse, bool store16, int n_pictures) {
+struct Iv {
+  long long lo, hi;
+  long long *pk;
+};
+Iv seen(long long lo, long long hi, long long *pk) {
+  *pk = std::max(*pk, std::max(lo < 0 ? -lo : lo, hi < 0 ? -hi : hi));
+  return Iv{lo, hi, pk};
+}
+Iv operator+(const Iv &a, const Iv &b) { return seen(a.lo + b.lo, a.hi + b.hi, a.pk); }
+Iv operator-(const Iv &a, const Iv &b) { return seen(a.lo - b.hi, a.hi - b.lo, a.pk); }
+Iv operator-(const Iv &a) { return seen(-a.hi, -a.lo, a.pk); }
+Iv operator+(const Iv &a, int b) { return seen(a.lo + b, a.hi + b, a.pk); }
+Iv operator*(int b, const Iv &a) { return b >= 0 ? seen(a.lo * b, a.hi * b, a.pk) : seen(a.hi * b, a.lo * b, a.pk); }
+Iv operator>>(const Iv &a, int b) { return seen(a.lo >> b, a.hi >> b, a.pk); }
+Iv operator<<(const Iv &a, int b) { return seen(a.lo * (1LL << b), a.hi * (1LL << b), a.pk); }
+Iv operator&(const Iv &a, int b) {
+  if (b != 1) abort();
+  return a.lo == a.hi ? seen(a.lo & 1, a.lo & 1, a.pk) : seen(0, 1, a.pk);
+}
+template <int K, bool SPLIT, int S = 0> void iv_lift(Iv &e, Iv &o) {
+  if constexpr (S < WT<K>::nsteps) {
+    if constexpr (step_targets_odd<K, S>()) o = o + lift_delta<K, S, SPLIT>([&](int) { return e; });
+    else e = e + lift_delta<K, S, SPLIT>([&](int) { return o; });
+    iv_lift<K, SPLIT, S + 1>(e, o);
+  }
+}
+template <int K> long long lift16_peak(int d) {
+  long long pk = 0;
+  const int acc = WT<K>::accuracy;
+  const Iv x = seen(-(1LL << (d - 1)) * (1LL << acc), ((1LL << (d - 1)) - 1) * (1LL << acc), &pk);
+  Iv e = x, o = x;
+  iv_lift<K, false>(e, o);
+  const Iv cols[2] = {e, o};
+  for (const Iv &c : cols) {
+    Iv ve = c, vo = c;
+    iv_lift<K, true>(ve, vo);
+  }
+  return pk;
+}
+
+}
+
+int vc2_lift16_bound(int kernel, int bit_depth, long long *peak) {
+  long long pk = 0;
+  if (bit_depth < 1 || bit_depth > 16) return VC2HIP_EINVAL;
+  switch (kernel) {
+    case VC2HIP_DD97: pk = lift16_peak<VC2HIP_DD97>(bit_depth); break;
+    case VC2HIP_LEGALL: pk = lift16_peak<VC2HIP_LEGALL>(bit_depth); break;
+    case VC2HIP_DD137: pk = lift16_peak<VC2HIP_DD137>(bit_depth); break;
+    case VC2HIP_HAAR0: pk = lift16_peak<VC2HIP_HAAR0>(bit_depth); break;
+    case VC2HIP_HAAR1: pk = lift16_peak<VC2HIP_HAAR1>(bit_depth); break;
+    case VC2HIP_FIDELITY: pk = lift16_peak<VC2HIP_FIDELITY>(bit_depth); break;
+    case VC2HIP_DAUB97: pk = lift16_peak<VC2HIP_DAUB97>(bit_depth); break;
+    default: return VC2HIP_EINVAL;
+  }
+  if (peak) *peak = pk;
+  return pk <= 32767 ? 1 : 0;
+}
+
+size_t vc2_pair_applicable(PairParams &pp, int kernel, bool edge, bool inverse, bool store16, int n_pictures, bool allow_l16) {
   PairTaps t;
   if (!pair_taps(kernel, inverse, t)) return 0;
   LevelParams &p = pp.a;
   const LevelParams &pb = pp.b;
+  pp.lift16 = 0;
+  if (allow_l16 && edge && !inverse && store16 && p.word_bytes == 2 && (kernel == VC2HIP_DD97 || kernel == VC2HIP_LEGALL) &&
+      vc2_lift16_bound(kernel, 16 - p.sample_shift, nullptr) == 1 && vc2_lift16_bound(kernel, 16 - p.sample_shift_c, nullptr) == 1)
+    pp.lift16 = 1;
   const int elem = store16 ? 2 : 4;
   const bool b_last = inverse ? pb.ll_from_store != 0 : pb.ll_to_store != 0;
   if (inverse && (p.bp8 || pb.bp8)) return 0;
@@ -1088,7 +1195,7 @@
   if (lds > 48 * 1024) return 0;
   int cols = 0;
   for (int c = 0; c < 3; ++c) if (p.st_strips[c]) cols += p.st_strips[c] * n_pictures;
-  const int slots = pair_slots(kernel, edge, inverse, store16, lds);
+  const int slots = pair_slots(kernel, edge, inverse, store16, lds, pp.lift16 != 0);
   if (slots <= 0) return 0;
   const int runin = -3 * t.sd + 3 * t.offl + 8;
   int nseg = 0;
@@ -1123,7 +1230,7 @@
   p.st_prio = prio;
   p.st_lds = (int)lds;
 #ifdef VC2HIP_ABLATE
-  if (getenv("VC2HIP_PAIR_DEBUG")) fprintf(stderr, "pair: kernel %d edge %d lds %zu (img a %zu) slots %d cols %d nseg %d runin %d\n", kernel, (int)edge, lds, imgA, slots, cols, nseg, runin);
+  if (getenv("VC2HIP_PAIR_DEBUG")) fprintf(stderr, "pair: kernel %d edge %d lift16 %d lds %zu (img a %zu) slots %d cols %d nseg %d runin %d\n", kernel, (int)edge, pp.lift16, lds, imgA, slots, cols, nseg, runin);
 #endif
   return lds;
 }
diff --git a/vc2-reference_amd/csrc/vc2hip_internal.h b/vc2-reference_amd/csrc/vc2hip_internal.h
--- a/vc2-reference_amd/csrc/vc2hip_internal.h
+++ b/vc2-reference_amd/csrc/vc2hip_internal.h
@@ -120,6 +120,7 @@
   int ring_ll, n_ll;
   int ss_a[3], ss_b[3];
   int piece_a[3], piece_b[3];
+  int lift16;
 };
 
 #include <stdlib.h>
diff --git a/vc2-reference_amd/csrc/vc2hip_stream_eng.h b/vc2-reference_amd/csrc/vc2hip_stream_eng.h
--- a/vc2-reference_amd/csrc/vc2hip_stream_eng.h
+++ b/vc2-reference_amd/csrc/vc2hip_stream_eng.h
@@ -12,19 +12,25 @@
 #endif
 constexpr int PFI = VC2_STREAM_PFI;
 
-template <int NP> struct RowT {
-  int v[2 * NP];
-  __device__ __forceinline__ int &operator[](int i) { return v[i]; }
-  __device__ __forceinline__ const int &operator[](int i) const { return v[i]; }
+template <int NP, class E = int> struct RowT {
+  E v[2 * NP];
+  __device__ __forceinline__ E &operator[](int i) { return v[i]; }
+  __device__ __forceinline__ const E &operator[](int i) const { return v[i]; }
 };
 using Row = RowT<4>;
-template <int NP> __device__ __forceinline__ RowT<NP> operator+(const RowT<NP> &a, const RowT<NP> &b) { RowT<NP> r; _Pragma("unroll") for (int i = 0; i < 2 * NP; ++i) r.v[i] = a.v[i] + b.v[i]; return r; }
-template <int NP> __device__ __forceinline__ RowT<NP> operator-(const RowT<NP> &a, const RowT<NP> &b) { RowT<NP> r; _Pragma("unroll") for (int i = 0; i < 2 * NP; ++i) r.v[i] = a.v[i] - b.v[i]; return r; }
-template <int NP> __device__ __forceinline__ RowT<NP> operator-(const RowT<NP> &a) { RowT<NP> r; _Pragma("unroll") for (int i = 0; i < 2 * NP; ++i) r.v[i] = -a.v[i]; return r; }
-template <int NP> __device__ __forceinline__ RowT<NP> operator+(const RowT<NP> &a, int b) { RowT<NP> r; _Pragma("unroll") for (int i = 0; i < 2 * NP; ++i) r.v[i] = a.v[i] + b; return r; }
-template <int NP> __device__ __forceinline__ RowT<NP> operator*(int b, const RowT<NP> &a) { RowT<NP> r; _Pragma("unroll") for (int i = 0; i < 2 * NP; ++i) r.v[i] = b * a.v[i]; return r; }
-template <int NP> __device__ __forceinline__ RowT<NP> operator>>(const RowT<NP> &a, int b) { RowT<NP> r; _Pragma("unroll") for (int i = 0; i < 2 * NP; ++i) r.v[i] = a.v[i] >> b; return r; }
-template <int NP> __device__ __forceinline__ RowT<NP> vc2_times9(const RowT<NP> &a) { RowT<NP> r; _Pragma("unroll") for (int i = 0; i < 2 * NP; ++i) r.v[i] = ::vc2_times9(a.v[i]); return r; }
+using RowH = RowT<2, vc2_h2>;
+template <class E> __device__ __forceinline__ E vc2_splat(int b) { if constexpr (std::is_same<E, int>::value) return b; else return (E)(short)b; }
+template <int NP, class E> __device__ __forceinline__ RowT<NP, E> operator+(const RowT<NP, E> &a, const RowT<NP, E> &b) { RowT<NP, E> r; _Pragma("unroll") for (int i = 0; i < 2 * NP; ++i) r.v[i] = a.v[i] + b.v[i]; return r; }
+template <int NP, class E> __device__ __forceinline__ RowT<NP, E> operator-(const RowT<NP, E> &a, const RowT<NP, E> &b) { RowT<NP, E> r; _Pragma("unroll") for (int i = 0; i < 2 * NP; ++i) r.v[i] = a.v[i] - b.v[i]; return r; }
+template <int NP, class E> __device__ __forceinline__ RowT<NP, E> operator-(const RowT<NP, E> &a) { RowT<NP, E> r; _Pragma("unroll") for (int i = 0; i < 2 * NP; ++i) r.v[i] = -a.v[i]; return r; }
+template <int NP, class E> __device__ __forceinline__ RowT<NP, E> operator+(const RowT<NP, E> &a, int b) { RowT<NP, E> r; _Pragma("unroll") for (int i = 0; i < 2 * NP; ++i) r.v[i] = a.v[i] + vc2_splat<E>(b); return r; }
+template <int NP, class E> __device__ __forceinline__ RowT<NP, E> operator*(int b, const RowT<NP, E> &a) { RowT<NP, E> r; _Pragma("unroll") for (int i = 0; i < 2 * NP; ++i) r.v[i] = vc2_splat<E>(b) * a.v[i]; return r; }
+template <int NP, class E> __device__ __forceinline__ RowT<NP, E> operator>>(const RowT<NP, E> &a, int b) { RowT<NP, E> r; _Pragma("unroll") for (int i = 0; i < 2 * NP; ++i) r.v[i] = a.v[i] >> vc2_splat<E>(b); return r; }
+template <int NP, class E> __device__ __forceinline__ RowT<NP, E> operator<<(const RowT<NP, E> &a, int b) { RowT<NP, E> r; _Pragma("unroll") for (int i = 0; i < 2 * NP; ++i) r.v[i] = a.v[i] << vc2_splat<E>(b); return r; }
+template <int NP, class E> __device__ __forceinline__ RowT<NP, E> operator&(const RowT<NP, E> &a, int b) { RowT<NP, E> r; _Pragma("unroll") for (int i = 0; i < 2 * NP; ++i) r.v[i] = a.v[i] & vc2_splat<E>(b); return r; }
+template <int NP, class E> __device__ __forceinline__ RowT<NP, E> vc2_times9(const RowT<NP, E> &a) { RowT<NP, E> r; _Pragma("unroll") for (int i = 0; i < 2 * NP; ++i) r.v[i] = ::vc2_times9(a.v[i]); return r; }
+__device__ __forceinline__ unsigned h2u(vc2_h2 x) { return __builtin_bit_cast(unsigned, x); }
+__device__ __forceinline__ vc2_h2 u2h(unsigned x) { return __builtin_bit_cast(vc2_h2, x); }
 
 template <int CTRL> __device__ __forceinline__ int dppm(int old, int v) {
   return __builtin_amdgcn_update_dpp(old, v, CTRL, 0xf, 0xf, false);
@@ -97,6 +103,36 @@
     h_step<K, 1, true, NP>(r, redge);
     h_step<K, 0, true, NP>(r, redge);
   }
+}
+
+template <int K, int S> __device__ __forceinline__ void h_step16(RowH &r, bool redge) {
+  constexpr bool odd = step_targets_odd<K, S>();
+  constexpr int dmin = step_dmin<K, S>(), dmax = step_dmax<K, S>();
+  static_assert(-dmin <= 2 && dmax <= 2, "taps beyond the adjacent lane's pair of dwords");
+  constexpr int TO = odd ? 2 : 0, UO = odd ? 0 : 2;
+  const unsigned d0 = h2u(r[UO]), d1 = h2u(r[UO + 1]);
+  unsigned dl = 0, dr = 0;
+  if constexpr (dmin < 0) dl = (unsigned)dppm<0x138>((int)(d0 << 16), (int)d1);
+  if constexpr (dmax > 0) {
+    const unsigned last = __builtin_amdgcn_perm(d1, d1, 0x03020302u);
+    const unsigned nb = (unsigned)dppm<0x130>((int)last, (int)d0);
+    dr = redge ? last : nb;
+  }
+  auto dw = [&](int q) -> unsigned { return q < 0 ? dl : q == 0 ? d0 : q == 1 ? d1 : dr; };
+#pragma unroll
+  for (int i = 0; i < 2; ++i) {
+    const vc2_h2 d = lift_delta<K, S>([&](int t) -> vc2_h2 {
+      const int j = 2 * i + t;
+      if (j % 2 == 0) return u2h(dw(j / 2));
+      return u2h(__builtin_amdgcn_alignbit(dw((j + 1) / 2), dw((j - 1) / 2), 16));
+    });
+    r[TO + i] = r[TO + i] + d;
+  }
+}
+template <int K> __device__ __forceinline__ void h_lift16(RowH &r, bool redge) {
+  static_assert(WT<K>::nsteps == 2, "two lifting steps");
+  h_step16<K, 0>(r, redge);
+  h_step16<K, 1>(r, redge);
 }
 
 template <int K, bool INV> struct VT {
@@ -123,9 +159,10 @@
 };
 
 template <int K> constexpr int RLK = K == VC2HIP_FIDELITY ? 8 : 4;
-template <int K, bool INV, int NP = 4> struct VEng {
+template <int K, bool INV, int NP = 4, class E = int> struct VEng {
   using T = VT<K, INV>;
-  using Row = RowT<NP>;
+  using Row = RowT<NP, E>;
+  static constexpr bool PK = std::is_same<E, vc2_h2>::value;
   static constexpr int RL = RLK<K>;
   static_assert(T::len_raw(false) <= RL && T::len_raw(true) <= RL && T::len_x(0) <= RL && T::len_x(1) <= RL &&
                 (T::N < 3 || (T::len_x(2) <= RL && T::len_x(3) <= RL)), "row ring too short for this wavelet");
@@ -137,7 +174,7 @@
 #pragma unroll
     for (int j = 0; j < RL; ++j)
 #pragma unroll
-      for (int k = 0; k < 2 * NP; ++k) { rw[0][j].v[k] = 0; rw[1][j].v[k] = 0; x[0][j].v[k] = 0; x[1][j].v[k] = 0; x[2][j].v[k] = 0; x[3][j].v[k] = 0; }
+      for (int k = 0; k < 2 * NP; ++k) { rw[0][j].v[k] = E{}; rw[1][j].v[k] = E{}; x[0][j].v[k] = E{}; x[1][j].v[k] = E{}; x[2][j].v[k] = E{}; x[3][j].v[k] = E{}; }
   }
   template <int SLOT> static __device__ __forceinline__ void put(Row (&w)[RL], const Row &r, bool first) {
 #pragma unroll
@@ -167,7 +204,7 @@
           if constexpr (P == 0) W[t - dmin] = rw[T::odd(0) ? 0 : 1][sl(U - T::off(P) + t)];
           else W[t - dmin] = x[P - 1][sl(U - T::off(P) + t)];
         }
-        const Row d = lift_delta<K, T::sid(P)>([&](int t) -> Row { return W[t - dmin]; });
+        const Row d = lift_delta<K, T::sid(P), PK>([&](int t) -> Row { return W[t - dmin]; });
         Row o;
         if constexpr (P < 2) o = rw[T::odd(P) ? 1 : 0][dst];
         else o = x[P - 2][dst];
diff --git a/vc2-reference_amd/csrc/vc2hip_wavelets.h b/vc2-reference_amd/csrc/vc2hip_wavelets.h
--- a/vc2-reference_amd/csrc/vc2hip_wavelets.h
+++ b/vc2-reference_amd/csrc/vc2hip_wavelets.h
@@ -1,4 +1,6 @@
 #pragma once
+#include <type_traits>
+
 #include "vc2hip_internal.h"
 
 template <int K> struct WT;
@@ -10,17 +12,23 @@
 template <> struct WT<VC2HIP_FIDELITY> { static constexpr int nsteps = 2, accuracy = 0, halo = 14; };
 template <> struct WT<VC2HIP_DAUB97>   { static constexpr int nsteps = 4, accuracy = 1, halo = 4; };
 
-template <int K, int S> __device__ __forceinline__ constexpr bool step_targets_odd() {
+template <int K, int S> __host__ __device__ __forceinline__ constexpr bool step_targets_odd() {
   if constexpr (K == VC2HIP_FIDELITY) return S == 1;
   else return (S % 2) == 0;
 }
 
 __device__ __forceinline__ int vc2_times9(int x) { return (int)(((unsigned)x << 3) + (unsigned)x); }
-template <class T> __device__ __forceinline__ T vc2_times9(const T &x) { const T d = x + x, q = d + d; return q + q + x; }
+typedef short vc2_h2 __attribute__((ext_vector_type(2)));
+typedef unsigned short vc2_u2 __attribute__((ext_vector_type(2)));
+__device__ __forceinline__ vc2_h2 vc2_times9(vc2_h2 x) { return (x << (short)3) + x; }
+template <class T> __host__ __device__ __forceinline__ T vc2_times9(const T &x) { const T d = x + x, q = d + d; return q + q + x; }
 
-template <int K, int S, class F> __device__ __forceinline__ auto lift_delta(F at) {
+template <int K, int S, bool SPLIT = false, class F> __host__ __device__ __forceinline__ auto lift_delta(F at) {
   if constexpr (K == VC2HIP_DD97 || K == VC2HIP_DD137) {
-    if constexpr (S == 0) return -((vc2_times9(at(0) + at(1)) - (at(-1) + at(2)) + 8) >> 4);
+    if constexpr (S == 0 && SPLIT) {
+      const auto t = at(0) + at(1);
+      return -((t >> 1) + ((((t & 1) << 3) + t - (at(-1) + at(2)) + 8) >> 4));
+    } else if constexpr (S == 0) return -((vc2_times9(at(0) + at(1)) - (at(-1) + at(2)) + 8) >> 4);
     else if constexpr (K == VC2HIP_DD97) return (at(-1) + at(0) + 2) >> 2;
     else return (vc2_times9(at(-1) + at(0)) - (at(-2) + at(1)) + 16) >> 5;
   } else if constexpr (K == VC2HIP_LEGALL) {
diff --git a/vc2-reference_amd/vc2hip_py.py b/vc2-reference_amd/vc2hip_py.py
--- a/vc2-reference_amd/vc2hip_py.py
+++ b/vc2-reference_amd/vc2hip_py.py
@@ -11,7 +11,7 @@
 
 FLAGS = {"STORE32": 0x001, "NO_STREAM": 0x002, "NO_PAIR": 0x004, "NO_BANDPLANES": 0x008, "NO_HEADS": 0x010, "NO_CBR_INDEX": 0x020,
          "GENERIC_DWT": 0x040, "SINGLE_PASS_VBR": 0x080, "CBR_GENERAL": 0x100, "LD_DIAGONALS": 0x200,
-         "PLANES8_ALWAYS": 0x400, "PLANES8_NEVER": 0x800, "TWO_PASS_VBR": 0x1000}
+         "PLANES8_ALWAYS": 0x400, "PLANES8_NEVER": 0x800, "TWO_PASS_VBR": 0x1000, "LIFT32": 0x2000}
 
 KERNELS = {"DD97": 0, "LeGall": 1, "DD137": 2, "Haar0": 3, "Haar1": 4, "Fidelity": 5, "Daub97": 6}
 CF = {"444": 0, "422": 1, "420": 2}
@@ -38,7 +38,7 @@
 class DwtLaunch(C.Structure):
     _fields_ = [("inverse", C.c_int), ("level", C.c_int), ("levels", C.c_int), ("family", C.c_int), ("edge", C.c_int),
                 ("store_bits", C.c_int), ("segments", C.c_int), ("tail", C.c_int), ("small_gather", C.c_int),
-                ("pictures", C.c_int), ("band_planes", C.c_int)]
+                ("pictures", C.c_int), ("band_planes", C.c_int), ("lift_bits", C.c_int)]
 
 
 class StreamParams(C.Structure):
@@ -67,7 +67,7 @@
     "vc2hip_profile_enable", "vc2hip_profile_only", "vc2hip_profile_count", "vc2hip_profile_get", "vc2hip_profile_reset",
     "vc2hip_host_alloc", "vc2hip_host_free", "vc2hip_encode_picture_begin", "vc2hip_encode_picture_end",
     "vc2hip_decode_picture_begin", "vc2hip_decode_picture_end", "vc2hip_band_plane_bits", "vc2hip_dwt_launches",
-    "vc2hip_picture_header", "vc2hip_stream_write_dev", "vc2hip_stream_read_dev",
+    "vc2hip_picture_header", "vc2hip_stream_write_dev", "vc2hip_stream_read_dev", "vc2hip_lift16_admits",
 ]
 
 
@@ -136,6 +136,7 @@
     lib.vc2hip_profile_reset.argtypes = [vp]
     lib.vc2hip_band_plane_bits.argtypes = [vp]
     lib.vc2hip_dwt_launches.argtypes = [vp, C.POINTER(DwtLaunch), C.c_int]
+    lib.vc2hip_lift16_admits.argtypes = [C.c_int, C.c_int, C.POINTER(C.c_longlong)]
     lib.vc2hip_host_alloc.argtypes = [C.c_size_t]
     lib.vc2hip_host_alloc.restype = vp
     lib.vc2hip_host_free.argtypes = [vp]
@@ -147,6 +148,14 @@
                                                 C.POINTER(C.c_int)]
     lib.vc2hip_decode_picture_end.argtypes = [vp, C.c_int]
     return lib
+
+
+def lift16_admits(lib, kernel, bits):
+    pk = C.c_longlong(0)
+    rc = lib.vc2hip_lift16_admits(kernel, bits, C.byref(pk))
+    if rc < 0:
+        raise Vc2HipError(rc, "vc2hip_lift16_admits")
+    return bool(rc), int(pk.value)
 
 
 def picture_format(width, height, cf, bits, word_bytes=2, chroma_bits=0):
```

Result: no change. 120,800 Mpixels/s (median of 6 runs) (+0.7%).
